# hyperplane-lab/RGBManip

Measured on AMD Instinct MI355X. Metric: adapose_poses_per_sec_batch256, higher is better.
Workload: dtype bf16

## Files before the change

### include/rgbm.h

```cpp
#ifndef RGBM_H_
#define RGBM_H_
#include <stddef.h>
#include <stdint.h>

#ifdef __cplusplus
extern "C" {
#endif

#define RGBM_VERSION 100
#define RGBM_F32 0
#define RGBM_BF16 1
#define RGBM_F16 2
#define RGBM_BF16X3 3

int rgbm_version(void);
const char* rgbm_last_error(void);

typedef struct rgbm_weight_desc {
  const char* name;
  const float* data;
  int ndim;
  const int64_t* shape;
} rgbm_weight_desc;

// ... 88 lines not shown
int rgbm_synth_render(const rgbm_synth_scene* scene, const double* rays_dev, float* color_dev, uint8_t* mask_dev, void* stream);

int rgbm_gae(int T, int N, const float* rewards, const uint8_t* dones, const float* values, const float* last_values,
             float gamma, float lam, float* returns, float* adv, double* sums, void* stream);
int rgbm_adv_normalise(int64_t n_local, float* adv, const double* sums, double count_total, void* stream);

typedef struct rgbm_policy_layout {
  int dims[5];
  int log_std;
  int w[2][4];
  int b[2][4];
  int total;
} rgbm_policy_layout;
int rgbm_policy_forward(const float* params, const rgbm_policy_layout* L, int n, int mode, const float* obs, const float* noise,
                        float* actions, float* logp, float* value, float* mu, void* stream);
int rgbm_ppo_partial_floats(const rgbm_policy_layout* L, int n, size_t* count);
int rgbm_ppo_minibatch_fwd_bwd(const float* params, const rgbm_policy_layout* L, int n, const float* obs, const float* actions,
                               const float* old_logp, const float* adv, const float* returns, const float* old_values,
                               const float* old_mu, const float* old_log_std, float clip, float vcoef, float ecoef,
                               float* partial_scratch, float* grads_flat, void* stream);
int rgbm_ppo_clip_adam(float* params, const float* grads_flat, float* exp_avg, float* exp_avg_sq, void* opt_state,
                       const rgbm_policy_layout* L, float inv_world, float max_norm, float desired_kl, float lr_min,
                       float lr_max, int adaptive, void* stream);

int rgbm_conv_nd(int dtype, const void* in_dev, int N, int D, int H, int W, int Cin, int Cin_pad, const float* w_host,
                 int Cout, int Cout_pad, int KD, int KH, int KW, int stride_d, int stride_hw, int pad_d, int pad_hw,
                 int dil_hw, int transposed, const float* bias_host, const float* bn_scale_host, const float* bn_shift_host,
                 const void* res_dev, int res_mode, int act, float slope, void* out_dev, void* stream);
int rgbm_bn_per_sample_scratch_bytes(int V, size_t* bytes);
int rgbm_bn_per_sample(int dtype, void* y_dev, const void* res_dev, const float* gamma_dev, const float* beta_dev, void* scratch_dev,
                       int V, int64_t nvox, int C, int relu, void* stream);
int rgbm_conv3d_tile(int layer, int dtype, const void* in_dev, int N, int D, int H, int W, const float* w_host,
                     const float* bn_scale_host, const float* bn_shift_host, const void* res_dev, void* out_dev, void* stream);
int rgbm_upsample_conv3x3(int dtype, const void* in_dev, int V, int h, int w, int Cin, const float* w_host, int Cout,
                          const float* bias_host, int act, float slope, void* z_scratch_dev, void* out_dev, void* stream);
int rgbm_upsample_conv3x3_final(int dtype, const void* in_dev, int V, int h, int w, const float* w3_host, const float* b3_host,
                                float slope, const float* wf_host, const float* bf_host, void* out_dev, int out_f32, void* stream);
int rgbm_stem(int dtype, const float* img1_dev, const float* img2_dev, const float* w_host, void* out_dev, int B, int S, void* stream);
int rgbm_maxpool3x3s2(int dtype, const void* in_dev, void* out_dev, int V, int H, int W, int C, void* stream);
int rgbm_resize_bilinear_ac(int dtype, const void* in_dev, void* out_dev, int V, int Hs, int Ws, int C, int Ho, int Wo,
                            void* stream);
int rgbm_adaptive_avgpool(int dtype, const void* in_dev, void* out_dev, int V, int H, int W, int C, int S, void* stream);
int rgbm_build_volume(int dtype, const void* feat_dev, const float* P_views_dev, const float* depths_dev, float* homog_scratch,
                      void* vol_dev, int V, int B, int D, int H, int W, void* stream);
int rgbm_conv0_sweep(const void* feat_dev, const float* P_views_dev, const float* depths_dev, float* homog_scratch,
                     const float* w_host, const float* bn_scale_host, const float* bn_shift_host, void* out_dev,
                     int V, int B, int D, int H, int W, void* stream);
int rgbm_conv0_sweep_dt(int dtype, const void* feat_dev, const float* P_views_dev, const float* depths_dev, float* homog_scratch,
                        const float* w_host, const float* bn_scale_host, const float* bn_shift_host, void* out_dev,
                        int V, int B, int D, int H, int W, void* stream);
int rgbm_conv0_sweep_f16feat(const void* feat_f16_dev, const float* P_views_dev, const float* depths_dev, float* homog_scratch,
                             const float* w_host, const float* bn_scale_host, const float* bn_shift_host, void* out_bf16_dev,
                             int V, int B, int D, int H, int W, void* stream);
int rgbm_adapose_forward_ex(rgbm_adapose_t* h, int B, const float* img1, const float* img2, const int32_t* choose1,
                            const int32_t* choose2, const float* P1, const float* P2, const float* depths, void* workspace,
                            size_t workspace_bytes, const rgbm_adapose_out* out, int stop_after, void* stream);
int rgbm_adapose_forward_graph(rgbm_adapose_t* h, int B, const float* img1, const float* img2, const int32_t* choose1,
                               const int32_t* choose2, const float* P1, const float* P2, const float* depths, void* workspace,
                               size_t workspace_bytes, const rgbm_adapose_out* out, void* stream, int32_t* n_nodes, int32_t* captured);
int rgbm_adapose_graph_clear(rgbm_adapose_t* h);
int rgbm_adapose_fetch(rgbm_adapose_t* h, int B, void* workspace, const char* name, float* out_dev, size_t capacity,
                       size_t* n_elems, void* stream);

#define RGBM_PROF_ROWS 42
int rgbm_debug_flags(int flags);
int rgbm_set_tuning(const char* key, long long value);
int rgbm_microbench_mfma_scratch_floats(int* n);
int rgbm_microbench_mfma(float* scratch, int iters, int random_operands, double* flops, void* stream);
int rgbm_microbench_copy(const void* src, void* dst, size_t bytes, void* stream);
int rgbm_prof_rows(void);
int rgbm_prof_start(void);
int rgbm_prof_stop(double* stats);
int rgbm_prof_select(int row);

#ifdef __cplusplus
}
#endif
#endif
```

### rgbmanip_amd/_lib.py

```python
from __future__ import annotations

import ctypes as C
import os

_HERE = os.path.dirname(os.path.abspath(__file__))
LIB_PATH = os.environ.get("RGBM_HIP_LIB") or os.path.join(_HERE, "librgbm_hip.so")

F32, BF16, F16, BF16X3 = 0, 1, 2, 3
ACT_NONE, ACT_RELU, ACT_PRELU, ACT_TANH = 0, 1, 2, 3
RES_NONE, RES_PRE_ACT, RES_POST_ACT = 0, 1, 2


PROF_ROWS = 42
PROF_KERNELS = [
    ("conv_igemm_glds_kernel<float, 16, 256>", "fp32"), ("conv_igemm_glds_kernel<float, 32, 256>", "fp32"),
    ("conv_igemm_glds_kernel<float, 64, 256>", "fp32"), ("conv_igemm_glds_kernel<float, 128, 128>", "fp32"),
    ("conv_igemm_glds_kernel<unsigned short, 16, 256>", "bf16"), ("conv_igemm_glds_kernel<unsigned short, 32, 256>", "bf16"),
    ("conv_igemm_glds_kernel<unsigned short, 64, 256>", "bf16"), ("conv_igemm_glds_kernel<unsigned short, 128, 128>", "bf16"),
    ("conv3d_tile_kernel<float, ...> (conv1..conv11)", "fp32"), ("conv3d_tile_kernel<unsigned short, ...> (conv1..conv11)", "bf16"),
    ("conv3d_tile_kernel<float, 32, 16, 4, 8, 8, 1, false, true> (conv0 + fused plane sweep)", "fp32"),
    ("conv3d_tile_kernel<unsigned short, 32, 16, 4, 8, 8, 1, false, true> (conv0 + fused plane sweep)", "bf16"),
    ("conv_igemm_ws_kernel<float, ...>", "fp32"), ("conv_igemm_ws_kernel<unsigned short, false, false> (128 channels x 256 pixels)", "bf16"),
    ("conv0_sweep_persistent_kernel<unsigned short> (conv0 + fused plane sweep of bf16 nets; sweep_f16 = 0 / fp16 nets: conv0_sweep_kernel)", "bf16"), ("conv_igemm_ws64_kernel", "bf16"),
    ("conv3d_tile_kernel<unsigned short, 32, 16, 6, 8, 8, 1, false, false> (conv0 on a materialised volume)", "bf16"),
# ... 47 lines not shown


class SynthScene(C.Structure):
    _fields_ = [("cam_pose", C.c_void_p), ("robot_pose", C.c_void_p), ("box", C.c_void_p),
                ("fx", C.c_double), ("fy", C.c_double), ("cx", C.c_double), ("cy", C.c_double),
                ("N", C.c_int), ("H", C.c_int), ("W", C.c_int), ("env0", C.c_int)]


_vp, _i, _f, _d, _sz, _i64 = C.c_void_p, C.c_int, C.c_float, C.c_double, C.c_size_t, C.c_int64

SIGNATURES = {
    "rgbm_version": (_i, []),
    "rgbm_last_error": (C.c_char_p, []),
    "rgbm_adapose_create": (_i, [C.POINTER(_vp), _i, C.POINTER(WeightDesc), _i, _i, _i]),
    "rgbm_adapose_destroy": (_i, [_vp]),
    "rgbm_adapose_set_chunk": (_i, [_vp, _i]),
    "rgbm_adapose_set_option": (_i, [_vp, C.c_char_p, _i]),
    "rgbm_adapose_workspace_bytes": (_i, [_vp, _i, C.POINTER(_sz)]),
    "rgbm_adapose_set_dropout": (_i, [_vp, _f, C.c_uint64]),
    "rgbm_adapose_dropout_masks": (_i, [_vp, _i, _vp]),
    "rgbm_adapose_set_dropout_masks": (_i, [_vp, _i, _vp]),
    "rgbm_adapose_forward": (_i, [_vp, _i, _vp, _vp, _vp, _vp, _vp, _vp, _vp, _vp, _sz, C.POINTER(AdaposeOut), _vp]),
    "rgbm_adapose_forward_ex": (_i, [_vp, _i, _vp, _vp, _vp, _vp, _vp, _vp, _vp, _vp, _sz, C.POINTER(AdaposeOut), _i, _vp]),
    "rgbm_adapose_forward_graph": (_i, [_vp, _i, _vp, _vp, _vp, _vp, _vp, _vp, _vp, _vp, _sz, C.POINTER(AdaposeOut), _vp, C.POINTER(C.c_int32),
                                        C.POINTER(C.c_int32)]),
    "rgbm_adapose_graph_clear": (_i, [_vp]),
    "rgbm_adapose_fetch": (_i, [_vp, _i, _vp, C.c_char_p, _vp, _sz, C.POINTER(_sz), _vp]),
    "rgbm_adapose_postprocess": (_i, [_i, _i, _i, _vp, _vp, _vp, _vp, _vp, _vp, _vp, _vp, _vp, _vp]),
    "rgbm_adapose_postprocess_scratch_bytes": (_i, [_i, C.POINTER(_sz)]),
    "rgbm_adapose_postprocess_ws": (_i, [_i, _i, _i, _vp, _vp, _vp, _vp, _vp, _vp, _vp, _vp, _vp, _vp, _sz, _vp]),
    "rgbm_adapose_postprocess_ransac": (_i, [_i, _i, _i, C.c_uint32, _vp, _vp, _vp, _vp, _vp, _vp, _vp, _vp, _vp]),
    "rgbm_adapose_postprocess_pnp": (_i, [_i, _i, C.c_uint32, _vp, _vp, _vp, _vp, _vp, _vp, _vp, _vp, _vp, _vp, _vp, _vp]),
    "rgbm_gae": (_i, [_i, _i, _vp, _vp, _vp, _vp, _f, _f, _vp, _vp, _vp, _vp]),
    "rgbm_adv_normalise": (_i, [_i64, _vp, _vp, _d, _vp]),
    "rgbm_policy_forward": (_i, [_vp, _vp, _i, _i, _vp, _vp, _vp, _vp, _vp, _vp, _vp]),
    "rgbm_ppo_partial_floats": (_i, [_vp, _i, C.POINTER(_sz)]),
    "rgbm_ppo_minibatch_fwd_bwd": (_i, [_vp, _vp, _i, _vp, _vp, _vp, _vp, _vp, _vp, _vp, _vp, _f, _f, _f, _vp, _vp, _vp]),
    "rgbm_ppo_clip_adam": (_i, [_vp, _vp, _vp, _vp, _vp, _vp, _f, _f, _f, _f, _f, _i, _vp]),
    "rgbm_conv_nd": (_i, [_i, _vp, _i, _i, _i, _i, _i, _i, _vp, _i, _i, _i, _i, _i, _i, _i, _i, _i, _i, _i, _vp, _vp, _vp,
                          _vp, _i, _i, _f, _vp, _vp]),
    "rgbm_bn_per_sample_scratch_bytes": (_i, [_i, C.POINTER(_sz)]),
    "rgbm_bn_per_sample": (_i, [_i, _vp, _vp, _vp, _vp, _vp, _i, _i64, _i, _i, _vp]),
    "rgbm_conv3d_tile": (_i, [_i, _i, _vp, _i, _i, _i, _i, _vp, _vp, _vp, _vp, _vp, _vp]),
    "rgbm_upsample_conv3x3": (_i, [_i, _vp, _i, _i, _i, _i, _vp, _i, _vp, _i, _f, _vp, _vp, _vp]),
    "rgbm_upsample_conv3x3_final": (_i, [_i, _vp, _i, _i, _i, _vp, _vp, _f, _vp, _vp, _vp, _i, _vp]),
    "rgbm_stem": (_i, [_i, _vp, _vp, _vp, _vp, _i, _i, _vp]),
    "rgbm_maxpool3x3s2": (_i, [_i, _vp, _vp, _i, _i, _i, _i, _vp]),
    "rgbm_resize_bilinear_ac": (_i, [_i, _vp, _vp, _i, _i, _i, _i, _i, _i, _vp]),
    "rgbm_adaptive_avgpool": (_i, [_i, _vp, _vp, _i, _i, _i, _i, _i, _vp]),
    "rgbm_build_volume": (_i, [_i, _vp, _vp, _vp, _vp, _vp, _i, _i, _i, _i, _i, _vp]),
    "rgbm_conv0_sweep": (_i, [_vp, _vp, _vp, _vp, _vp, _vp, _vp, _vp, _i, _i, _i, _i, _i, _vp]),
    "rgbm_conv0_sweep_dt": (_i, [_i, _vp, _vp, _vp, _vp, _vp, _vp, _vp, _vp, _i, _i, _i, _i, _i, _vp]),
    "rgbm_conv0_sweep_f16feat": (_i, [_vp, _vp, _vp, _vp, _vp, _vp, _vp, _vp, _i, _i, _i, _i, _i, _vp]),
    "rgbm_prepare_inputs": (_i, [_vp, _vp, _vp, _i, _i, _i, _i, _i, C.c_uint32, _vp, _vp, _vp, _vp, _vp, _vp, _vp, _vp]),
    "rgbm_prepare_inputs_indexed": (_i, [_vp, _vp, _vp, _vp, _i, _i, _i, _i, _i, C.c_uint32, _vp, _vp, _vp, _vp, _vp, _vp, _vp, _vp]),
    "rgbm_prepare_inputs_ex": (_i, [_vp, _vp, _vp, _vp, _i, _i, _i, _i, _i, _i, C.c_uint32, _vp, _vp, _vp, _vp, _vp, _vp, _vp, _vp]),
    "rgbm_projection": (_i, [_vp, _vp, _vp, _i, _vp]),
    "rgbm_mask_extent": (_i, [_vp, _i, _i, _i, _vp, _vp, _vp]),
    "rgbm_lookat_quat": (_i, [_vp, _i, _i, _vp, _vp]),
    "rgbm_control_action_to_pose": (_i, [_vp, _i, C.POINTER(C.c_double), C.POINTER(C.c_double), C.POINTER(C.c_double), _i, _vp, _vp]),
    "rgbm_control_reward": (_i, [C.POINTER(ControlRewardArgs), _vp]),
    "rgbm_control_grasp_frame": (_i, [_vp, _i, _vp, _vp, _vp]),
    "rgbm_synth_camera": (_i, [C.POINTER(SynthScene), _vp, _vp, _vp, _vp]),
    "rgbm_synth_render": (_i, [C.POINTER(SynthScene), _vp, _vp, _vp, _vp]),
    "rgbm_debug_flags": (_i, [_i]),
    "rgbm_set_tuning": (_i, [C.c_char_p, _i64]),
    "rgbm_prof_rows": (_i, []),
    "rgbm_microbench_mfma_scratch_floats": (_i, [C.POINTER(C.c_int)]),
    "rgbm_microbench_mfma": (_i, [_vp, _i, _i, C.POINTER(C.c_double), _vp]),
    "rgbm_microbench_copy": (_i, [_vp, _vp, C.c_size_t, _vp]),
    "rgbm_prof_start": (_i, []),
    "rgbm_prof_select": (_i, [_i]),
    "rgbm_prof_stop": (_i, [C.POINTER(C.c_double)]),
}

_lib = None


def load():
    global _lib
    if _lib is not None:
        return _lib
    if not os.path.exists(LIB_PATH):
        raise RgbmError(f"{LIB_PATH} not found: build it with rgbmanip_amd/csrc/build.sh "
                        f"(or `python -c 'import __graft_entry__ as g; g.build()'`). There is no CPU fallback.")
    lib = C.CDLL(LIB_PATH)
    for name, (res, args) in SIGNATURES.items():
        fn = getattr(lib, name)
        fn.restype = res
        fn.argtypes = args
    if lib.rgbm_prof_rows() != PROF_ROWS:
        raise RgbmError(f"{LIB_PATH}: rgbm_prof_rows() = {lib.rgbm_prof_rows()}, this binding expects {PROF_ROWS} (stale build?)")
    _lib = lib
    return lib


def check(rc: int, what: str = ""):
    if rc != 0:
        msg = load().rgbm_last_error()
        raise RgbmError(f"{what} failed (code {rc}): {msg.decode() if msg else ''}")


def stream_ptr(stream=None):
    import torch
    s = stream if stream is not None else torch.cuda.current_stream()
    return C.c_void_p(s.cuda_stream)
# ... 5 lines not shown
```

### rgbmanip_amd/csrc/adapose.cpp

```cpp
#include "adapose.h"

#include <math.h>
#include <string.h>

namespace rgbm {

static const int kLayerPlanes[4] = {64, 128, 256, 512};
static const int kLayerBlocks[4] = {3, 4, 6, 3};
static const int kLayerStride[4] = {1, 2, 1, 1};
static const int kLayerDil[4] = {1, 1, 2, 4};
static const int kPspBins[4] = {1, 2, 3, 6};
static const int kPspSmallViews = 32;


static const HostTensor* find(const StateDict& sd, const std::string& name) {
  auto it = sd.find(name);
  return it == sd.end() ? nullptr : &it->second;
}

#define GET(var, name)                                               \
  const HostTensor* var = find(sd, name);                            \
  RGBM_REQUIRE(var != nullptr, std::string("missing weight ") + (name))

static int init_conv2d(ConvLayer& L, int dtype, const StateDict& sd, const std::string& wname, const char* bname, int Cin,
// ... 205 lines not shown
      if (upload_f32(w->data, w->numel(), &head_w[h][l])) return -2;
      if (upload_f32(b->data, b->numel(), &head_b[h][l])) return -2;
    }
  }
  return 0;
}

void AdaPose::destroy() {
  conv1.destroy();
  if (stem_w) (void)hipFree(stem_w);
  stem_w = nullptr;
  for (int i = 0; i < n_blocks; ++i) { blocks[i].c1.destroy(); blocks[i].c2.destroy(); if (blocks[i].has_ds) blocks[i].ds.destroy(); }
  for (auto& l : psp) l.destroy();
  up1.destroy(); up2.destroy(); up3.destroy(); fin.destroy();
  up1c.destroy(); up2c.destroy(); tail.destroy();
  if (drop_masks) (void)hipFree(drop_masks);
  if (drop_state) (void)hipFree(drop_state);
  drop_masks = nullptr; drop_state = nullptr; drop_cap_views = 0; drop_p = 0.f; drop_explicit = 0; drop_last_B = 0;
  for (auto& l : c3d) l.destroy();
  for (auto& l : dc) l.destroy();
  for (auto& l : c3d_raw) l.destroy();
  for (auto& l : dc_raw) l.destroy();
  for (int i = 0; i < 10; ++i) { if (bn_gamma[i]) (void)hipFree(bn_gamma[i]); if (bn_beta[i]) (void)hipFree(bn_beta[i]); bn_gamma[i] = bn_beta[i] = nullptr; }
  inst.destroy();
  for (auto& l : nh) l.destroy();
  for (auto& l : npm) l.destroy();
  for (auto& l : pm1) l.destroy();
  for (auto& l : pm2) l.destroy();
  for (auto& t : t3d) { if (t.w) (void)hipFree(t.w); if (t.bias) (void)hipFree(t.bias); t.w = nullptr; t.bias = nullptr; }
  if (sweep_w) (void)hipFree(sweep_w);
  sweep_w = nullptr;
  if (sweep_w_f16) (void)hipFree(sweep_w_f16);
  sweep_w_f16 = nullptr;
  if (w11_x3) (void)hipFree(w11_x3);
  w11_x3 = nullptr;
  if (w11_taps) (void)hipFree(w11_taps);
  w11_taps = nullptr;
  if (wprob) (void)hipFree(wprob);
  if (pm2_0_wfull) (void)hipFree(pm2_0_wfull);
  if (pmlp_table) { (void)hipFree(pmlp_table); pmlp_table = nullptr; }
  if (pm2_0_bias) (void)hipFree(pm2_0_bias);
  for (int h = 0; h < 3; ++h) for (int l = 0; l < 3; ++l) { if (head_w[h][l]) (void)hipFree(head_w[h][l]); if (head_b[h][l]) (void)hipFree(head_b[h][l]); }
}

bool AdaPose::feat_f32_only() const {
  return dtype == BF16X3 && cost_impl == 3 && sweep_w != nullptr && norm_mode == 0 && !(g_debug_flags & 4096);
}

bool AdaPose::feat_f16() const {
  return dtype == BF16 && sweep_f16 != 0 && cost_impl == 3 && sweep_w_f16 != nullptr && norm_mode == 0 && !(g_debug_flags & 4096) && (upconv & 4) &&
         tail.ready() && tail.f16_ready();
}

bool AdaPose::sparse_active() const {
  const bool b16 = dtype_size(dtype) == 2;
  return sparse_dec != 0 && norm_mode == 0 && cost_impl == 3 && (b16 || (dtype == BF16X3 && w11_x3)) && sparse_tail && sweep_w != nullptr &&
         !(g_debug_flags & 4096);
}

int AdaPose::chunk_views(int V) const {
  const int cap = norm_mode == 1 && max_chunk > 32 ? 32 : max_chunk;
  return V < cap ? V : cap;
}

int AdaPose::plan(int B, Arena& A, Buffers& bf) const {
  const int V = 2 * B, P = n_pts, S = img;
  const size_t es = dtype_size(dtype);
  const size_t VP = (size_t)V * P;
  bf.Pviews = (float*)A.alloc((size_t)V * 16 * 4);
  bf.homog = (float*)A.alloc((size_t)V * 12 * 4);
  bf.choose = (int*)A.alloc(VP * 4);
  bf.masks = (unsigned char*)A.alloc((size_t)V * sparse_mask_bytes_per_view(img));
  bf.sweep_list = (int*)A.alloc((size_t)V * ((img + 11) / 12) * ((img + 15) / 16) * 4);
  bf.sweep_count = (int*)A.alloc((size_t)(V + 64) * 4);
  bf.feat = A.alloc((size_t)V * S * S * 32 * es);
  bf.featf = dtype == BF16X3 ? (float*)A.alloc((size_t)V * S * S * 32 * 4) : nullptr;
  bf.X0 = (float*)A.alloc(VP * 32 * 4);
  bf.X1 = (float*)A.alloc(VP * 64 * 4);
  bf.H128 = (float*)A.alloc(VP * 128 * 4);
  bf.H64 = (float*)A.alloc(VP * 64 * 4);
  bf.nocs4 = (float*)A.alloc(VP * 4 * 4);
  bf.N32 = (float*)A.alloc(VP * 32 * 4);
  bf.PF96 = (float*)A.alloc(VP * 96 * 4);
  bf.PF96h = pose_dtype() == F16 ? A.alloc(VP * 96 * 2) : nullptr;
  bf.prob = (float*)A.alloc(VP * n_depth * 4);
  bf.depth = (float*)A.alloc(VP * 4);
  bf.Q128a = (float*)A.alloc(VP * 128 * 4);
  bf.Q128b = (float*)A.alloc(VP * 128 * 4);
  bf.G256a = (float*)A.alloc(VP * 256 * 4);
  bf.G256b = (float*)A.alloc(VP * 256 * 4);
  bf.glob = (float*)A.alloc((size_t)V * 128 * 4);
  bf.vbias = (float*)A.alloc((size_t)V * 256 * 4);
  bf.pf2 = (float*)A.alloc((size_t)V * 256 * 4);
  bf.h1 = (float*)A.alloc((size_t)V * 256 * 4);
  bf.h2 = (float*)A.alloc((size_t)V * 128 * 4);
  bf.r6 = (float*)A.alloc((size_t)V * 8 * 4);
  bf.R = (float*)A.alloc((size_t)V * 9 * 4);
  bf.tv = (float*)A.alloc((size_t)V * 4 * 4);
  bf.sv = (float*)A.alloc((size_t)V * 4 * 4);
  const size_t m0 = A.mark();
  bf.imgpad = A.alloc((size_t)V * S * S * img_cpad * es);
  bf.c1 = A.alloc((size_t)V * (S / 2) * (S / 2) * 64 * es);
  const size_t lbuf = (size_t)V * ((size_t)(S / 4) * (S / 4) * 64 > (size_t)(S / 8) * (S / 8) * 512 ? (size_t)(S / 4) * (S / 4) * 64 : (size_t)(S / 8) * (S / 8) * 512) * es;
  for (int i = 0; i < 4; ++i) bf.lb[i] = A.alloc(lbuf);
  for (int i = 0; i < 4; ++i) {
    bf.pooled[i] = A.alloc((size_t)V * kPspBins[i] * kPspBins[i] * 512 * es);
    bf.stage[i] = A.alloc((size_t)V * kPspBins[i] * kPspBins[i] * 128 * es);
  }
  const size_t f8 = (size_t)(S / 8) * (S / 8), f4 = (size_t)(S / 4) * (S / 4), f2 = (size_t)(S / 2) * (S / 2), f1 = (size_t)S * S;
  bf.cat = A.alloc((size_t)V * f8 * 1024 * es);
  bf.ups = A.alloc((size_t)V * f4 * 1024 * es);
  bf.u1 = A.alloc((size_t)V * f4 * 256 * es);
  bf.u2 = A.alloc((size_t)V * f2 * 64 * es);
  bf.u3 = A.alloc((size_t)V * f1 * 64 * es);
  A.release(m0);
  const int Vc = chunk_views(V);
  const int D = n_depth;
  const size_t vox = (size_t)D * S * S;
  bf.vol = (cost_impl >= 2 && norm_mode == 0) ? nullptr : A.alloc((size_t)Vc * vox * 32 * es);
  bf.bn_scratch = norm_mode == 1 ? A.alloc(bn_scratch_bytes(Vc)) : nullptr;
  bf.c[0] = A.alloc((size_t)Vc * vox * 8 * es);
  bf.c[1] = A.alloc((size_t)Vc * (vox / 8) * 16 * es);
  bf.c[2] = A.alloc((size_t)Vc * (vox / 8) * 16 * es);
  bf.c[3] = A.alloc((size_t)Vc * (vox / 64) * 32 * es);
  bf.c[4] = A.alloc((size_t)Vc * (vox / 64) * 32 * es);
  bf.c[5] = A.alloc((size_t)Vc * (vox / 512) * 64 * es);
  bf.c[6] = A.alloc((size_t)Vc * (vox / 512) * 64 * es);
  bf.u7 = A.alloc((size_t)Vc * (vox / 64) * 32 * es);
// ... 39 lines not shown
      if (int rc = blk.ds.run(x, r, V, 1, H, W, blk.planes, nullptr, 0, nullptr, 0, s)) return rc;
      res = r;
    }
    if (int rc = blk.c2.run(t, y, V, 1, Ho, Wo, blk.planes, res, RES_PRE_ACT, nullptr, 0, s)) return rc;
    H = Ho; W = Wo;
    xi = (xi + 3) & 3;
  }
  const void* f = bf.lb[xi];
  last_f_index = xi;
  RGBM_REQUIRE(H == S / 8 && W == S / 8, "feature stride");
  if (g_debug_flags & 1024) {
    if (int rc = launch_copy_channels(dtype, f, bf.cat, (long long)V * H * W, 512, 1024, 0, s)) return rc;
    {
      void* outs[4] = {bf.pooled[0], bf.pooled[1], bf.pooled[2], bf.pooled[3]};
      if (int rc = launch_adaptive_avgpool_multi(dtype, f, outs, kPspBins, 4, V, H, W, 512, s)) return rc;
    }
    for (int i = 0; i < 4; ++i) {
      const int Sb = kPspBins[i];
      if (int rc = psp[i].run(bf.pooled[i], bf.stage[i], V, 1, Sb, Sb, 128, nullptr, 0, nullptr, 0, s)) return rc;
      if (int rc = launch_resize_bilinear_ac(dtype, bf.stage[i], bf.cat, V, Sb, Sb, 128, H, W, 1024, 512 + 128 * i, s)) return rc;
    }
  } else {
    bool small = V <= kPspSmallViews;
    for (int i = 0; i < 4; ++i)
      small = small && psp[i].packs.size() == 1 && psp[i].packs[0].Kpad == 512 && psp[i].Cout_pad == 128 && psp[i].bias == nullptr;
    if (small) {
      const void* w[4] = {psp[0].packs[0].w, psp[1].packs[0].w, psp[2].packs[0].w, psp[3].packs[0].w};
      void* outs[4] = {bf.stage[0], bf.stage[1], bf.stage[2], bf.stage[3]};
      if (int rc = launch_psp_pool_conv(dtype, f, 512, w, outs, kPspBins, V, H, W, psp[0].g.act, psp[0].g.slope, s)) return rc;
    } else {
      void* outs[4] = {bf.pooled[0], bf.pooled[1], bf.pooled[2], bf.pooled[3]};
      if (int rc = launch_adaptive_avgpool_multi(dtype, f, outs, kPspBins, 4, V, H, W, 512, s)) return rc;
      for (int i = 0; i < 4; ++i)
        if (int rc = psp[i].run(bf.pooled[i], bf.stage[i], V, 1, kPspBins[i], kPspBins[i], 128, nullptr, 0, nullptr, 0, s)) return rc;
    }
    const void* stages[4] = {bf.stage[0], bf.stage[1], bf.stage[2], bf.stage[3]};
    if (int rc = launch_psp_resize_cat(dtype, f, stages, kPspBins, bf.cat, V, H, W, s)) return rc;
  }
  RGBM_REQUIRE(drop == nullptr || (upconv & 3) == 3, "dropout needs option upconv bits 0 and 1 (up_1 / up_2 through the tap combination)");
  if (upconv & 1) {
    if (int rc = up1c.run(bf.cat, bf.ups, bf.u1, V, H, W, 256, s, drop)) return rc;
  } else {
    if (int rc = launch_resize_bilinear_ac(dtype, bf.cat, bf.ups, V, H, W, 1024, 2 * H, 2 * W, 1024, 0, s)) return rc;
    if (int rc = up1.run(bf.ups, bf.u1, V, 1, 2 * H, 2 * W, 256, nullptr, 0, nullptr, 0, s)) return rc;
  }
  if (upconv & 2) {
    if (int rc = up2c.run(bf.u1, bf.ups, bf.u2, V, 2 * H, 2 * W, 64, s, drop ? drop + 256 : nullptr)) return rc;
  } else {
    if (int rc = launch_resize_bilinear_ac(dtype, bf.u1, bf.ups, V, 2 * H, 2 * W, 256, 4 * H, 4 * W, 256, 0, s)) return rc;
    if (int rc = up2.run(bf.ups, bf.u2, V, 1, 4 * H, 4 * W, 64, nullptr, 0, nullptr, 0, s)) return rc;
  }
  fin.out_plain_f32 = feat_f32_only();
  if ((upconv & 4) && tail.ready())
    return tail.run(bf.u2, fin.out_plain_f32 ? (void*)bf.featf : bf.feat, fin.out_plain_f32 ? 1 : feat_f16() ? 2 : 0, V, 4 * H, 4 * W, s);
  if (int rc = launch_resize_bilinear_ac(dtype, bf.u2, bf.ups, V, 4 * H, 4 * W, 64, 8 * H, 8 * W, 64, 0, s)) return rc;
  fin.out_plain_f32 = feat_f32_only();
  if (int rc = up3.run_then_1x1(fin, bf.ups, bf.u3, 64, fin.out_plain_f32 ? (void*)bf.featf : bf.feat, 32, V, 1, 8 * H, 8 * W, fuse_final != 0, nullptr, s)) return rc;
  return 0;
}

int AdaPose::cost_volume(const Buffers& bf, int V, int B, const float* depths, hipStream_t s) const {
  const int S = img, D = n_depth, P = n_pts;
  const int Vh = view2_heads ? V : B;
  const int Vc0 = chunk_views(V);
  const bool b16 = dtype_size(dtype) == 2;
  bool sweep_sparse = false;
  auto tile = [&](int layer, const void* in, void* out, const void* res, int Vc, int Di, int Hi, int Wi, int Do, int Ho,
                  int Wo, bool transposed, int v0, const unsigned char* tmask = nullptr) -> int {
    const int li = layer == 10 ? 0 : layer;
    Conv3dTileDesc d;
    memset(&d, 0, sizeof(d));
    d.in = in; d.wgt = t3d[li].w; d.out = out; d.bias = t3d[li].bias; d.res = res;
    d.N = Vc; d.Di = Di; d.Hi = Hi; d.Wi = Wi; d.Do = Do; d.Ho = Ho; d.Wo = Wo;
    d.Dq = transposed ? Di : Do; d.Hq = transposed ? Hi : Ho; d.Wq = transposed ? Wi : Wo;
    d.Cout = t3d[li].Cout; d.relu = 1;
    d.feat = bf.feat; d.homog = bf.homog; d.depths = depths; d.v0 = v0; d.V = V; d.B = B;
    d.out_classmajor = layer == 9 ? 1 : 0;
    d.tile_mask = tmask;
    d.tile_mask_stride = sparse_mask_bytes_per_view(S);
    if (layer == 10 && sweep_sparse) { d.tile_list = bf.sweep_list; d.tile_count = bf.sweep_count; }
    d.prof_variant = dtype == BF16X3 ? (layer == 10 ? 28 : 27) : layer == 10 ? 10 + (dtype != F32 ? 1 : 0) : (dtype != F32 ? 16 + layer : 8);
    d.algo_flops = 2.0 * Vc * (double)(transposed ? Di * Hi * Wi : Do * Ho * Wo) * t3d[li].Cout * 27.0 * t3d[li].Cin;
    d.algo_bytes = ((layer == 10 ? (double)Vc * Hi * Wi * t3d[li].Cin : (double)Vc * Di * Hi * Wi * t3d[li].Cin) +
                    (double)Vc * Do * Ho * Wo * t3d[li].Cout * (res ? 2 : 1)) * (double)dtype_size(dtype);
    if (layer == 10 && cost_impl == 3 && b16 && sweep_w && !(g_debug_flags & 4096)) {
      d.wgt = sweep_w;
      if (feat_f16()) { d.wgt = sweep_w_f16; d.feat_f16 = 1; }
      return launch_conv0_sweep(d, dtype, s);
    }
    if (layer == 10 && cost_impl == 3 && dtype == BF16X3 && sweep_w && !(g_debug_flags & 4096)) {
      d.wgt = sweep_w;
      d.feat = bf.featf;
      return launch_conv0_sweep_x3(d, s);
    }
    return launch_conv3d_tile(layer, dtype, d, s);
  };
  const bool sparse_ok = sparse_active();
  for (int v0 = 0; norm_mode == 0 && cost_impl >= 1 && v0 < Vh; v0 += Vc0) {
    const int Vc = Vh - v0 < Vc0 ? Vh - v0 : Vc0;
    const unsigned char* mk[10] = {nullptr, nullptr, nullptr, nullptr, nullptr, nullptr, nullptr, nullptr, nullptr, nullptr};
    sweep_sparse = false;
    if (sparse_ok) {
      int td, th, tw;
      for (int L : {1, 2, 3, 4, 5, 7, 8}) RGBM_REQUIRE(!conv3d_tile_dims(L, dtype, &td, &th, &tw) && th == 8 && tw == 8, "sparse cost regularisation: 8 x 8 tiles expected");
      if (int rc = launch_sparse_masks(bf.choose, v0, Vc, P, S, bf.masks, bf.sweep_list, bf.sweep_count, s)) return rc;
      for (int L : {7, 8}) mk[L] = bf.masks + sparse_mask_offset(S, L);
      if (sparse_dec >= 2) {
        for (int L : {1, 2, 3, 4, 5}) mk[L] = bf.masks + sparse_mask_offset(S, L);
        sweep_sparse = true;
      }
    }
    if (cost_impl == 1) {
      if (int rc = launch_build_volume(dtype, bf.feat, bf.homog, depths, bf.vol, v0, Vc, V, B, D, S, S, s)) return rc;
      if (int rc = tile(0, bf.vol, bf.c[0], nullptr, Vc, D, S, S, D, S, S, false, v0)) return rc;
    } else {
      if (int rc = tile(10, nullptr, bf.c[0], nullptr, Vc, D, S, S, D, S, S, false, v0)) return rc;
    }
    if (int rc = tile(1, bf.c[0], bf.c[1], nullptr, Vc, D, S, S, D / 2, S / 2, S / 2, false, v0, mk[1])) return rc;
    if (int rc = tile(2, bf.c[1], bf.c[2], nullptr, Vc, D / 2, S / 2, S / 2, D / 2, S / 2, S / 2, false, v0, mk[2])) return rc;
    if (int rc = tile(3, bf.c[2], bf.c[3], nullptr, Vc, D / 2, S / 2, S / 2, D / 4, S / 4, S / 4, false, v0, mk[3])) return rc;
    if (int rc = tile(4, bf.c[3], bf.c[4], nullptr, Vc, D / 4, S / 4, S / 4, D / 4, S / 4, S / 4, false, v0, mk[4])) return rc;
    if (int rc = tile(5, bf.c[4], bf.c[5], nullptr, Vc, D / 4, S / 4, S / 4, D / 8, S / 8, S / 8, false, v0, mk[5])) return rc;
    if (cost_impl == 3 && (b16 || dtype == BF16X3) && igemm_conv6) {
      if (int rc = c3d[6].run(bf.c[5], bf.c[6], Vc, D / 8, S / 8, S / 8, 64, nullptr, RES_NONE, nullptr, 0, s)) return rc;
    } else {
      if (int rc = tile(6, bf.c[5], bf.c[6], nullptr, Vc, D / 8, S / 8, S / 8, D / 8, S / 8, S / 8, false, v0)) return rc;
    }
    if (int rc = tile(7, bf.c[6], bf.u7, bf.c[4], Vc, D / 8, S / 8, S / 8, D / 4, S / 4, S / 4, true, v0, mk[7])) return rc;
    if (int rc = tile(8, bf.u7, bf.u9, bf.c[2], Vc, D / 4, S / 4, S / 4, D / 2, S / 2, S / 2, true, v0, mk[8])) return rc;
    if (cost_impl == 3 && (b16 || (dtype == BF16X3 && w11_x3)) && sparse_tail) {
      if (int rc = launch_prob_sparse(bf.u9, bf.c[0], dtype == BF16X3 ? w11_x3 : t3d[9].w, t3d[9].bias, wprob, bf.choose, depths, bf.prob,
                                      bf.depth, v0, Vc, B, P, D, S, S, dtype, s, w11_taps)) return rc;
      continue;
    }
    if (int rc = tile(9, bf.u9, bf.u11, bf.c[0], Vc, D / 2, S / 2, S / 2, D, S, S, true, v0)) return rc;
    if (int rc = launch_prob_softmax_depth(dtype, bf.u11, wprob, bf.choose, depths, bf.prob, bf.depth, v0, Vc, B, P, D, S, S, 1, s)) return rc;
  }
  for (int v0 = 0; norm_mode == 1 && v0 < Vh; v0 += Vc0) {
    const int Vc = Vh - v0 < Vc0 ? Vh - v0 : Vc0;
    if (int rc = launch_build_volume(dtype, bf.feat, bf.homog, depths, bf.vol, v0, Vc, V, B, D, S, S, s)) return rc;
// ... 28 lines not shown
    if (int rc = c3d[5].run(bf.c[4], bf.c[5], Vc, D / 4, S / 4, S / 4, 64, nullptr, 0, nullptr, 0, s)) return rc;
    if (int rc = c3d[6].run(bf.c[5], bf.c[6], Vc, D / 8, S / 8, S / 8, 64, nullptr, 0, nullptr, 0, s)) return rc;
    if (int rc = dc[0].run(bf.c[6], bf.u7, Vc, D / 8, S / 8, S / 8, 32, bf.c[4], RES_POST_ACT, nullptr, 0, s)) return rc;
    if (int rc = dc[1].run(bf.u7, bf.u9, Vc, D / 4, S / 4, S / 4, 16, bf.c[2], RES_POST_ACT, nullptr, 0, s)) return rc;
    if (int rc = dc[2].run(bf.u9, bf.u11, Vc, D / 2, S / 2, S / 2, 8, bf.c[0], RES_POST_ACT, nullptr, 0, s)) return rc;
    if (int rc = launch_prob_softmax_depth(dtype, bf.u11, wprob, bf.choose, depths, bf.prob, bf.depth, v0, Vc, B, P, D, S, S, 0, s)) return rc;
  }
  return 0;
}

int AdaPose::forward(int B, const float* img1, const float* img2, const int* choose1, const int* choose2, const float* P1,
                     const float* P2, const float* depths, void* workspace, size_t workspace_size, const Outputs& out,
                     hipStream_t s, int stop_after) const {
  RGBM_REQUIRE(B > 0, "batch");
  RGBM_REQUIRE(((uintptr_t)workspace & 255) == 0, "workspace must be 256-byte aligned");
  RGBM_REQUIRE(n_depth % 8 == 0 && img % 8 == 0, "depth/img must be multiples of 8");
  const size_t need = workspace_bytes(B);
  RGBM_REQUIRE(workspace_size >= need, "workspace too small: need " + std::to_string(need));
  Arena A(workspace, workspace_size);
  Buffers bf;
  plan(B, A, bf);
  const int V = 2 * B, P = n_pts, S = img, D = n_depth;
  const size_t VP = (size_t)V * P;

  if (int rc = launch_stage_in(P1, P2, choose1, choose2, bf.Pviews, bf.choose, B, P, s)) return rc;
  const float* drop = nullptr;
  if (drop_active()) {
    RGBM_REQUIRE(V <= drop_cap_views && drop_masks && (drop_explicit || drop_state), "dropout: mask buffer smaller than the batch");
    RGBM_REQUIRE((upconv & 3) == 3, "dropout needs option upconv bits 0 and 1 (up_1 / up_2 through the tap combination)");
    if (drop_explicit) {
      RGBM_REQUIRE(drop_explicit == B, "dropout: the masks set for the next forward are for batch " + std::to_string(drop_explicit));
      drop_explicit = 0;
    } else {
      if (int rc = launch_dropout_masks(drop_masks, drop_state, B, drop_p, drop_seed, drop_no_advance ? 0 : 1, s)) return rc;
    }
    drop = drop_masks;
    drop_last_B = B;
  }
  if (int rc = pspnet(bf, V, img1, img2, s, drop)) return rc;
  if (int rc = launch_homography(bf.Pviews, bf.homog, V, B, s)) return rc;
  const void* featg = bf.feat;
  int fdt = dtype;
  if (dtype == BF16X3) {
    if (!feat_f32_only())
      if (int rc = launch_bx3_to_f32(bf.feat, bf.featf, (long long)V * S * S * 32, s)) return rc;
    featg = bf.featf; fdt = F32;
  }
  if (feat_f16()) fdt = F16;
  if (stop_after == 1) return 0;

  const int Vh = view2_heads ? V : B;
  if (pmlp_table != nullptr && !(g_debug_flags & 2048) && ((long long)Vh * P) % 64 == 0) {
    PointMlpDesc pd{};
    pd.table = pmlp_table; pd.feat = featg; pd.choose = bf.choose; pd.nocs4 = bf.nocs4; pd.pf = bf.PF96 + 32; pd.ldpf = 96; pd.P = P; pd.HW = S * S;
    pd.N = (long long)Vh * P;
    if (int rc = launch_point_mlp(fdt, pd, s)) return rc;
  } else {
    if (int rc = launch_gather_points(fdt, featg, bf.choose, bf.X0, Vh, P, S * S, 32, s)) return rc;
    if (int rc = inst.run(bf.X0, bf.X1, Vh, 1, 1, P, 64, nullptr, 0, nullptr, 0, s)) return rc;
    if (int rc = nh[0].run(bf.X1, bf.H128, Vh, 1, 1, P, 128, nullptr, 0, nullptr, 0, s)) return rc;
    if (int rc = nh[1].run(bf.H128, bf.H64, Vh, 1, 1, P, 64, nullptr, 0, nullptr, 0, s)) return rc;
    if (int rc = nh[2].run(bf.H64, bf.nocs4, Vh, 1, 1, P, 4, nullptr, 0, nullptr, 0, s)) return rc;
    if (int rc = npm[0].run(bf.nocs4, bf.N32, Vh, 1, 1, P, 32, nullptr, 0, nullptr, 0, s)) return rc;
    if (int rc = npm[1].run(bf.N32, bf.PF96 + 32, Vh, 1, 1, P, 96, nullptr, 0, nullptr, 0, s)) return rc;
  }

  if (int rc = cost_volume(bf, V, B, depths, s)) return rc;
  if (stop_after == 2) return 0;

  if (int rc = launch_fuse_points(fdt, featg, bf.homog, depths, bf.choose, bf.prob, bf.PF96, V, B, P, D, S, S, 96, 0, s, Vh)) return rc;
  const int pdt = pose_dtype();
  const void* pf_in = bf.PF96;
  if (pdt == F16) {
    if (int rc = launch_f32_to_f16(bf.PF96, bf.PF96h, (long long)Vh * P * 96, s)) return rc;
    pf_in = bf.PF96h;
  } else if (pdt == BF16X3) {
    if (int rc = launch_f32_to_bx3(bf.PF96, bf.PF96, (long long)Vh * P * 96, s)) return rc;
  }
  if (int rc = pm1[0].run(pf_in, bf.Q128a, Vh, 1, 1, P, 128, nullptr, 0, nullptr, 0, s)) return rc;
  if (int rc = pm1[1].run(bf.Q128a, bf.Q128b, Vh, 1, 1, P, 128, nullptr, 0, nullptr, 0, s)) return rc;
  if (int rc = launch_mean_points_partial(pdt, bf.Q128b, (float*)bf.Q128a, Vh, P, 128, s)) return rc;
  if (int rc = launch_view_linear_mean((const float*)bf.Q128a, P, bf.glob, pm2_0_wfull, pm2_0_bias, bf.vbias, Vh, 128, 256, 256, 128, 0, s)) return rc;
  if (int rc = pm2[0].run(bf.Q128b, bf.G256a, Vh, 1, 1, P, 256, nullptr, 0, bf.vbias, 256, s)) return rc;
  if (int rc = pm2[1].run(bf.G256a, bf.G256b, Vh, 1, 1, P, 256, nullptr, 0, nullptr, 0, s)) return rc;
  if (int rc = launch_mean_points_partial(pdt, bf.G256b, (float*)bf.G256a, Vh, P, 256, s)) return rc;
  float* hout[3] = {bf.r6, bf.tv, bf.sv};
  const int hdim[3] = {6, 3, 3};
  if (int rc = launch_pose_heads_mean((const float*)bf.G256a, P, bf.pf2, bf.R, head_w, head_b, hout, hdim, Vh, s)) return rc;

  {
    float* const on[2] = {out.nocs1, out.nocs2};
    float* const od[2] = {out.depth1, out.depth2};
    float* const orr[2] = {out.r1, out.r2};
    float* const ot[2] = {out.t1, out.t2};
    float* const os[2] = {out.s1, out.s2};
    if (int rc = launch_stage_out(bf.nocs4, bf.depth, bf.R, bf.tv, bf.sv, on, od, orr, ot, os, B, P, view2_heads, s)) return rc;
  }
  (void)VP;
  return 0;
}

}
```

### rgbmanip_amd/csrc/adapose.h

```cpp
#pragma once
#include "kernels.h"
#include "layers.h"

namespace rgbm {

struct Arena {
  char* base; size_t off; size_t cap; size_t peak;
  explicit Arena(void* b, size_t c) : base((char*)b), off(0), cap(c), peak(0) {}
  void* alloc(size_t bytes) {
    off = align_up(off, 256);
    void* p = base ? base + off : nullptr;
    off += bytes;
    if (off > peak) peak = off;
    return p;
  }
  size_t mark() const { return off; }
  void release(size_t m) { off = m; }
};

struct AdaPose {
  int dtype = F32;
  int pose_dtype() const { return dtype == BF16 ? F16 : (dtype == BF16X3 && pose_x3) ? BF16X3 : F32; }
  int pose_x3 = 1;
  int img = 224, n_pts = 1024, n_depth = 24;
// ... 28 lines not shown
  void* sweep_w = nullptr;
  int cost_impl = 3;
  void* w11_x3 = nullptr;
  float* wprob = nullptr;
  ConvLayer inst, nh[3], npm[2], pm1[2], pm2[2];
  float* pm2_0_wfull = nullptr;
  float* pmlp_table = nullptr;
  float* pm2_0_bias = nullptr;
  float* head_w[3][3] = {{nullptr}};
  float* head_b[3][3] = {{nullptr}};

  float drop_p = 0.f;
  unsigned long long drop_seed = 0;
  float* drop_masks = nullptr;
  unsigned long long* drop_state = nullptr;
  int drop_cap_views = 0;
  mutable int drop_explicit = 0;
  mutable int drop_last_B = 0;
  int drop_no_advance = 0;
  bool drop_active() const { return drop_p > 0.f || drop_explicit > 0; }

  struct Buffers {
    float *Pviews, *homog; int* choose; void* feat;
    unsigned char* masks;
    int *sweep_list, *sweep_count;
    float* featf;
    float *X0, *X1, *H128, *H64, *nocs4, *N32, *PF96, *prob, *depth, *Q128a, *Q128b, *G256a, *G256b;
    void* PF96h;
    float *glob, *vbias, *pf2, *h1, *h2, *r6, *R, *tv, *sv;
    void *imgpad, *c1, *lb[4], *pooled[4], *stage[4], *cat, *ups, *u1, *u2, *u3;
    void *vol, *c[7], *u7, *u9, *u11;
    void* bn_scratch;
  };
  struct Outputs {
    float *nocs1, *nocs2;
    float *depth1, *depth2;
    float *r1, *r2;
    float *t1, *t2, *s1, *s2;
  };

  int create(const StateDict& sd, int dtype, int norm_mode = 0);
  void destroy();
  size_t workspace_bytes(int B) const;
  int forward(int B, const float* img1, const float* img2, const int* choose1, const int* choose2, const float* P1,
              const float* P2, const float* depths, void* workspace, size_t workspace_size, const Outputs& out,
              hipStream_t s, int stop_after = 0) const;
  mutable int last_f_index = 0;

  int plan(int B, Arena& A, Buffers& bf) const;
  int pspnet(const Buffers& bf, int V, const float* img1, const float* img2, hipStream_t s, const float* drop = nullptr) const;
  int cost_volume(const Buffers& bf, int V, int B, const float* depths, hipStream_t s) const;
  int chunk_views(int V) const;
  bool feat_f32_only() const;
  bool feat_f16() const;
  bool sparse_active() const;
};

const char* last_error_cstr();

}
```

### rgbmanip_amd/csrc/capi.cpp

```cpp
#include "../../include/rgbm.h"

#include <string.h>

#include <algorithm>
#include <string>
#include <vector>

#include "adapose.h"
#include "control.h"
#include "prof.h"

using namespace rgbm;

struct ForwardGraph {
  int B = 0;
  const void* in[7] = {nullptr};
  void* ws = nullptr;
  size_t ws_bytes = 0;
  rgbm_adapose_out out;
  int opt_version = 0;
  int tuning_version = 0;
  hipGraph_t graph = nullptr;
  hipGraphExec_t exec = nullptr;
  size_t nodes = 0;
// ... 189 lines not shown
    ++i;
  }
  if (!hit) {
    h->net.drop_no_advance = 1;
    const int rw = h->net.forward(B, img1, img2, choose1, choose2, P1, P2, depths, workspace, workspace_bytes, to_out(out), s, 0);
    h->net.drop_no_advance = 0;
    if (rw) return rw;
    ForwardGraph g;
    g.B = B; memcpy(g.in, in, sizeof(in)); g.ws = workspace; g.ws_bytes = workspace_bytes; g.out = *out;
    g.opt_version = h->opt_version; g.tuning_version = g_tuning_version;
    RGBM_CHECK_HIP(hipStreamBeginCapture(s, hipStreamCaptureModeThreadLocal));
    const int rc = h->net.forward(B, img1, img2, choose1, choose2, P1, P2, depths, workspace, workspace_bytes, to_out(out), s, 0);
    const hipError_t ee = hipStreamEndCapture(s, &g.graph);
    if (rc) { if (g.graph) (void)hipGraphDestroy(g.graph); return rc; }
    if (ee != hipSuccess || !g.graph) { set_error(std::string("hipStreamEndCapture: ") + hipGetErrorString(ee)); return -2; }
    if (hipGraphGetNodes(g.graph, nullptr, &g.nodes) != hipSuccess) g.nodes = 0;
    const hipError_t ei = hipGraphInstantiate(&g.exec, g.graph, nullptr, nullptr, 0);
    if (ei != hipSuccess) { (void)hipGraphDestroy(g.graph); set_error(std::string("hipGraphInstantiate: ") + hipGetErrorString(ei)); return -2; }
    if (h->graphs.size() >= kMaxGraphs) {
      size_t lru = 0;
      for (size_t i = 1; i < h->graphs.size(); ++i) if (h->graphs[i].last_use < h->graphs[lru].last_use) lru = i;
      drop_graph(h->graphs[lru]);
      h->graphs.erase(h->graphs.begin() + lru);
    }
    h->graphs.push_back(g);
    hit = &h->graphs.back();
    if (captured) *captured = 1;
  }
  hit->last_use = ++h->tick;
  if (n_nodes) *n_nodes = (int32_t)hit->nodes;
  RGBM_CHECK_HIP(hipGraphLaunch(hit->exec, s));
  return 0;
}

int rgbm_adapose_fetch(rgbm_adapose_t* h, int B, void* workspace, const char* name, float* out_dev, size_t capacity,
                       size_t* n_elems, void* stream) {
  RGBM_REQUIRE(h && workspace && name && out_dev && n_elems, "fetch arguments");
  const AdaPose& n = h->net;
  Arena A(workspace, 0);
  AdaPose::Buffers bf;
  n.plan(B, A, bf);
  const size_t V = 2 * (size_t)B, S = n.img, P = n.n_pts, D = n.n_depth;
  const size_t Vc = n.chunk_views((int)V);
  const std::string nm = name;
  const void* src = nullptr; size_t cnt = 0; int dt = n.dtype;
  if (nm == "imgpad") { src = bf.imgpad; cnt = V * S * S * n.img_cpad; }
  else if (nm == "conv1") { src = bf.c1; cnt = V * (S / 2) * (S / 2) * 64; }
  else if (nm == "layer4") { src = bf.lb[n.last_f_index]; cnt = V * (S / 8) * (S / 8) * 512; }
  else if (nm == "cat") { src = bf.cat; cnt = V * (S / 8) * (S / 8) * 1024; }
  else if (nm == "u1") { src = bf.u1; cnt = V * (S / 4) * (S / 4) * 256; }
  else if (nm == "u2") { src = bf.u2; cnt = V * (S / 2) * (S / 2) * 64; }
  else if (nm == "u3") { src = bf.u3; cnt = V * S * S * 64; }
  else if (nm == "feat") { src = bf.feat; cnt = V * S * S * 32; if (n.feat_f32_only()) { src = bf.featf; dt = F32; } else if (n.feat_f16()) dt = F16; }
  else if (nm == "vol") { src = bf.vol; cnt = Vc * D * S * S * 32; }
  else if (nm == "c0") { src = bf.c[0]; cnt = Vc * D * S * S * 8; }
  else if (nm == "c2") { src = bf.c[2]; cnt = Vc * (D / 2) * (S / 2) * (S / 2) * 16; }
  else if (nm == "c4") { src = bf.c[4]; cnt = Vc * (D / 4) * (S / 4) * (S / 4) * 32; }
  else if (nm == "c6") { src = bf.c[6]; cnt = Vc * (D / 8) * (S / 8) * (S / 8) * 64; }
  else if (nm == "u7") { src = bf.u7; cnt = Vc * (D / 4) * (S / 4) * (S / 4) * 32; }
  else if (nm == "u9") { src = bf.u9; cnt = Vc * (D / 2) * (S / 2) * (S / 2) * 16; }
  else if (nm == "u11") { src = bf.u11; cnt = Vc * D * S * S * 8; }
  else if (nm == "homog") { src = bf.homog; cnt = V * 12; dt = F32; }
  else if (nm == "prob") { src = bf.prob; cnt = V * P * D; dt = F32; }
  else if (nm == "pf96") { src = bf.PF96; cnt = V * P * 96; dt = n.pose_dtype() == BF16X3 ? BF16X3 : F32; }
  else if (nm == "pf2") { src = bf.pf2; cnt = V * 256; dt = F32; }
  else if (nm == "r6") { src = bf.r6; cnt = V * 6; dt = F32; }
  RGBM_REQUIRE(src != nullptr, "unknown intermediate name: " + nm);
  const bool tap3d = nm == "c0" || nm == "c2" || nm == "c4" || nm == "c6" || nm == "u7" || nm == "u9";
  RGBM_REQUIRE(!(tap3d && n.sparse_active()), "tap '" + nm + "' needs a dense cost regularisation: set option sparse_dec = 0 before the forward "
               "(the default computes it only inside the chosen pixels' dependency cones)");
  *n_elems = cnt;
  RGBM_REQUIRE(cnt <= capacity, "fetch capacity too small");
  return launch_to_f32(dt, src, out_dev, (long long)cnt, (hipStream_t)stream);
}

int rgbm_adapose_postprocess(int B, int P, int img_size, const float* nocs1, const float* depth1, const float* r1,
                             const int32_t* choose1, const double* Kcrop, const double* E1, double* bbox_world, double* ts,
                             int32_t* valid, void* stream) {
  RGBM_REQUIRE(B > 0 && nocs1 && depth1 && r1 && choose1 && Kcrop && E1 && bbox_world && ts && valid, "postprocess arguments");
  return launch_postprocess(nocs1, depth1, r1, choose1, Kcrop, E1, bbox_world, ts, valid, B, P, img_size, (hipStream_t)stream);
}

int rgbm_adapose_postprocess_scratch_bytes(int B, size_t* bytes) {
  RGBM_REQUIRE(B > 0 && bytes, "postprocess_scratch_bytes arguments");
  *bytes = postprocess_slices(B) > 1 ? postprocess_scratch_bytes(B) : 0;
  return 0;
}

int rgbm_adapose_postprocess_ws(int B, int P, int img_size, const float* nocs1, const float* depth1, const float* r1,
                                const int32_t* choose1, const double* Kcrop, const double* E1, double* bbox_world, double* ts,
                                int32_t* valid, void* scratch, size_t scratch_bytes, void* stream) {
  RGBM_REQUIRE(B > 0 && nocs1 && depth1 && r1 && choose1 && Kcrop && E1 && bbox_world && ts && valid, "postprocess arguments");
  return launch_postprocess(nocs1, depth1, r1, choose1, Kcrop, E1, bbox_world, ts, valid, B, P, img_size, (hipStream_t)stream,
                            scratch, scratch_bytes);
}

int rgbm_adapose_postprocess_ransac(int B, int P, int img_size, uint32_t seed, const float* nocs1, const float* depth1,
                                    const int32_t* choose1, const double* Kcrop, const double* E1, double* bbox_world, double* srt,
                                    int32_t* valid, void* stream) {
  return launch_umeyama_ransac(nocs1, depth1, choose1, Kcrop, E1, bbox_world, srt, valid, B, P, img_size, seed, (hipStream_t)stream);
}

int rgbm_gae(int T, int N, const float* rewards, const uint8_t* dones, const float* values, const float* last_values,
             float gamma, float lam, float* returns, float* adv, double* sums, void* stream) {
  RGBM_REQUIRE(rewards && dones && values && last_values && returns && adv && sums, "gae arguments");
  return launch_gae(T, N, rewards, dones, values, last_values, gamma, lam, returns, adv, sums, (hipStream_t)stream);
}

int rgbm_adv_normalise(int64_t n_local, float* adv, const double* sums, double count_total, void* stream) {
  RGBM_REQUIRE(adv && sums && n_local > 0 && count_total > 1.0, "adv_normalise arguments");
  return launch_adv_normalise(n_local, adv, sums, count_total, (hipStream_t)stream);
}

int rgbm_conv_nd(int dtype, const void* in_dev, int N, int D, int H, int W, int Cin, int Cin_pad, const float* w_host,
                 int Cout, int Cout_pad, int KD, int KH, int KW, int stride_d, int stride_hw, int pad_d, int pad_hw,
                 int dil_hw, int transposed, const float* bias_host, const float* bn_scale_host, const float* bn_shift_host,
                 const void* res_dev, int res_mode, int act, float slope, void* out_dev, void* stream) {
  RGBM_REQUIRE(in_dev && w_host && out_dev, "conv arguments");
  ConvGeom g;
  g.Cin = Cin; g.Cout = Cout; g.KD = KD; g.KH = KH; g.KW = KW;
  g.sd = stride_d; g.sh = g.sw = stride_hw; g.pd = pad_d; g.ph = g.pw = pad_hw;
  g.dild = 1; g.dilh = g.dilw = dil_hw; g.transposed = transposed != 0; g.act = act; g.slope = slope;
  ConvLayer L;
  int rc = L.init(dtype, g, w_host, bias_host, bn_scale_host, bn_shift_host, Cin_pad, Cout_pad);
  if (!rc) rc = L.run(in_dev, out_dev, N, D, H, W, Cout_pad, res_dev, res_mode, nullptr, 0, (hipStream_t)stream);
// ... 73 lines not shown
}
int rgbm_microbench_mfma(float* scratch, int iters, int random_operands, double* flops, void* stream) {
  return rgbm::launch_microbench_mfma(scratch, iters, random_operands, flops, (hipStream_t)stream);
}
int rgbm_microbench_copy(const void* src, void* dst, size_t bytes, void* stream) {
  return rgbm::launch_microbench_copy(src, dst, bytes, (hipStream_t)stream);
}
int rgbm_prof_start(void) { return rgbm::prof_start(); }
int rgbm_prof_select(int row) {
  RGBM_REQUIRE(row >= -1 && row < rgbm::kProfVariants, "prof_select: row out of range");
  return rgbm::prof_select(row);
}
int rgbm_prof_stop(double* stats) {
  RGBM_REQUIRE(stats != nullptr, "prof_stop arguments");
  return rgbm::prof_stop(stats, rgbm::kProfVariants);
}
}

extern "C" int rgbm_conv3d_tile(int layer, int dtype, const void* in_dev, int N, int D, int H, int W, const float* w_host,
                                const float* bn_scale_host, const float* bn_shift_host, const void* res_dev, void* out_dev,
                                void* stream) {
  static const int cin[10] = {32, 8, 16, 16, 32, 32, 64, 64, 32, 16};
  static const int cout[10] = {8, 16, 16, 32, 32, 64, 64, 32, 16, 8};
  static const int stride[10] = {1, 2, 1, 2, 1, 2, 1, 1, 1, 1};
  RGBM_REQUIRE(layer >= 0 && layer < 10 && in_dev && w_host && bn_scale_host && bn_shift_host && out_dev, "conv3d_tile arguments");
  const bool tr = layer >= 7;
  const int coutp = cout[layer] < 16 ? 16 : cout[layer];
  std::vector<float> packed;
  conv3d_tile_pack(w_host, bn_scale_host, cin[layer], cout[layer], coutp, tr, dtype, packed);
  void* wdev = nullptr; float* bdev = nullptr;
  if (upload_packed(packed, dtype, &wdev)) return -2;
  std::vector<float> bpad(coutp, 0.f);
  for (int o = 0; o < cout[layer]; ++o) bpad[o] = bn_shift_host[o];
  if (upload_f32(bpad.data(), bpad.size(), &bdev)) return -2;
  Conv3dTileDesc d;
  memset(&d, 0, sizeof(d));
  d.in = in_dev; d.wgt = wdev; d.out = out_dev; d.bias = bdev; d.res = res_dev;
  d.N = N; d.Di = D; d.Hi = H; d.Wi = W;
  if (tr) { d.Do = 2 * D; d.Ho = 2 * H; d.Wo = 2 * W; d.Dq = D; d.Hq = H; d.Wq = W; }
  else {
    const int s = stride[layer];
    d.Do = (D + 2 - 3) / s + 1; d.Ho = (H + 2 - 3) / s + 1; d.Wo = (W + 2 - 3) / s + 1;
    d.Dq = d.Do; d.Hq = d.Ho; d.Wq = d.Wo;
  }
  d.Cout = cout[layer]; d.relu = 1; d.prof_variant = -1;
  int rc = launch_conv3d_tile(layer, dtype, d, (hipStream_t)stream);
  if (!rc) { hipError_t e = hipStreamSynchronize((hipStream_t)stream); if (e != hipSuccess) { set_error(hipGetErrorString(e)); rc = -2; } }
  (void)hipFree(wdev); (void)hipFree(bdev);
  return rc;
}

static int conv0_sweep_entry(int dtype, int feat_f16, const void* feat_dev, const float* P_views_dev, const float* depths_dev,
                             float* homog_scratch, const float* w_host, const float* bn_scale_host, const float* bn_shift_host,
                             void* out_dev, int V, int B, int D, int H, int W, void* stream) {
  RGBM_REQUIRE(feat_dev && P_views_dev && depths_dev && homog_scratch && w_host && bn_scale_host && bn_shift_host && out_dev,
               "conv0_sweep arguments");
  RGBM_REQUIRE(dtype == BF16 || dtype == F16 || dtype == BF16X3, "conv0_sweep: 16-bit storage types or bf16x3 (fp32 features in, split-pair c0 out)");
  if (int rc = launch_homography(P_views_dev, homog_scratch, V, B, (hipStream_t)stream)) return rc;
  std::vector<float> packed;
  conv0_sweep_pack(w_host, bn_scale_host, packed);
  void* wdev = nullptr; float* bdev = nullptr;
  if (dtype == BF16X3) { if (conv0_sweep_x3_upload(packed, &wdev)) return -2; }
  else if (upload_packed(packed, feat_f16 ? (int)F16 : dtype, &wdev)) return -2;
  std::vector<float> bpad(16, 0.f);
  for (int o = 0; o < 8; ++o) bpad[o] = bn_shift_host[o];
  if (upload_f32(bpad.data(), bpad.size(), &bdev)) return -2;
  Conv3dTileDesc d;
  memset(&d, 0, sizeof(d));
  d.wgt = wdev; d.out = out_dev; d.bias = bdev;
  d.N = V; d.Di = D; d.Hi = H; d.Wi = W; d.Do = D; d.Ho = H; d.Wo = W; d.Dq = D; d.Hq = H; d.Wq = W;
  d.Cout = 8; d.relu = 1; d.prof_variant = -1;
  d.feat = feat_dev; d.homog = homog_scratch; d.depths = depths_dev; d.v0 = 0; d.V = V; d.B = B;
  d.feat_f16 = feat_f16;
  int rc = dtype == BF16X3 ? launch_conv0_sweep_x3(d, (hipStream_t)stream) : launch_conv0_sweep(d, dtype, (hipStream_t)stream);
  if (!rc) { hipError_t e = hipStreamSynchronize((hipStream_t)stream); if (e != hipSuccess) { set_error(hipGetErrorString(e)); rc = -2; } }
  (void)hipFree(wdev); (void)hipFree(bdev);
  return rc;
}

extern "C" int rgbm_conv0_sweep_dt(int dtype, const void* feat_dev, const float* P_views_dev, const float* depths_dev,
                                   float* homog_scratch, const float* w_host, const float* bn_scale_host, const float* bn_shift_host,
                                   void* out_dev, int V, int B, int D, int H, int W, void* stream) {
  return conv0_sweep_entry(dtype, 0, feat_dev, P_views_dev, depths_dev, homog_scratch, w_host, bn_scale_host, bn_shift_host, out_dev, V, B, D,
                           H, W, stream);
}

extern "C" int rgbm_conv0_sweep_f16feat(const void* feat_f16_dev, const float* P_views_dev, const float* depths_dev,
                                        float* homog_scratch, const float* w_host, const float* bn_scale_host,
                                        const float* bn_shift_host, void* out_bf16_dev, int V, int B, int D, int H, int W, void* stream) {
  return conv0_sweep_entry(BF16, 1, feat_f16_dev, P_views_dev, depths_dev, homog_scratch, w_host, bn_scale_host, bn_shift_host, out_bf16_dev,
                           V, B, D, H, W, stream);
}

extern "C" int rgbm_conv0_sweep(const void* feat_dev, const float* P_views_dev, const float* depths_dev, float* homog_scratch,
                                const float* w_host, const float* bn_scale_host, const float* bn_shift_host, void* out_dev,
                                int V, int B, int D, int H, int W, void* stream) {
  return rgbm_conv0_sweep_dt(BF16, feat_dev, P_views_dev, depths_dev, homog_scratch, w_host, bn_scale_host, bn_shift_host, out_dev,
                             V, B, D, H, W, stream);
}

extern "C" int rgbm_prepare_inputs(const float* rgb_dev, const uint8_t* mask_dev, const double* K_dev, int N, int H, int W, int S,
                                   int P, uint32_t seed, float* img_out, int32_t* choose_out, float* pts2d_out, double* Kcrop_out,
                                   int32_t* window_out, int32_t* valid_out, uint8_t* scratch, void* stream) {
  return launch_prepare_inputs(rgb_dev, mask_dev, K_dev, nullptr, N, H, W, S, P, seed, img_out, choose_out, pts2d_out, Kcrop_out,
                               window_out, valid_out, scratch, (hipStream_t)stream);
}

extern "C" int rgbm_prepare_inputs_indexed(const float* rgb_dev, const uint8_t* mask_dev, const double* K_dev,
                                           const int32_t* frame_map_dev, int N, int H, int W, int S, int P, uint32_t seed,
                                           float* img_out, int32_t* choose_out, float* pts2d_out, double* Kcrop_out,
                                           int32_t* window_out, int32_t* valid_out, uint8_t* scratch, void* stream) {
  RGBM_REQUIRE(frame_map_dev, "prepare_inputs_indexed frame_map");
  return launch_prepare_inputs(rgb_dev, mask_dev, K_dev, frame_map_dev, N, H, W, S, P, seed, img_out, choose_out, pts2d_out,
                               Kcrop_out, window_out, valid_out, scratch, (hipStream_t)stream);
}

extern "C" int rgbm_prepare_inputs_ex(const float* rgb_dev, const uint8_t* mask_dev, const double* K_dev, const int32_t* frame_map_dev,
                                      int frame0, int N, int H, int W, int S, int P, uint32_t seed, float* img_out, int32_t* choose_out,
                                      float* pts2d_out, double* Kcrop_out, int32_t* window_out, int32_t* valid_out, uint8_t* scratch,
                                      void* stream) {
  RGBM_REQUIRE(frame0 >= 0, "prepare_inputs_ex frame0");
  return launch_prepare_inputs(rgb_dev, mask_dev, K_dev, frame_map_dev, N, H, W, S, P, seed, img_out, choose_out, pts2d_out,
                               Kcrop_out, window_out, valid_out, scratch, (hipStream_t)stream, frame0);
}

extern "C" int rgbm_adapose_postprocess_pnp(int B, int P, uint32_t seed, const float* nocs1, const float* pts2d1, const float* nocs2,
                                            const float* pts2d2, const double* K, const double* E1, const double* E2, double* bbox_out,
                                            double* srt_out, int32_t* info_out, int32_t* valid_out, void* stream) {
  return launch_pnp_ransac(nocs1, pts2d1, nocs2, pts2d2, K, E1, E2, bbox_out, srt_out, info_out, valid_out, B, P, seed, (hipStream_t)stream);
}

extern "C" int rgbm_projection(const double* Kcrop_dev, const double* E_dev, float* P_dev, int N, void* stream) {
  return launch_projection(Kcrop_dev, E_dev, P_dev, N, (hipStream_t)stream);
}

extern "C" int rgbm_mask_extent(const uint8_t* mask_dev, int N, int H, int W, int32_t* ext_out, int32_t* count_out, void* stream) {
  return launch_mask_extent(mask_dev, N, H, W, ext_out, count_out, (hipStream_t)stream);
}

static_assert(sizeof(rgbm_control_reward_args) == sizeof(rgbm::ControlRewardArgs), "control reward args ABI mismatch");
static_assert(sizeof(rgbm_synth_scene) == sizeof(rgbm::SynthScene), "synth scene ABI mismatch");
extern "C" int rgbm_lookat_quat(const double* dir_dev, int N, int batch_zero, double* quat_dev, void* stream) {
  return rgbm::launch_lookat_quat(dir_dev, quat_dev, N, batch_zero, (hipStream_t)stream);
}
// ... 68 lines not shown
```

### rgbmanip_amd/csrc/conv0_sweep.hip

```cpp
#include <type_traits>
#include "common.h"
#include "kernels.h"
#include "prof.h"


namespace rgbm {

namespace {

constexpr int SW_TH = 12, SW_TW = 16;
constexpr int SW_HH = SW_TH + 2, SW_HW = SW_TW + 2;
constexpr int SW_NV = SW_HH * SW_HW;
#ifndef SW_COOP
#define SW_COOP 1
#endif
constexpr int SW_LAG = 1;
#ifndef SW_NSLOT_N
#define SW_NSLOT_N 3
#endif
#ifndef SW_VS_BYTES
#define SW_VS_BYTES 80
#endif
constexpr int SW_VS = SW_VS_BYTES;
constexpr int SW_SLOT = SW_NV * SW_VS;
constexpr int SW_NPW = (SW_NV + 63) / 64;
#ifndef SW_SKIP
#define SW_SKIP 0
#endif
#ifndef SW_OCC
#define SW_OCC 3
#endif
#ifndef SW_CR
#define SW_CR 3
#endif
constexpr int SW_CR_ = SW_CR;
constexpr int SW_NCW = SW_TH / SW_CR_;
constexpr int SW_THREADS = (SW_NPW + SW_NCW) * 64;
constexpr int SW_NSLOT = SW_NSLOT_N;
constexpr int SW_LDS = SW_NSLOT * SW_SLOT;
static_assert(SW_TH % SW_CR_ == 0, "a consumer wave owns SW_CR rows");
static_assert(SW_NSLOT_N > SW_LAG, "the ring holds the plane being written and the SW_LAG behind it");
constexpr int SW_NPAIR = (SW_CR_ + 1) / 2;

struct SweepDesc {
  const unsigned short* feat;
  const unsigned short* wgt;
  const float* bias;
  const float* homog;
  const float* depths;
  unsigned short* out;
  int N, D, H, W, v0, V, B, nth, ntw, relu;
  const int* tile_list; const int* tile_count;
};

struct Corner {
  unsigned off[4];
  float w[4];
  unsigned wp[4];
  bool skip;
};

typedef __attribute__((ext_vector_type(2))) float f32x2;
typedef __attribute__((ext_vector_type(4))) unsigned u32x4;

template <typename T> struct Sw16;
typedef __attribute__((ext_vector_type(4))) unsigned sw_u4v;
template <> struct Sw16<unsigned short> {
  __device__ static __forceinline__ f32x2 unpack(unsigned u) { return f32x2{__uint_as_float(u << 16), __uint_as_float(u & 0xffff0000u)}; }
  __device__ static __forceinline__ unsigned pack(f32x2 v) { return pack2_bf16(v.x, v.y); }
  __device__ static __forceinline__ f32x4 mma(const uint4& a, const uint4& b, const f32x4& c) {
    return __builtin_amdgcn_mfma_f32_16x16x32_bf16(__builtin_bit_cast(bf16x8, a), __builtin_bit_cast(bf16x8, b), c, 0, 0, 0);
  }
};
template <> struct Sw16<f16_t> {
  typedef __attribute__((ext_vector_type(2))) _Float16 h2;
  __device__ static __forceinline__ f32x2 unpack(unsigned u) { return __builtin_convertvector(__builtin_bit_cast(h2, u), f32x2); }
  __device__ static __forceinline__ unsigned pack(f32x2 v) {
    const h2 h = {(f16_t)sat_f16(v.x), (f16_t)sat_f16(v.y)};
    return __builtin_bit_cast(unsigned, h);
  }
  __device__ static __forceinline__ f32x4 mma(const uint4& a, const uint4& b, const f32x4& c) {
    return __builtin_amdgcn_mfma_f32_16x16x32_f16(__builtin_bit_cast(f16x8, a), __builtin_bit_cast(f16x8, b), c, 0, 0, 0);
  }
};

template <typename T, int BL>
__device__ __forceinline__ uint4 blend_chunk(const uint4& r, const u32x4& a, const u32x4& b, const u32x4& c, const u32x4& e,
                                             const Corner& cn) {
  const float* w = cn.w;
  const unsigned rr[4] = {r.x, r.y, r.z, r.w}, aa[4] = {a[0], a[1], a[2], a[3]}, bb[4] = {b[0], b[1], b[2], b[3]};
  const unsigned cc[4] = {c[0], c[1], c[2], c[3]}, ee[4] = {e[0], e[1], e[2], e[3]};
  unsigned o[4];
#pragma unroll
  for (int q = 0; q < 4; ++q) {
    if constexpr (BL == 2) {
      const f32x2 fr = Sw16<T>::unpack(rr[q]);
      const unsigned ab_lo = __builtin_amdgcn_perm(bb[q], aa[q], 0x05040100u), ab_hi = __builtin_amdgcn_perm(bb[q], aa[q], 0x07060302u);
      const unsigned ce_lo = __builtin_amdgcn_perm(ee[q], cc[q], 0x05040100u), ce_hi = __builtin_amdgcn_perm(ee[q], cc[q], 0x07060302u);
      typedef __bf16 bf2 __attribute__((ext_vector_type(2)));
      const bf2 w01 = __builtin_bit_cast(bf2, cn.wp[0]), w23 = __builtin_bit_cast(bf2, cn.wp[1]);
      float t0 = __builtin_amdgcn_fdot2_f32_bf16(__builtin_bit_cast(bf2, ab_lo), w01, fr.x, false);
      float t1 = __builtin_amdgcn_fdot2_f32_bf16(__builtin_bit_cast(bf2, ab_hi), w01, fr.y, false);
      t0 = __builtin_amdgcn_fdot2_f32_bf16(__builtin_bit_cast(bf2, ce_lo), w23, t0, false);
      t1 = __builtin_amdgcn_fdot2_f32_bf16(__builtin_bit_cast(bf2, ce_hi), w23, t1, false);
// ... 41 lines not shown
    asm("v_pk_fma_f16 %0, %1, %2, %0" : "+v"(t) : "v"(ee[q]), "v"(cn.wp[3]));
    o[q] = t;
  }
  } else {
#pragma unroll
  for (int q = 0; q < 4; ++q) {
    float lo, hi;
    asm("v_fma_mix_f32 %0, %1, %2, 0 op_sel:[0,0,0] op_sel_hi:[1,0,0]" : "=v"(lo) : "v"(aa[q]), "v"(w[0]));
    asm("v_fma_mix_f32 %0, %1, %2, 0 op_sel:[1,0,0] op_sel_hi:[1,0,0]" : "=v"(hi) : "v"(aa[q]), "v"(w[0]));
    SW_MIX(0, lo, bb[q], w[1], lo); SW_MIX(1, hi, bb[q], w[1], hi);
    SW_MIX(0, lo, cc[q], w[2], lo); SW_MIX(1, hi, cc[q], w[2], hi);
    SW_MIX(0, lo, ee[q], w[3], lo); SW_MIX(1, hi, ee[q], w[3], hi);
    asm("v_fma_mix_f32 %0, %1, 1.0, %2 op_sel:[0,0,0] op_sel_hi:[1,0,0]" : "=v"(lo) : "v"(rr[q]), "v"(lo));
    asm("v_fma_mix_f32 %0, %1, 1.0, %2 op_sel:[1,0,0] op_sel_hi:[1,0,0]" : "=v"(hi) : "v"(rr[q]), "v"(hi));
    const h2 h = {(f16_t)lo, (f16_t)hi};
    o[q] = __builtin_bit_cast(unsigned, h);
  }
  }
  return make_uint4(o[0], o[1], o[2], o[3]);
}
#undef SW_MIX

__device__ __forceinline__ void sw_ray(const float (&hm)[12], float x, float y, float& rx, float& ry, float& rz) {
  rx = __builtin_fmaf(hm[0], x, __builtin_fmaf(hm[1], y, hm[2]));
  ry = __builtin_fmaf(hm[3], x, __builtin_fmaf(hm[4], y, hm[5]));
  rz = __builtin_fmaf(hm[6], x, __builtin_fmaf(hm[7], y, hm[8]));
}
__device__ __forceinline__ void sw_corner_weights(float rx, float ry, float rz, float t0, float t1, float t2, float depth, float sx, float sy,
                                                  int W, int H, bool inb, float (&w)[4], unsigned (&off)[4]) {
  const float px = __builtin_fmaf(rx, depth, t0), py = __builtin_fmaf(ry, depth, t1), pz = __builtin_fmaf(rz, depth, t2);
  const float rinv = __builtin_amdgcn_rcpf(pz);
  const float ix = __builtin_fmaf(px * rinv, sx, -0.5f), iy = __builtin_fmaf(py * rinv, sy, -0.5f);
  const bool fin = isfinite(ix) && isfinite(iy);
  const float fx = floorf(ix), fy = floorf(iy);
  const int x0 = (int)fx, y0 = (int)fy;
  const float tx = ix - fx, ty = iy - fy;
  const bool xin0 = (unsigned)x0 < (unsigned)W, xin1 = (unsigned)(x0 + 1) < (unsigned)W;
  const bool yin0 = (unsigned)y0 < (unsigned)H, yin1 = (unsigned)(y0 + 1) < (unsigned)H;
  const int xc0 = min(max(x0, 0), W - 1), xc1 = min(max(x0, -1) + 1, W - 1);
  const int yc0 = min(max(y0, 0), H - 1), yc1 = min(max(y0, -1) + 1, H - 1);
  const float ux = 1.f - tx, uy = 1.f - ty;
  w[0] = (inb && xin0 && yin0) ? ux * uy : 0.f;
  w[1] = (inb && xin1 && yin0) ? tx * uy : 0.f;
  w[2] = (inb && xin0 && yin1) ? ux * ty : 0.f;
  w[3] = (inb && xin1 && yin1) ? tx * ty : 0.f;
  if (inb && !fin) w[0] = __builtin_nanf("");
  const unsigned r0 = (unsigned)(yc0 * W), r1 = (unsigned)(yc1 * W);
  off[0] = (r0 + (unsigned)xc0) * 64u;
  off[1] = (r0 + (unsigned)xc1) * 64u;
  off[2] = (r1 + (unsigned)xc0) * 64u;
  off[3] = (r1 + (unsigned)xc1) * 64u;
}

}

template <typename T, typename TO, int BL>
__global__ __launch_bounds__(SW_THREADS, SW_OCC) void conv0_sweep_kernel(const SweepDesc d) {
  extern __shared__ __attribute__((aligned(16))) unsigned char planes[];
  const int tid = threadIdx.x, lane = tid & 63, wave = tid >> 6;

  const int nblk = d.tile_list ? d.tile_count[0] : (int)gridDim.x;
  if ((int)blockIdx.x >= nblk) return;
  const int bq = nblk >> 3, br = nblk & 7, xcd = blockIdx.x & 7, bidx = blockIdx.x >> 3;
  int t = (xcd < br ? xcd * (bq + 1) : br * (bq + 1) + (xcd - br) * bq) + bidx;
  if (d.tile_list) t = d.tile_list[t];
  const int tw = t % d.ntw; t /= d.ntw;
  const int th = t % d.nth; t /= d.nth;
  const int n = t;
  const int h0 = th * SW_TH, w0 = tw * SW_TW;
  const int D = d.D, H = d.H, W = d.W;
  const int vv = d.v0 + n;

  if (wave < SW_NPW) {
    if (std::is_same<T, f16_t>::value) __builtin_amdgcn_s_setreg(1 | (23 << 6), 1);
    if constexpr (BL == 3 && SW_COOP != 0) {
    const int ck = lane & 3;
    const int pv = tid;
    const bool act = pv < SW_NV;
    const int hh = pv / SW_HW, hw = pv - hh * SW_HW;
    const int gh = h0 - 1 + hh, gw = w0 - 1 + hw;
    const bool inb = act && (unsigned)gh < (unsigned)H && (unsigned)gw < (unsigned)W;
    const int partner = (vv + d.B) % d.V, bb = vv % d.B;
    const float* __restrict__ hm = d.homog + (long long)vv * 12;
    const float* __restrict__ dep = d.depths + (long long)bb * D;
    const unsigned char* __restrict__ srcb = reinterpret_cast<const unsigned char*>(d.feat + (long long)partner * H * W * 32);
    uint4 ref[4];
    unsigned dsto[4];
    bool actr[4];
#pragma unroll
    for (int r = 0; r < 4; ++r) {
      const int cv = wave * 64 + (lane & ~3) + r;
      const int ch_ = cv / SW_HW, cw_ = cv - ch_ * SW_HW;
      const int ggh = h0 - 1 + ch_, ggw = w0 - 1 + cw_;
      actr[r] = cv < SW_NV;
      dsto[r] = (unsigned)(cv * SW_VS + ck * 16);
      ref[r] = make_uint4(0u, 0u, 0u, 0u);
      if (actr[r] && (unsigned)ggh < (unsigned)H && (unsigned)ggw < (unsigned)W)
        ref[r] = *reinterpret_cast<const uint4*>(d.feat + (((long long)vv * H + ggh) * W + ggw) * 32 + ck * 8);
    }
    float hmv[12];
#pragma unroll
    for (int e = 0; e < 12; ++e) hmv[e] = hm[e];
    float rx, ry, rz;
    sw_ray(hmv, (float)gw, (float)gh, rx, ry, rz);
    const float t0 = hmv[9], t1 = hmv[10], t2 = hmv[11];
    const float sx = (float)W / (float)(W - 1), sy = (float)H / (float)(H - 1);
    const int dbits = __float_as_int(lane < D ? dep[lane] : 1.f);
    auto corners = [&](int z, unsigned (&off)[4], unsigned (&wp)[4]) {
      float w[4];
      sw_corner_weights(rx, ry, rz, t0, t1, t2, __int_as_float(__builtin_amdgcn_readlane(dbits, z)), sx, sy, W, H, inb, w, off);
#pragma unroll
      for (int q = 0; q < 4; ++q) {
        const Sw16<f16_t>::h2 h = {(f16_t)w[q], (f16_t)w[q]};
        wp[q] = __builtin_bit_cast(unsigned, h);
      }
    };
    u32x4 g[4][4];
#pragma unroll
    for (int k = 0; k < 4; ++k)
#pragma unroll
      for (int q = 0; q < 4; ++q) g[k][q] = u32x4{0u, 0u, 0u, 0u};
    unsigned wco[4][4];
#define SW_CGATHER(R, Q, OFF) asm volatile("global_load_dwordx4 %0, %1, %2" : "+v"(g[R][Q]) : "v"(OFF), "s"(srcb) : "memory")
#define SW_CWAIT12(K) asm volatile("s_waitcnt vmcnt(12)" : "+v"(g[K][0]), "+v"(g[K][1]), "+v"(g[K][2]), "+v"(g[K][3]) :: "memory")
#define SW_CREQ(R, OFFV, WPV)                                                                                         \
    do {                                                                                                              \
      unsigned o_[4];                                                                                                 \
      _Pragma("unroll") for (int q = 0; q < 4; ++q) {                                                                 \
        o_[q] = (unsigned)__builtin_amdgcn_update_dpp(0, (int)(OFFV)[q], (R) * 0x55, 0xf, 0xf, false) | (unsigned)(ck * 16);      \
        wco[R][q] = (unsigned)__builtin_amdgcn_update_dpp(0, (int)(WPV)[q], (R) * 0x55, 0xf, 0xf, false);             \
      }                                                                                                               \
      SW_CGATHER(R, 0, o_[0]); SW_CGATHER(R, 1, o_[1]); SW_CGATHER(R, 2, o_[2]); SW_CGATHER(R, 3, o_[3]);             \
    } while (0)
    unsigned noff[4], nwp[4];
    corners(0, noff, nwp);
    SW_CREQ(0, noff, nwp); SW_CREQ(1, noff, nwp); SW_CREQ(2, noff, nwp); SW_CREQ(3, noff, nwp);
    auto blend4 = [&](const uint4& r, const u32x4& a, const u32x4& b, const u32x4& c, const u32x4& e, const unsigned (&w)[4]) {
      const unsigned rr[4] = {r.x, r.y, r.z, r.w}, aa[4] = {a[0], a[1], a[2], a[3]}, bb4[4] = {b[0], b[1], b[2], b[3]};
      const unsigned cc[4] = {c[0], c[1], c[2], c[3]}, ee[4] = {e[0], e[1], e[2], e[3]};
      unsigned o[4];
#pragma unroll
      for (int q = 0; q < 4; ++q) {
        unsigned t;
        asm("v_pk_fma_f16 %0, %1, %2, %3" : "=v"(t) : "v"(aa[q]), "v"(w[0]), "v"(rr[q]));
        asm("v_pk_fma_f16 %0, %1, %2, %0" : "+v"(t) : "v"(bb4[q]), "v"(w[1]));
        asm("v_pk_fma_f16 %0, %1, %2, %0" : "+v"(t) : "v"(cc[q]), "v"(w[2]));
        asm("v_pk_fma_f16 %0, %1, %2, %0" : "+v"(t) : "v"(ee[q]), "v"(w[3]));
        o[q] = t;
      }
      return make_uint4(o[0], o[1], o[2], o[3]);
    };
    for (int z = 0; z < D; ++z) {
      corners(min(z + 1, D - 1), noff, nwp);
#pragma unroll
      for (int k = 0; k < 4; ++k) asm volatile("" : "+v"(ref[k].x), "+v"(ref[k].y), "+v"(ref[k].z), "+v"(ref[k].w));
      unsigned char* dst = planes + (z % SW_NSLOT) * SW_SLOT;
#define SW_CROUND(R)                                                                                                  \
      do {                                                                                                            \
        SW_CWAIT12(R);                                                                                                \
        {                                                                                                             \
          const uint4 o4 = blend4(ref[R], g[R][0], g[R][1], g[R][2], g[R][3], wco[R]);                                \
          if (actr[R]) *reinterpret_cast<uint4*>(dst + dsto[R]) = o4;                                                 \
        }                                                                                                             \
        SW_CREQ(R, noff, nwp);                                                                                        \
      } while (0)
      SW_CROUND(0); SW_CROUND(1); SW_CROUND(2); SW_CROUND(3);
#undef SW_CROUND
      asm volatile("s_waitcnt lgkmcnt(0)" ::: "memory");
      __builtin_amdgcn_s_barrier();
      asm volatile("" ::: "memory");
    }
    for (int z = D; z < D + SW_LAG; ++z) {
      __builtin_amdgcn_s_barrier();
      asm volatile("" ::: "memory");
    }
#undef SW_CGATHER
#undef SW_CWAIT12
#undef SW_CREQ
    } else {
    const int pv = tid;
    const bool act = pv < SW_NV;
    const int hh = pv / SW_HW, hw = pv - hh * SW_HW;
    const int gh = h0 - 1 + hh, gw = w0 - 1 + hw;
    const bool inb = act && (unsigned)gh < (unsigned)H && (unsigned)gw < (unsigned)W;
    const int partner = (vv + d.B) % d.V, bb = vv % d.B;
    const float* __restrict__ hm = d.homog + (long long)vv * 12;
    const float* __restrict__ dep = d.depths + (long long)bb * D;
    const unsigned char* __restrict__ srcb = reinterpret_cast<const unsigned char*>(d.feat + (long long)partner * H * W * 32);
    unsigned char* dst0 = planes + pv * SW_VS;

    uint4 ref[4];
#pragma unroll
    for (int k = 0; k < 4; ++k) ref[k] = make_uint4(0u, 0u, 0u, 0u);
    if (inb) {
      const unsigned short* pr = d.feat + (((long long)vv * H + gh) * W + gw) * 32;
#pragma unroll
      for (int k = 0; k < 4; ++k) ref[k] = *reinterpret_cast<const uint4*>(pr + k * 8);
    }

    float hmv[12];
#pragma unroll
    for (int e = 0; e < 12; ++e) hmv[e] = hm[e];
    float rx, ry, rz;
    sw_ray(hmv, (float)gw, (float)gh, rx, ry, rz);
    const float t0 = hmv[9], t1 = hmv[10], t2 = hmv[11];
    const float sx = (float)W / (float)(W - 1), sy = (float)H / (float)(H - 1);

    const int dbits = __float_as_int(lane < D ? dep[lane] : 1.f);

    auto corners = [&](int z, Corner& c) {
      sw_corner_weights(rx, ry, rz, t0, t1, t2, __int_as_float(__builtin_amdgcn_readlane(dbits, z)), sx, sy, W, H, inb, c.w, c.off);
      if constexpr (BL == 2) {
        c.wp[0] = pack2_bf16(c.w[0], c.w[1]);
        c.wp[1] = pack2_bf16(c.w[2], c.w[3]);
      }
      if constexpr (std::is_same<T, f16_t>::value && BL == 3) {
#pragma unroll
        for (int q = 0; q < 4; ++q) {
          const Sw16<f16_t>::h2 h = {(f16_t)c.w[q], (f16_t)c.w[q]};
          c.wp[q] = __builtin_bit_cast(unsigned, h);
        }
      }
      if constexpr (SW_SKIP && std::is_same<T, unsigned short>::value) {
        c.skip = __builtin_amdgcn_ballot_w64(c.w[0] != 0.f || c.w[1] != 0.f || c.w[2] != 0.f || c.w[3] != 0.f) == 0ull;
        const unsigned keep = c.skip ? 0u : ~0u;
#pragma unroll
        for (int q = 0; q < 4; ++q) c.off[q] &= keep;
      } else {
        c.skip = false;
// ... 95 lines not shown
        }
        if (o >= 0 && ook[pr]) {
          float v[4];
          TO* const dst = reinterpret_cast<TO*>(d.out) + ((((long long)n * D + o) * H + oh[pr]) * W + ow) * 8 + ch;
#pragma unroll
          for (int r = 0; r < 4; ++r) {
            v[r] = hi[r] + Lp[pr][r];
            v[r] = v[r] < 0.f ? 0.f : v[r];
          }
          store4(dst, v);
        }
        Lp[pr] = lo;
      }
    };

    for (int z = 0; z < D + SW_LAG; ++z) {
      if (z >= SW_LAG) {
        const int p = z - SW_LAG;
        const unsigned char* slot = planes + (p % SW_NSLOT) * SW_SLOT + boff;
        f32x4 Xn[SW_CR_];
#pragma unroll
        for (int f = 0; f < SW_CR_; ++f) Xn[f] = binit;
        uint4 b[SW_CR_ + 2][3];
#pragma unroll
        for (int r = 0; r < SW_CR_ + 2; ++r)
#pragma unroll
          for (int c = 0; c < 3; ++c) {
            b[r][c] = *reinterpret_cast<const uint4*>(slot + (r * SW_HW + c) * SW_VS);
          }
#pragma unroll
        for (int tp = 0; tp < 9; ++tp) {
#pragma unroll
          for (int f = 0; f < SW_CR_; ++f) {
            Xn[f] = Sw16<T>::mma(A01[tp], b[f + tp / 3][tp % 3], Xn[f]);
            Xp[f] = Sw16<T>::mma(A2[tp], b[f + tp / 3][tp % 3], Xp[f]);
          }
        }
        emit(p - 1);
#pragma unroll
        for (int f = 0; f < SW_CR_; ++f) Xp[f] = Xn[f];
      }
      asm volatile("s_waitcnt lgkmcnt(0)" ::: "memory");
      __builtin_amdgcn_s_barrier();
      asm volatile("" ::: "memory");
    }
    emit(D - 1);
  }
}

constexpr int SWP_LAG = 1;
constexpr int SWP_NSLOT = 4;
constexpr int SWP_LDS = SWP_NSLOT * SW_SLOT;

template <typename TO, bool MIX>
__global__ __launch_bounds__(SW_THREADS, 2) void conv0_sweep_persistent_kernel(const SweepDesc d) {
  typedef f16_t T;
  extern __shared__ __attribute__((aligned(16))) unsigned char planes[];
  const int tid = threadIdx.x, lane = tid & 63, wave = tid >> 6;
  const int D = d.D, H = d.H, W = d.W;
  const int nblk = d.tile_list ? d.tile_count[0] : d.N * d.nth * d.ntw;
  const int bq = nblk >> 3, br = nblk & 7, xcd = blockIdx.x & 7;
  const int xbase = xcd < br ? xcd * (bq + 1) : br * (bq + 1) + (xcd - br) * bq, xcnt = bq + (xcd < br);
  const int nt = ((int)(blockIdx.x >> 3) < xcnt) ? (xcnt - (int)(blockIdx.x >> 3) + (int)(gridDim.x >> 3) - 1) / (int)(gridDim.x >> 3) : 0;
  if (nt <= 0) return;
  auto tile_index = [&](int i) -> int {
    const int t = xbase + (int)(blockIdx.x >> 3) + i * (int)(gridDim.x >> 3);
    return __builtin_amdgcn_readfirstlane(d.tile_list ? d.tile_list[t] : t);
  };

  if (wave < SW_NPW) {
    __builtin_amdgcn_s_setreg(1 | (23 << 6), 1);
    const int ck = lane & 3;
    const int pv = tid;
    const bool act = pv < SW_NV;
    const int hh = pv / SW_HW, hw = pv - hh * SW_HW;
    unsigned dsto[4];
    bool actr[4];
    int rhh[4], rhw[4];
#pragma unroll
    for (int r = 0; r < 4; ++r) {
      const int cv = wave * 64 + (lane & ~3) + r;
      rhh[r] = cv / SW_HW; rhw[r] = cv - rhh[r] * SW_HW;
      actr[r] = cv < SW_NV;
      dsto[r] = (unsigned)(cv * SW_VS + ck * 16);
    }
    const float sx = (float)W / (float)(W - 1), sy = (float)H / (float)(H - 1);
    struct TileP { int inb; float rx, ry, rz, t0, t1, t2; int dbits; const unsigned char* srcb; };
    struct TileRaw { float hm[12]; int dbits; int gh, gw; const unsigned char* srcb; };
    auto tile_request = [&](int t, TileRaw& R, uint4 (&rf)[4]) {
      const int tw = t % d.ntw; t /= d.ntw;
      const int th = t % d.nth; t /= d.nth;
      const int n = t, h0 = th * SW_TH, w0 = tw * SW_TW, vv = d.v0 + n;
      const int partner = (vv + d.B) % d.V, bb = vv % d.B;
      const float* __restrict__ hm = d.homog + (long long)vv * 12;
#pragma unroll
      for (int e = 0; e < 12; ++e) R.hm[e] = hm[e];
      R.dbits = __float_as_int(lane < D ? d.depths[(long long)bb * D + lane] : 1.f);
      R.gh = h0 - 1 + hh; R.gw = w0 - 1 + hw;
      R.srcb = reinterpret_cast<const unsigned char*>(d.feat + (long long)partner * H * W * 32);
#pragma unroll
      for (int r = 0; r < 4; ++r) {
        const int ggh = h0 - 1 + rhh[r], ggw = w0 - 1 + rhw[r];
        rf[r] = make_uint4(0u, 0u, 0u, 0u);
        if (actr[r] && (unsigned)ggh < (unsigned)H && (unsigned)ggw < (unsigned)W)
          rf[r] = *reinterpret_cast<const uint4*>(d.feat + (((long long)vv * H + ggh) * W + ggw) * 32 + ck * 8);
      }
    };
    auto tile_finish = [&](const TileRaw& R, TileP& P) {
      P.inb = act && (unsigned)R.gh < (unsigned)H && (unsigned)R.gw < (unsigned)W;
      sw_ray(R.hm, (float)R.gw, (float)R.gh, P.rx, P.ry, P.rz);
      P.t0 = R.hm[9]; P.t1 = R.hm[10]; P.t2 = R.hm[11];
      P.dbits = R.dbits; P.srcb = R.srcb;
    };
    auto corners = [&](int z, const TileP& P, unsigned (&off)[4], unsigned (&wp)[4]) {
      float w[4];
      sw_corner_weights(P.rx, P.ry, P.rz, P.t0, P.t1, P.t2, __int_as_float(__builtin_amdgcn_readlane(P.dbits, z)), sx, sy, W, H, P.inb != 0, w, off);
#pragma unroll
      for (int q = 0; q < 4; ++q) {
        if constexpr (MIX) wp[q] = __float_as_uint(w[q]);
        else {
          const Sw16<f16_t>::h2 h = {(f16_t)w[q], (f16_t)w[q]};
          wp[q] = __builtin_bit_cast(unsigned, h);
        }
      }
    };
    u32x4 g[4][4];
#pragma unroll
    for (int k = 0; k < 4; ++k)
#pragma unroll
      for (int q = 0; q < 4; ++q) g[k][q] = u32x4{0u, 0u, 0u, 0u};
    unsigned wco[4][4];
#define SWP_GATHER(R, Q, OFF, BASE) asm volatile("global_load_dwordx4 %0, %1, %2" : "+v"(g[R][Q]) : "v"(OFF), "s"(BASE) : "memory")
#define SWP_WAIT12(K) asm volatile("s_waitcnt vmcnt(12)" : "+v"(g[K][0]), "+v"(g[K][1]), "+v"(g[K][2]), "+v"(g[K][3]) :: "memory")
#define SWP_REQ(R, OFFV, WPV, BASE)                                                                                   \
    do {                                                                                                              \
      unsigned o_[4];                                                                                                 \
      _Pragma("unroll") for (int q = 0; q < 4; ++q) {                                                                 \
        o_[q] = (unsigned)__builtin_amdgcn_update_dpp(0, (int)(OFFV)[q], (R) * 0x55, 0xf, 0xf, false) | (unsigned)(ck * 16);      \
        wco[R][q] = (unsigned)__builtin_amdgcn_update_dpp(0, (int)(WPV)[q], (R) * 0x55, 0xf, 0xf, false);             \
      }                                                                                                               \
      SWP_GATHER(R, 0, o_[0], BASE); SWP_GATHER(R, 1, o_[1], BASE); SWP_GATHER(R, 2, o_[2], BASE); SWP_GATHER(R, 3, o_[3], BASE);  \
    } while (0)
    auto blend4 = [&](const uint4& r, const u32x4& a, const u32x4& b, const u32x4& c, const u32x4& e, const unsigned (&w)[4]) {
      const unsigned rr[4] = {r.x, r.y, r.z, r.w}, aa[4] = {a[0], a[1], a[2], a[3]}, bb4[4] = {b[0], b[1], b[2], b[3]};
      const unsigned cc[4] = {c[0], c[1], c[2], c[3]}, ee[4] = {e[0], e[1], e[2], e[3]};
      unsigned o[4];
      if constexpr (MIX) {
#define SWP_MIX(HI, D, H, W, C) asm("v_fma_mix_f32 %0, %1, %2, %3 op_sel:[" #HI ",0,0] op_sel_hi:[1,0,0]" : "=v"(D) : "v"(H), "v"(W), "v"(C))
#pragma unroll
        for (int q = 0; q < 4; ++q) {
          float lo, hi;
          asm("v_fma_mix_f32 %0, %1, %2, 0 op_sel:[0,0,0] op_sel_hi:[1,0,0]" : "=v"(lo) : "v"(aa[q]), "v"(w[0]));
          asm("v_fma_mix_f32 %0, %1, %2, 0 op_sel:[1,0,0] op_sel_hi:[1,0,0]" : "=v"(hi) : "v"(aa[q]), "v"(w[0]));
          SWP_MIX(0, lo, bb4[q], w[1], lo); SWP_MIX(1, hi, bb4[q], w[1], hi);
          SWP_MIX(0, lo, cc[q], w[2], lo); SWP_MIX(1, hi, cc[q], w[2], hi);
          SWP_MIX(0, lo, ee[q], w[3], lo); SWP_MIX(1, hi, ee[q], w[3], hi);
          asm("v_fma_mix_f32 %0, %1, 1.0, %2 op_sel:[0,0,0] op_sel_hi:[1,0,0]" : "=v"(lo) : "v"(rr[q]), "v"(lo));
          asm("v_fma_mix_f32 %0, %1, 1.0, %2 op_sel:[1,0,0] op_sel_hi:[1,0,0]" : "=v"(hi) : "v"(rr[q]), "v"(hi));
          const Sw16<f16_t>::h2 h = {(f16_t)lo, (f16_t)hi};
          o[q] = __builtin_bit_cast(unsigned, h);
        }
#undef SWP_MIX
      } else {
#pragma unroll
      for (int q = 0; q < 4; ++q) {
        unsigned t;
        asm("v_pk_fma_f16 %0, %1, %2, %3" : "=v"(t) : "v"(aa[q]), "v"(w[0]), "v"(rr[q]));
        asm("v_pk_fma_f16 %0, %1, %2, %0" : "+v"(t) : "v"(bb4[q]), "v"(w[1]));
        asm("v_pk_fma_f16 %0, %1, %2, %0" : "+v"(t) : "v"(cc[q]), "v"(w[2]));
        asm("v_pk_fma_f16 %0, %1, %2, %0" : "+v"(t) : "v"(ee[q]), "v"(w[3]));
        o[q] = t;
      }
      }
      return make_uint4(o[0], o[1], o[2], o[3]);
    };
#define SWP_PLANE(PREQ, ZREQ)                                                                                         \
    do {                                                                                                              \
      corners((ZREQ), (PREQ), noff, nwp);                                                                             \
      unsigned char* dst = planes + slot * SW_SLOT;                                                                   \
      SWP_ROUND(0, (PREQ).srcb); SWP_ROUND(1, (PREQ).srcb); SWP_ROUND(2, (PREQ).srcb); SWP_ROUND(3, (PREQ).srcb);     \
      slot = (slot + 1) & (SWP_NSLOT - 1);                                                                            \
      asm volatile("s_waitcnt lgkmcnt(0)" ::: "memory");       \
      __builtin_amdgcn_s_barrier();                                                                                   \
      asm volatile("" ::: "memory");                                                                                  \
    } while (0)
#define SWP_ROUND(R, BASE)                                                                                            \
    do {                                                                                                              \
      SWP_WAIT12(R);                                                                                                  \
      const uint4 o4 = blend4(ref[R], g[R][0], g[R][1], g[R][2], g[R][3], wco[R]);                                    \
      if (actr[R]) *reinterpret_cast<uint4*>(dst + dsto[R]) = o4;                                                     \
      SWP_REQ(R, noff, nwp, BASE);                                                                                    \
    } while (0)
    TileRaw raw;
    TileP cur, nxt;
    uint4 ref[4], nref[4];
    unsigned noff[4], nwp[4];
    int slot = 0;
    int t1 = nt > 1 ? tile_index(1) : 0;
    tile_request(tile_index(0), raw, ref);
    tile_finish(raw, cur);
    corners(0, cur, noff, nwp);
    SWP_REQ(0, noff, nwp, cur.srcb); SWP_REQ(1, noff, nwp, cur.srcb); SWP_REQ(2, noff, nwp, cur.srcb); SWP_REQ(3, noff, nwp, cur.srcb);
    for (int ti = 0; ti < nt; ++ti) {
      const bool has_next = ti + 1 < nt;
      if (has_next) tile_request(t1, raw, nref);
      const int t2 = ti + 2 < nt ? tile_index(ti + 2) : 0;
      for (int z = 0; z + 1 < D; ++z) {
#pragma unroll
        for (int k = 0; k < 4; ++k) asm volatile("" : "+v"(ref[k].x), "+v"(ref[k].y), "+v"(ref[k].z), "+v"(ref[k].w));
        SWP_PLANE(cur, z + 1);
      }
      if (has_next) tile_finish(raw, nxt); else nxt = cur;
      SWP_PLANE(nxt, has_next ? 0 : D - 1);
      if (has_next) {
        cur = nxt;
#pragma unroll
        for (int r = 0; r < 4; ++r) ref[r] = nref[r];
      }
      t1 = t2;
    }
    for (int k = 0; k < SWP_LAG; ++k) {
      __builtin_amdgcn_s_barrier();
      asm volatile("" ::: "memory");
    }
#undef SWP_GATHER
#undef SWP_WAIT12
#undef SWP_REQ
#undef SWP_PLANE
#undef SWP_ROUND
  } else {
    const int cw = wave - SW_NPW;
    const int lr = lane & 15, lg = lane >> 4;
    uint4 A01[9], A2[9];
    {
      const uint4* wq = reinterpret_cast<const uint4*>(d.wgt);
#pragma unroll
      for (int s = 0; s < 9; ++s) {
        A01[s] = wq[(s * 16 + lr) * 4 + lg];
        A2[s] = wq[((9 + s) * 16 + lr) * 4 + lg];
      }
    }
    const int ch = (lg & 1) * 4;
    f32x4 binit;
#pragma unroll
    for (int r = 0; r < 4; ++r) binit[r] = lg >= 2 ? d.bias[(lg & 1) * 4 + r] : 0.f;
    const int boff = ((cw * SW_CR_) * SW_HW + lr) * SW_VS + lg * 16;
    __builtin_amdgcn_s_barrier();
    asm volatile("" ::: "memory");
    int slot = 0;
    int t1 = nt > 1 ? tile_index(1) : 0;
    int tcur = tile_index(0);
    for (int ti = 0; ti < nt; ++ti) {
      const int t2 = ti + 2 < nt ? tile_index(ti + 2) : 0;
      int t = tcur;
      const int tw = t % d.ntw; t /= d.ntw;
      const int th = t % d.nth; t /= d.nth;
      const int n = t, h0 = th * SW_TH, w0 = tw * SW_TW;
      const int ow = w0 + lr;
      int oh[SW_NPAIR];
      bool ook[SW_NPAIR];
#pragma unroll
      for (int pr = 0; pr < SW_NPAIR; ++pr) {
        const bool self = 2 * pr + 1 >= SW_CR_;
        oh[pr] = h0 + cw * SW_CR_ + pr * 2 + (self ? 0 : (lg >> 1));
        ook[pr] = oh[pr] < H && ow < W && !(self && lg >= 2);
      }
      f32x4 Xp[SW_CR_], Lp[SW_NPAIR];
#pragma unroll
      for (int f = 0; f < SW_CR_; ++f) Xp[f] = f32x4{0.f, 0.f, 0.f, 0.f};
#pragma unroll
      for (int pr = 0; pr < SW_NPAIR; ++pr) Lp[pr] = f32x4{0.f, 0.f, 0.f, 0.f};
      auto emit = [&](int o) {
#pragma unroll
        for (int pr = 0; pr < SW_NPAIR; ++pr) {
          f32x4 hi, lo;
#pragma unroll
          for (int r = 0; r < 4; ++r) {
            const int f1 = 2 * pr + 1 < SW_CR_ ? 2 * pr + 1 : 2 * pr;
// ... 19 lines not shown
        f32x4 Xn[SW_CR_];
#pragma unroll
        for (int f = 0; f < SW_CR_; ++f) Xn[f] = binit;
#pragma unroll
        for (int tp = 0; tp < 9; ++tp) {
#pragma unroll
          for (int f = 0; f < SW_CR_; ++f) {
            const uint4 b = *reinterpret_cast<const uint4*>(sl + ((f + tp / 3) * SW_HW + tp % 3) * SW_VS);
            Xn[f] = Sw16<T>::mma(A01[tp], b, Xn[f]);
            Xp[f] = Sw16<T>::mma(A2[tp], b, Xp[f]);
          }
        }
        emit(p - 1);
#pragma unroll
        for (int f = 0; f < SW_CR_; ++f) Xp[f] = Xn[f];
        asm volatile("s_waitcnt lgkmcnt(0)" ::: "memory");
        __builtin_amdgcn_s_barrier();
        asm volatile("" ::: "memory");
      }
      emit(D - 1);
      tcur = t1; t1 = t2;
    }
  }
}

void conv0_sweep_pack(const float* w, const float* scale, std::vector<float>& packed) {
  packed.assign((size_t)18 * 16 * 4 * 8, 0.f);
  for (int s = 0; s < 18; ++s)
    for (int row = 0; row < 16; ++row) {
      const int tpl = s % 9, o = row & 7;
      int kd;
      if (s < 9) kd = row < 8 ? 0 : 1;
      else { if (row < 8) continue; kd = 2; }
      const int widx = kd * 9 + tpl;
      for (int g = 0; g < 4; ++g)
        for (int e = 0; e < 8; ++e) {
          const int c = g * 8 + e;
          packed[(((size_t)s * 16 + row) * 4 + g) * 8 + e] = w[((long long)o * 32 + c) * 27 + widx] * (scale ? scale[o] : 1.f);
        }
    }
}

int launch_conv0_sweep(const Conv3dTileDesc& t, int dtype, hipStream_t s) {
  RGBM_REQUIRE(dtype == BF16 || dtype == F16, "conv0 sweep: 16-bit storage types only");
  RGBM_REQUIRE(!t.feat_f16 || dtype == BF16, "conv0 sweep: feat_f16 is the bf16 nets' option");
  SweepDesc d;
  d.feat = reinterpret_cast<const unsigned short*>(t.feat);
  d.wgt = reinterpret_cast<const unsigned short*>(t.wgt);
  d.bias = t.bias; d.homog = t.homog; d.depths = t.depths;
  d.out = reinterpret_cast<unsigned short*>(t.out);
  d.N = t.N; d.D = t.Di; d.H = t.Hi; d.W = t.Wi; d.v0 = t.v0; d.V = t.V; d.B = t.B; d.relu = t.relu;
  d.nth = (d.H + SW_TH - 1) / SW_TH; d.ntw = (d.W + SW_TW - 1) / SW_TW;
  d.tile_list = t.tile_list; d.tile_count = t.tile_count;
  RGBM_REQUIRE(d.feat && d.wgt && d.bias && d.homog && d.depths && d.out && d.D >= 1 && d.D <= 64 && t.Cout == 8, "conv0 sweep arguments");
  RGBM_REQUIRE(t.relu == 1, "conv0 sweep: the kernel applies conv0's ReLU unconditionally");
  RGBM_REQUIRE((d.tile_list == nullptr) == (d.tile_count == nullptr), "conv0 sweep: tile list and count go together");
  const long long nblk = (long long)d.N * d.nth * d.ntw;
  RGBM_REQUIRE(nblk > 0 && nblk < (1ll << 31), "conv0 sweep grid out of range");
  typedef unsigned short u16;
#define SW_LAUNCH(...)                                                                                             \
  do {                                                                                                             \
    auto kern = conv0_sweep_kernel<__VA_ARGS__>;                                                                   \
    if (int rc = ensure_dynamic_lds(reinterpret_cast<const void*>(kern), SW_LDS)) return rc;                       \
    prof_begin_launch(s, t.prof_variant >= 0 ? 14 : -1, t.algo_flops, t.algo_bytes);                               \
    hipLaunchKernelGGL(kern, dim3((unsigned)nblk), dim3(SW_THREADS), SW_LDS, s, d);                                \
  } while (0)
  const bool f21 = (g_debug_flags & (1 << 21)) != 0, f22 = (g_debug_flags & (1 << 22)) != 0;
  if (((dtype == BF16 && t.feat_f16) || dtype == F16) && !(g_debug_flags & (1 << 28))) {
    auto kern = dtype == BF16 ? conv0_sweep_persistent_kernel<u16, false> : f21 ? conv0_sweep_persistent_kernel<f16_t, false>
                                                                                : conv0_sweep_persistent_kernel<f16_t, true>;
    if (int rc = ensure_dynamic_lds(reinterpret_cast<const void*>(kern), SWP_LDS)) return rc;
    int n_cu = 0;
    if (int rc = persistent_grid_cus(&n_cu)) return rc;
    const int grid = nblk < n_cu ? (int)((nblk + 7) / 8 * 8) : n_cu;
    prof_begin_launch(s, t.prof_variant >= 0 ? 14 : -1, t.algo_flops, t.algo_bytes);
    hipLaunchKernelGGL(kern, dim3((unsigned)grid), dim3(SW_THREADS), SWP_LDS, s, d);
  }
  else if (dtype == BF16 && t.feat_f16) SW_LAUNCH(f16_t, u16, 3);
  else if (dtype == BF16 && f22) SW_LAUNCH(u16, u16, 2);
  else if (dtype == BF16 && f21) SW_LAUNCH(u16, u16, 1);
  else if (dtype == BF16) SW_LAUNCH(u16, u16, 0);
  else if (f21) SW_LAUNCH(f16_t, f16_t, 3);
  else SW_LAUNCH(f16_t, f16_t, 0);
#undef SW_LAUNCH
  prof_end_launch(s);
  RGBM_CHECK_HIP(hipGetLastError());
  return 0;
}

}
```

### rgbmanip_amd/csrc/head_kernels.hip

```cpp
#include "common.h"
#include "kernels.h"

namespace rgbm {

template <typename T>
__global__ void gather_points_kernel(const T* __restrict__ feat, const int* __restrict__ choose, float* __restrict__ out,
                                     int V, int P, int HW, int C) {
  const int q = C / 4;
  const long long total = (long long)V * P * q;
  for (long long i = blockIdx.x * (long long)blockDim.x + threadIdx.x; i < total; i += (long long)gridDim.x * blockDim.x) {
    const int c4 = (int)(i % q);
    const long long vp = i / q;
    const long long v = vp / P;
    const int pix = choose[vp];
    float x[4];
    load4(feat + (v * HW + pix) * C + c4 * 4, x);
    store4(out + vp * C + c4 * 4, x);
  }
}

int launch_gather_points(int dtype, const void* feat, const int* choose, float* out, int V, int P, int HW, int C,
                         hipStream_t s) {
  const long long total = (long long)V * P * (C / 4);
  const unsigned g = (unsigned)((total + 255) / 256);
  if (dtype == BF16)
    hipLaunchKernelGGL(gather_points_kernel<unsigned short>, dim3(g), dim3(256), 0, s, (const unsigned short*)feat, choose,
                       out, V, P, HW, C);
  else if (dtype == F16)
    hipLaunchKernelGGL(gather_points_kernel<f16_t>, dim3(g), dim3(256), 0, s, (const f16_t*)feat, choose,
                       out, V, P, HW, C);
  else if (dtype == BF16X3)
    hipLaunchKernelGGL(gather_points_kernel<bx3_t>, dim3(g), dim3(256), 0, s, (const bx3_t*)feat, choose,
                       out, V, P, HW, C);
  else
    hipLaunchKernelGGL(gather_points_kernel<float>, dim3(g), dim3(256), 0, s, (const float*)feat, choose, out, V, P, HW, C);
  RGBM_CHECK_HIP(hipGetLastError());
  return 0;
}


namespace pmlp {
constexpr int NL = 6;
constexpr int cin(int l) { return l == 0 ? 32 : l == 1 ? 64 : l == 2 ? 128 : l == 3 ? 64 : l == 4 ? 16 : 32; }
constexpr int cout(int l) { return l == 0 ? 64 : l == 1 ? 128 : l == 2 ? 64 : l == 3 ? 16 : l == 4 ? 32 : 64; }
constexpr int act(int l) { return l == 3 ? ACT_TANH : ACT_RELU; }
constexpr int w_off(int l) { int o = 0; for (int i = 0; i < l; ++i) o += cin(i) * cout(i); return o; }
constexpr int b_off(int l) { int o = 0; for (int i = 0; i < l; ++i) o += cout(i); return o; }
constexpr int W_FLOATS = w_off(NL), B_FLOATS = b_off(NL);
constexpr int ACT_A = 128 * 16, ACT_B = 64 * 16;
constexpr size_t LDS_BYTES = (size_t)(W_FLOATS + B_FLOATS + 4 * (ACT_A + ACT_B)) * sizeof(float);
}

template <int L>
__device__ __forceinline__ void pmlp_layer(const float* __restrict__ wl, const float* __restrict__ bl, const float* __restrict__ xin,
                                           float* __restrict__ xout, int lane, float* __restrict__ gout4, float* __restrict__ gout64, int ldg) {
  using namespace pmlp;
  constexpr int CI = cin(L), CO = cout(L), KS4 = CI / 16, NT = CO / 16, G = NT < 4 ? NT : 4, AC = act(L);
  const float* wf = wl + w_off(L);
  const float* bf = bl + b_off(L);
#pragma unroll
  for (int t0 = 0; t0 < NT; t0 += G) {
    f32x4 acc[G];
#pragma unroll
    for (int g = 0; g < G; ++g) acc[g] = f32x4{0.f, 0.f, 0.f, 0.f};
#pragma unroll
    for (int k4 = 0; k4 < KS4; ++k4) {
      float bx[4];
#pragma unroll
      for (int j = 0; j < 4; ++j) bx[j] = xin[(k4 * 4 + j) * 64 + lane];
      f32x4 a[G];
#pragma unroll
      for (int g = 0; g < G; ++g) a[g] = *reinterpret_cast<const f32x4*>(wf + (((t0 + g) * KS4 + k4) * 64 + lane) * 4);
#pragma unroll
      for (int j = 0; j < 4; ++j)
#pragma unroll
        for (int g = 0; g < G; ++g) acc[g] = __builtin_amdgcn_mfma_f32_16x16x4f32(a[g][j], bx[j], acc[g], 0, 0, 0);
    }
#pragma unroll
    for (int g = 0; g < G; ++g) {
      const int ch = (t0 + g) * 16 + 4 * (lane >> 4);
      const f32x4 bv = *reinterpret_cast<const f32x4*>(bf + ch);
      float v[4];
#pragma unroll
      for (int i = 0; i < 4; ++i) {
        const float r = acc[g][i] + bv[i];
        v[i] = AC == ACT_RELU ? (r < 0.f ? 0.f : r) : AC == ACT_TANH ? tanhf(r) : r;
      }
      if (L == 3) {
        if (lane < 16) *reinterpret_cast<float4*>(gout4 + (long long)lane * 4) = make_float4(v[0], v[1], v[2], v[3]);
      }
      if (L == NL - 1) {
        *reinterpret_cast<float4*>(gout64 + (long long)(lane & 15) * ldg + ch) = make_float4(v[0], v[1], v[2], v[3]);
      } else {
#pragma unroll
        for (int i = 0; i < 4; ++i) xout[(ch + i) * 16 + (lane & 15)] = v[i];
      }
    }
  }
}

template <typename TF>
__global__ __launch_bounds__(256) void point_mlp_kernel(const PointMlpDesc d) {
  using namespace pmlp;
  extern __shared__ __attribute__((aligned(16))) float pm_lds[];
  float* wl = pm_lds;
  float* bl = wl + W_FLOATS;
  const int tid = threadIdx.x, lane = tid & 63, wave = tid >> 6;
  float* xa = bl + B_FLOATS + wave * (ACT_A + ACT_B);
  float* xb = xa + ACT_A;
  for (int i = tid; i < (W_FLOATS + B_FLOATS) / 4; i += 256) reinterpret_cast<float4*>(wl)[i] = reinterpret_cast<const float4*>(d.table)[i];
  __syncthreads();
  const TF* __restrict__ feat = reinterpret_cast<const TF*>(d.feat);
  const long long ntile = d.N / 64;
  for (long long tile = blockIdx.x; tile < ntile; tile += gridDim.x) {
    const long long p0 = tile * 64 + wave * 16;
#pragma unroll
    for (int r = 0; r < 2; ++r) {
      const int q = lane + 64 * r, pt = q >> 3, c4 = q & 7;
      const long long vp = p0 + pt;
      const long long v = vp / d.P;
      const int pix = d.choose[vp];
      float x[4];
      load4(feat + (v * d.HW + pix) * 32 + c4 * 4, x);
#pragma unroll
      for (int e = 0; e < 4; ++e) xa[(c4 * 4 + e) * 16 + pt] = x[e];
    }
    pmlp_layer<0>(wl, bl, xa, xb, lane, nullptr, nullptr, 0);
    pmlp_layer<1>(wl, bl, xb, xa, lane, nullptr, nullptr, 0);
    pmlp_layer<2>(wl, bl, xa, xb, lane, nullptr, nullptr, 0);
    pmlp_layer<3>(wl, bl, xb, xa, lane, d.nocs4 + p0 * 4, nullptr, 0);
    pmlp_layer<4>(wl, bl, xa, xb, lane, nullptr, nullptr, 0);
    pmlp_layer<5>(wl, bl, xb, xa, lane, nullptr, d.pf + p0 * d.ldpf, d.ldpf);
  }
}

int point_mlp_table_floats() { return pmlp::W_FLOATS + pmlp::B_FLOATS; }

void point_mlp_pack(const float* const w[6], const float* const b[6], float* table) {
  using namespace pmlp;
  const int cin_real[NL] = {32, 64, 128, 64, 3, 32}, cout_real[NL] = {64, 128, 64, 3, 32, 64};
  for (int l = 0; l < NL; ++l) {
    const int CI = cin(l), CO = cout(l), KS4 = CI / 16;
    for (int i = 0; i < CI * CO; ++i) {
      const int j = i & 3, ln = (i >> 2) & 63, q = i >> 8;
      const int k4 = q % KS4, t = q / KS4;
      const int row = 16 * t + (ln & 15), k = 16 * k4 + 4 * j + (ln >> 4);
      table[w_off(l) + i] = (row < cout_real[l] && k < cin_real[l]) ? w[l][(size_t)row * cin_real[l] + k] : 0.f;
    }
    for (int i = 0; i < CO; ++i) table[W_FLOATS + b_off(l) + i] = (b[l] != nullptr && i < cout_real[l]) ? b[l][i] : 0.f;
  }
}

int launch_point_mlp(int feat_dtype, const PointMlpDesc& d, hipStream_t s) {
  RGBM_REQUIRE(d.N > 0 && d.N % 64 == 0 && d.P > 0 && d.ldpf % 4 == 0 && d.table, "point MLP: V * P must be a multiple of 64");
  static_assert((pmlp::W_FLOATS + pmlp::B_FLOATS) % 4 == 0, "the table is copied in 16-byte pieces");
  static_assert(pmlp::LDS_BYTES <= 160 * 1024, "point MLP: weights + four waves' activations must fit the LDS");
  int n_cu = 0;
  if (int rc = persistent_grid_cus(&n_cu)) return rc;
  const long long ntile = d.N / 64;
  const unsigned grid = (unsigned)(ntile < n_cu ? ntile : n_cu);
  const void* fn = feat_dtype == BF16 ? reinterpret_cast<const void*>(point_mlp_kernel<unsigned short>)
                   : feat_dtype == F16 ? reinterpret_cast<const void*>(point_mlp_kernel<f16_t>)
                   : feat_dtype == BF16X3 ? reinterpret_cast<const void*>(point_mlp_kernel<bx3_t>)
                                          : reinterpret_cast<const void*>(point_mlp_kernel<float>);
  if (int rc = ensure_dynamic_lds(fn, (int)pmlp::LDS_BYTES)) return rc;
  if (feat_dtype == BF16)
    hipLaunchKernelGGL(point_mlp_kernel<unsigned short>, dim3(grid), dim3(256), pmlp::LDS_BYTES, s, d);
  else if (feat_dtype == F16)
    hipLaunchKernelGGL(point_mlp_kernel<f16_t>, dim3(grid), dim3(256), pmlp::LDS_BYTES, s, d);
  else if (feat_dtype == BF16X3)
    hipLaunchKernelGGL(point_mlp_kernel<bx3_t>, dim3(grid), dim3(256), pmlp::LDS_BYTES, s, d);
  else
    hipLaunchKernelGGL(point_mlp_kernel<float>, dim3(grid), dim3(256), pmlp::LDS_BYTES, s, d);
  RGBM_CHECK_HIP(hipGetLastError());
  return 0;
}
// ... 55 lines not shown
    float dep = 0.f;
    const int b = v % B;
    const long long o = ((long long)v * P + (pidx - (long long)vl * P));
    for (int dz = 0; dz < D; ++dz) {
      const float pr = logit[pl][dz] * inv;
      prob[o * D + dz] = pr;
      dep += pr * depths[b * D + dz];
    }
    depth_out[o] = dep;
  }
}

int launch_prob_softmax_depth(int dtype, const void* u11, const float* wprob, const int* choose, const float* depths,
                              float* prob, float* depth_out, int v0, int Vc, int B, int P, int D, int H, int W,
                              int classmajor, hipStream_t s) {
  RGBM_REQUIRE(D <= 24, "prob kernel supports up to 24 depth planes");
  const unsigned g = (unsigned)(((long long)Vc * P + 63) / 64);
  if (dtype == BF16)
    hipLaunchKernelGGL(prob_softmax_depth_kernel<unsigned short>, dim3(g), dim3(256), 0, s, (const unsigned short*)u11, wprob,
                       choose, depths, prob, depth_out, v0, Vc, B, P, D, H, W, classmajor);
  else if (dtype == F16)
    hipLaunchKernelGGL(prob_softmax_depth_kernel<f16_t>, dim3(g), dim3(256), 0, s, (const f16_t*)u11, wprob,
                       choose, depths, prob, depth_out, v0, Vc, B, P, D, H, W, classmajor);
  else if (dtype == BF16X3)
    hipLaunchKernelGGL(prob_softmax_depth_kernel<bx3_t>, dim3(g), dim3(256), 0, s, (const bx3_t*)u11, wprob,
                       choose, depths, prob, depth_out, v0, Vc, B, P, D, H, W, classmajor);
  else
    hipLaunchKernelGGL(prob_softmax_depth_kernel<float>, dim3(g), dim3(256), 0, s, (const float*)u11, wprob, choose, depths,
                       prob, depth_out, v0, Vc, B, P, D, H, W, classmajor);
  RGBM_CHECK_HIP(hipGetLastError());
  return 0;
}

__device__ __forceinline__ void warp_coords_h(const float* __restrict__ hm, float x, float y, float depth, int H, int W,
                                              float& ix, float& iy) {
  const float rx = hm[0] * x + hm[1] * y + hm[2];
  const float ry = hm[3] * x + hm[4] * y + hm[5];
  const float rz = hm[6] * x + hm[7] * y + hm[8];
  const float px = rx * depth + hm[9], py = ry * depth + hm[10], pz = rz * depth + hm[11];
  const float u = px / pz, vv = py / pz;
  const float gx = u / ((float)(W - 1) / 2.f) - 1.f;
  const float gy = vv / ((float)(H - 1) / 2.f) - 1.f;
  ix = ((gx + 1.f) * (float)W - 1.f) / 2.f;
  iy = ((gy + 1.f) * (float)H - 1.f) / 2.f;
}

template <typename T> __device__ __forceinline__ float round_through(float f) { return f; }
template <> __device__ __forceinline__ float round_through<unsigned short>(float f) { return bf16_to_f32(f32_to_bf16(f)); }
template <> __device__ __forceinline__ float round_through<f16_t>(float f) { return (float)(f16_t)sat_f16(f); }

template <typename T, bool ROUND_BF16>
__global__ void fuse_points_kernel(const T* __restrict__ feat, const float* __restrict__ homog, const float* __restrict__ depths,
                                   const int* __restrict__ choose, const float* __restrict__ prob, float* __restrict__ out,
                                   int V, int B, int P, int D, int H, int W, int ldo, int ch_off, int Vn) {
  constexpr int C = 32;
  const long long total = (long long)Vn * P * (C / 4);
  for (long long i = blockIdx.x * (long long)blockDim.x + threadIdx.x; i < total; i += (long long)gridDim.x * blockDim.x) {
    const int c4 = (int)(i & 7);
    const long long vp = i >> 3;
    const int v = (int)(vp / P);
    const int partner = (v + B) % V;
    const int b = v % B;
    const int pix = choose[vp];
    const int y = pix / W, x = pix - y * W;
    float ref[4];
    load4(feat + (((long long)v * H + y) * W + x) * C + c4 * 4, ref);
    const T* src = feat + (long long)partner * H * W * C + c4 * 4;
    float acc[4] = {0.f, 0.f, 0.f, 0.f};
    const int lane = threadIdx.x & 63, grp = lane & ~7;
    float cix[3], ciy[3];
    const float* hmv = homog + (long long)__builtin_amdgcn_readfirstlane(v) * 12;
#pragma unroll
    for (int q = 0; q < 3; ++q) {
      const int dz = q * 8 + c4;
      cix[q] = ciy[q] = 0.f;
      if (dz < D) warp_coords_h(hmv, (float)x, (float)y, depths[b * D + dz], H, W, cix[q], ciy[q]);
    }
    for (int dz = 0; dz < D; ++dz) {
      const int q = dz >> 3, srcl = grp + (dz & 7);
      float ix = __shfl(q == 0 ? cix[0] : (q == 1 ? cix[1] : cix[2]), srcl);
      float iy = __shfl(q == 0 ? ciy[0] : (q == 1 ? ciy[1] : ciy[2]), srcl);
      const bool fin = isfinite(ix) && isfinite(iy);
      ix = fminf(fmaxf(fin ? ix : 0.f, -4.f), 1.0e6f);
      iy = fminf(fmaxf(fin ? iy : 0.f, -4.f), 1.0e6f);
      const float fx = floorf(ix), fy = floorf(iy);
      const int x0 = (int)fx, y0 = (int)fy;
      const float tx = ix - fx, ty = iy - fy;
      const bool xin0 = (unsigned)x0 < (unsigned)W, xin1 = (unsigned)(x0 + 1) < (unsigned)W;
      const bool yin0 = (unsigned)y0 < (unsigned)H, yin1 = (unsigned)(y0 + 1) < (unsigned)H;
      const int xc0 = min(max(x0, 0), W - 1), xc1 = min(max(x0 + 1, 0), W - 1);
      const int yc0 = min(max(y0, 0), H - 1), yc1 = min(max(y0 + 1, 0), H - 1);
      float s00[4], s01[4], s10[4], s11[4];
      load4(src + ((long long)yc0 * W + xc0) * C, s00);
      load4(src + ((long long)yc0 * W + xc1) * C, s01);
      load4(src + ((long long)yc1 * W + xc0) * C, s10);
      load4(src + ((long long)yc1 * W + xc1) * C, s11);
      const float w00 = (xin0 && yin0) ? (1.f - tx) * (1.f - ty) : 0.f, w01 = (xin1 && yin0) ? tx * (1.f - ty) : 0.f;
      const float w10 = (xin0 && yin1) ? (1.f - tx) * ty : 0.f, w11 = (xin1 && yin1) ? tx * ty : 0.f;
      const float pr = prob[vp * D + dz];
#pragma unroll
      for (int e = 0; e < 4; ++e) {
        float wv = 0.f;
        if (xin0 && yin0) wv += s00[e] * w00;
        if (xin1 && yin0) wv += s01[e] * w01;
        if (xin0 && yin1) wv += s10[e] * w10;
        if (xin1 && yin1) wv += s11[e] * w11;
        if (!fin) wv = __builtin_nanf("");
        float f = ref[e] + wv;
        if (ROUND_BF16) f = round_through<T>(f);
        acc[e] += f * pr;
      }
    }
    store4(out + vp * ldo + ch_off + c4 * 4, acc);
  }
}

int launch_fuse_points(int dtype, const void* feat, const float* homog, const float* depths, const int* choose,
                       const float* prob, float* out, int V, int B, int P, int D, int H, int W, int ldo, int ch_off,
                       hipStream_t s, int Vn) {
  if (Vn < 0) Vn = V;
  const long long total = (long long)Vn * P * 8;
  RGBM_REQUIRE(D >= 1 && D <= 24 && total > 0 && (total + 255) / 256 < (1ll << 31), "fuse_points supports up to 24 depth planes");
  RGBM_REQUIRE((P & 7) == 0, "fuse_points: the point count must be a multiple of 8 (a wave's 8 points share one view's homography)");
  const unsigned g = (unsigned)((total + 255) / 256);
  if (dtype == BF16)
    hipLaunchKernelGGL((fuse_points_kernel<unsigned short, true>), dim3(g), dim3(256), 0, s, (const unsigned short*)feat,
                       homog, depths, choose, prob, out, V, B, P, D, H, W, ldo, ch_off, Vn);
  else if (dtype == F16)
    hipLaunchKernelGGL((fuse_points_kernel<f16_t, true>), dim3(g), dim3(256), 0, s, (const f16_t*)feat,
                       homog, depths, choose, prob, out, V, B, P, D, H, W, ldo, ch_off, Vn);
  else if (dtype == BF16X3)
    hipLaunchKernelGGL((fuse_points_kernel<bx3_t, false>), dim3(g), dim3(256), 0, s, (const bx3_t*)feat,
                       homog, depths, choose, prob, out, V, B, P, D, H, W, ldo, ch_off, Vn);
  else
    hipLaunchKernelGGL((fuse_points_kernel<float, false>), dim3(g), dim3(256), 0, s, (const float*)feat, homog, depths,
                       choose, prob, out, V, B, P, D, H, W, ldo, ch_off, Vn);
  RGBM_CHECK_HIP(hipGetLastError());
  return 0;
}

constexpr int kMeanSplit = 8;
template <typename TI>
__global__ __launch_bounds__(256) void mean_points_kernel(const TI* __restrict__ in, float* __restrict__ partial, int P, int C) {
  constexpr int E = 16 / sizeof(TI);
  __shared__ float part[256 * E];
  const int v = blockIdx.x / kMeanSplit, sl = blockIdx.x % kMeanSplit;
  const int p0 = (int)((long long)P * sl / kMeanSplit), p1 = (int)((long long)P * (sl + 1) / kMeanSplit);
  const int tpr = C / E, rows = 256 / tpr;
  const int cc = threadIdx.x % tpr, rp = threadIdx.x / tpr;
  float acc[E];
#pragma unroll
  for (int e = 0; e < E; ++e) acc[e] = 0.f;
  if (rp < rows)
#pragma unroll 8
    for (int p = p0 + rp; p < p1; p += rows) {
      float t[E];
      unpack_chunk(*reinterpret_cast<const uint4*>(in + ((long long)v * P + p) * C + cc * E), t, TI());
#pragma unroll
      for (int e = 0; e < E; ++e) acc[e] += t[e];
    }
  if (rp < rows) {
#pragma unroll
    for (int e = 0; e < E; ++e) part[rp * C + cc * E + e] = acc[e];
  }
  __syncthreads();
  for (int c = threadIdx.x; c < C; c += 256) {
    float sum = 0.f;
    for (int r = 0; r < rows; ++r) sum += part[r * C + c];
    partial[(long long)blockIdx.x * C + c] = sum;
  }
}

__device__ __forceinline__ float mean_from_partials(const float* __restrict__ partial, long long v, int c, int C, int P) {
  float sum = 0.f;
#pragma unroll
  for (int sl = 0; sl < kMeanSplit; ++sl) sum += partial[(v * kMeanSplit + sl) * C + c];
  return sum / (float)P;
}

__global__ __launch_bounds__(256) void mean_points_finish_kernel(const float* __restrict__ partial, float* __restrict__ out, int P, int C) {
  const int v = blockIdx.x;
  for (int c = threadIdx.x; c < C; c += 256) out[(long long)v * C + c] = mean_from_partials(partial, v, c, C, P);
}

int launch_mean_points_partial(int dtype, const void* in, float* scratch, int V, int P, int C, hipStream_t s) {
  RGBM_REQUIRE(dtype == F32 || dtype == F16 || dtype == BF16X3, "mean_points: fp32, fp16 or split-pair input");
  RGBM_REQUIRE(scratch != nullptr && (const void*)scratch != in, "mean_points: scratch");
  const int E = dtype == F16 ? 8 : 4;
  RGBM_REQUIRE(C % E == 0 && C / E <= 256 && 256 % (C / E) == 0, "mean_points: channel count");
// ... 256 lines not shown
```

### rgbmanip_amd/csrc/kernels.h

```cpp
#pragma once
#include <vector>

#include "common.h"

namespace rgbm {

int launch_nchw_to_nhwc_pad(int dtype, const float* in, void* out, int V, int C, int H, int W, int Cp, hipStream_t s);
int launch_maxpool3x3s2(int dtype, const void* in, void* out, int V, int H, int W, int C, hipStream_t s);
int launch_resize_bilinear_ac(int dtype, const void* in, void* out, int V, int Hs, int Ws, int C, int Ho, int Wo, int ldo,
                              int ch_off, hipStream_t s);
int launch_copy_channels(int dtype, const void* in, void* out, long long npix, int C, int ldo, int ch_off, hipStream_t s);
int launch_adaptive_avgpool(int dtype, const void* in, void* out, int V, int H, int W, int C, int S, hipStream_t s);
int launch_adaptive_avgpool_multi(int dtype, const void* in, void* const* outs, const int* bins, int nb, int V, int H, int W, int C,
                                  hipStream_t s);
int launch_psp_pool_conv(int dtype, const void* in, int ldi, const void* const* w, void* const* outs, const int* bins, int V, int H, int W,
                         int act, float slope, hipStream_t s);
int launch_psp_resize_cat(int dtype, const void* f, const void* const* stages, const int* bins, void* out, int V, int Ho, int Wo, hipStream_t s);
int launch_homography(const float* P_views, float* out, int V, int B, hipStream_t s);
int launch_build_volume(int dtype, const void* feat, const float* homog, const float* depths, void* vol, int v0, int Vc, int V,
                        int B, int D, int H, int W, hipStream_t s);

int launch_upconv_combine(int dtype, const void* z, const float* bias, void* out, int V, int h, int w, int Co, int ldo, int act,
                          float slope, hipStream_t s, const float* drop = nullptr);
int launch_upconv_final(int dtype, const void* x, const void* wz, const float* bias, float slope, const void* wf, const float* biasf,
                        void* out, int out_f32, int V, int h, int w, hipStream_t s, const void* wf_f16 = nullptr);

constexpr int kDropoutPerView = 256 + 64;
unsigned dropout_threshold(float p);
float dropout_scale(float p);
int launch_dropout_masks(float* masks, unsigned long long* state, int B, float p, unsigned long long seed, int advance, hipStream_t s);

size_t bn_scratch_bytes(int V);
int launch_bn_per_sample(int dtype, void* y, const void* res, const float* gamma, const float* beta, void* scratch, int V,
                         long long nvox, int C, int relu, hipStream_t s);

int launch_to_f32(int dtype, const void* in, float* out, long long n, hipStream_t s);

int launch_gather_points(int dtype, const void* feat, const int* choose, float* out, int V, int P, int HW, int C, hipStream_t s);
int launch_prob_softmax_depth(int dtype, const void* u11, const float* wprob, const int* choose, const float* depths,
                              float* prob, float* depth_out, int v0, int Vc, int B, int P, int D, int H, int W, int classmajor,
                              hipStream_t s);
int launch_fuse_points(int dtype, const void* feat, const float* homog, const float* depths, const int* choose,
                       const float* prob, float* out, int V, int B, int P, int D, int H, int W, int ldo, int ch_off,
                       hipStream_t s, int Vn = -1);
int launch_mean_points(int dtype, const void* in, float* out, float* scratch, int V, int P, int C, hipStream_t s);
int launch_f32_to_f16(const float* in, void* out, long long n, hipStream_t s);
void stem_pack(const float* w, std::vector<float>& packed);
int launch_stem(int dtype, const float* img1, const float* img2, const void* wpk, void* out, int B, int V, int S, hipStream_t s);
int launch_f32_to_bx3(const float* in, void* out, long long n, hipStream_t s);
int launch_view_linear(const float* x, const float* W, const float* bias, float* out, int V, int I, int O, int ldw, int i0,
                       int relu, hipStream_t s);
struct PointMlpDesc {
  const float* table;
  const void* feat;
  const int* choose;
  float* nocs4;
  float* pf;
  int ldpf, P, HW;
  long long N;
};
int point_mlp_table_floats();
void point_mlp_pack(const float* const w[6], const float* const b[6], float* table);
int launch_point_mlp(int feat_dtype, const PointMlpDesc& d, hipStream_t s);
int launch_ortho6d(const float* r6, float* R, int V, hipStream_t s);
int launch_mean_points_partial(int dtype, const void* in, float* scratch, int V, int P, int C, hipStream_t s);
int launch_view_linear_mean(const float* partial, int P, float* mean_out, const float* W, const float* bias, float* out, int V, int I, int O,
                            int ldw, int i0, int relu, hipStream_t s);
int launch_pose_heads_mean(const float* partial, int P, float* mean_out, float* R, float* const w[3][3], float* const b[3][3],
                           float* const out[3], const int odim[3], int V, hipStream_t s);
int launch_pose_heads(const float* pf2, float* const w[3][3], float* const b[3][3], float* const out[3], const int odim[3], int V,
                      hipStream_t s);
int launch_stage_in(const float* P1, const float* P2, const int* c1, const int* c2, float* Pviews, int* choose, int B, int P, hipStream_t s);
int launch_stage_out(const float* nocs4, const float* depth, const float* R, const float* tv, const float* sv, float* const nocs[2],
                     float* const dep[2], float* const r[2], float* const t[2], float* const sz[2], int B, int P, int view2, hipStream_t s);
int launch_copy_cols(const float* in, float* out, long long rows, int ldi, int ldo, int n, hipStream_t s);

struct Conv3dTileDesc {
  const void* in; const void* wgt; void* out; const float* bias; const void* res;
  int N, Di, Hi, Wi;
  int Do, Ho, Wo;
  int Dq, Hq, Wq;
  int ntd, nth, ntw;
  int Cout, relu;
  const void* feat; const float* homog; const float* depths; int v0, V, B;
  int prof_variant; double algo_flops, algo_bytes;
  int out_classmajor;
  int feat_f16;
  const int* tile_list; const int* tile_count;
  int tile_mask_stride;
  const unsigned char* tile_mask;
};
extern int g_debug_flags;
extern long long g_ws_min_rows;
extern int g_tuning_version;
extern int g_gemm_kernel;
void conv3d_tile_pack(const float* w, const float* scale, int Cin, int Cout, int coutp, bool transposed, int dtype,
                      std::vector<float>& packed);
int launch_conv3d_tile(int layer, int dtype, const Conv3dTileDesc& d, hipStream_t s);
int sparse_mask_bytes_per_view(int S);
int sparse_mask_offset(int S, int layer);
int launch_sparse_masks(const int* choose, int v0, int Vc, int P, int S, unsigned char* masks, int* sweep_list, int* sweep_count,
                        hipStream_t s);
int conv3d_tile_dims(int layer, int dtype, int* TD, int* TH, int* TW);

void conv0_sweep_pack(const float* w, const float* scale, std::vector<float>& packed);
int launch_conv0_sweep(const Conv3dTileDesc& d, int dtype, hipStream_t s);

int conv0_sweep_x3_upload(const std::vector<float>& packed, void** dev);
int launch_conv0_sweep_x3(const Conv3dTileDesc& d, hipStream_t s);
int launch_bx3_to_f32(const void* in, float* out, long long n, hipStream_t s);

int launch_prob_sparse(const void* u9, const void* c0, const void* w11_packed, const float* bias11, const float* wprob,
                       const int* choose, const float* depths, float* prob, float* depth_out, int v0, int Vc, int B, int P,
                       int D, int H, int W, int dtype, hipStream_t s, const void* w11_taps = nullptr);
void prob_sparse_pack(const float* w, const float* scale, std::vector<float>& packed);

int launch_prepare_inputs(const float* rgb, const unsigned char* mask, const double* K, const int* frame_map, int N, int H, int W, int S, int P,
                          unsigned seed, float* img, int* choose, float* pts2d, double* Kcrop, int* window, int* valid,
                          unsigned char* small_scratch, hipStream_t s, int frame0 = 0);

int launch_umeyama_ransac(const float* nocs, const float* depth, const int* choose, const double* Kc, const double* E1,
                          double* bbox, double* srt, int* valid, int B, int P, int img, unsigned seed, hipStream_t s);

int launch_projection(const double* Kc, const double* E, float* P, int n, hipStream_t s);
int launch_pnp_ransac(const float* nocs1, const float* pts1, const float* nocs2, const float* pts2, const double* K, const double* E1,
                      const double* E2, double* bbox, double* srt, int* info, int* valid, int B, int P, unsigned seed, hipStream_t s);

int launch_mask_extent(const unsigned char* mask, int N, int H, int W, int* ext, int* count, hipStream_t s);

int launch_postprocess(const float* nocs, const float* depth, const float* rot, const int* choose, const double* Kc,
                       const double* E1, double* bbox, double* ts_out, int* valid, int B, int P, int img, hipStream_t s,
                       void* scratch = nullptr, size_t scratch_bytes = 0);
int launch_microbench_mfma(float* scratch, int iters, int random_operands, double* flops, hipStream_t s);
int microbench_mfma_scratch_floats(int* n);
int launch_microbench_copy(const void* src, void* dst, size_t bytes, hipStream_t s);
size_t postprocess_scratch_bytes(int B);
int postprocess_slices(int B);

int launch_gae(int T, int N, const float* rewards, const unsigned char* dones, const float* values, const float* last_values,
               float gamma, float lam, float* returns, float* adv, double* sums, hipStream_t s);
// ... 16 lines not shown
```

### rgbmanip_amd/csrc/layers.cpp

```cpp
#include "layers.h"
#include "kernels.h"

#include <string.h>

#include <map>
#include <mutex>
#include <utility>
#include <vector>

namespace rgbm {

static thread_local std::string g_err;
void set_error(const std::string& s) { g_err = s; }
const char* last_error_cstr() { return g_err.c_str(); }

static inline unsigned short host_f32_to_bf16(float f) {
  unsigned u;
  memcpy(&u, &f, 4);
  if ((u & 0x7fffffffu) > 0x7f800000u) return (unsigned short)((u >> 16) | 0x40);
  u += 0x7fffu + ((u >> 16) & 1u);
  return (unsigned short)(u >> 16);
}

int ensure_dynamic_lds(const void* fn, int bytes) {
// ... 262 lines not shown
  g.Cin = Cin; g.Cout = 9 * Cout; g.act = ACT_NONE;
  split = (dtype != F32 && 9 * Cout > 256 && (9 * Cout) % 256 != 0 && (9 * Cout) % 256 <= 64 && Cin % 64 == 0) ? (9 * Cout) / 256 * 256 : 0;
  if (split) {
    ConvGeom g1 = g, g2 = g;
    g1.Cout = split; g2.Cout = 9 * Cout - split;
    if (int rc = gemm.init(dtype, g1, wz.data(), nullptr, nullptr, nullptr, Cin, g1.Cout)) return rc;
    if (int rc = gemm2.init(dtype, g2, wz.data() + (size_t)split * Cin, nullptr, nullptr, nullptr, Cin, g2.Cout)) return rc;
  } else {
    if (int rc = gemm.init(dtype, g, wz.data(), nullptr, nullptr, nullptr, Cin, 9 * Cout)) return rc;
  }
  if (bias_h) { if (upload_f32(bias_h, Cout, &bias)) return -2; }
  return 0;
}

void UpConvLayer::destroy() {
  gemm.destroy();
  gemm2.destroy();
  split = 0;
  if (bias) (void)hipFree(bias);
  bias = nullptr;
}

int UpConvLayer::run(const void* in, void* z, void* out, int V, int h, int w, int ldo, hipStream_t s, const float* drop) const {
  if (int rc = gemm.run(in, z, V, 1, h, w, 9 * Cout, nullptr, RES_NONE, nullptr, 0, s)) return rc;
  if (split)
    if (int rc = gemm2.run(in, reinterpret_cast<char*>(z) + (size_t)split * dtype_size(gemm.dtype), V, 1, h, w, 9 * Cout, nullptr, RES_NONE, nullptr, 0, s)) return rc;
  return launch_upconv_combine(gemm.dtype, z, bias, out, V, h, w, Cout, ldo, act, slope, s, drop);
}

int UpConvFinal::init(int dtype_, const float* w3, const float* b3, float slope_, const float* wfin, const float* bfin) {
  RGBM_REQUIRE(dtype_ == BF16 || dtype_ == F16 || dtype_ == BF16X3, "upconv + final: 16-bit or split-pair storage");
  dtype = dtype_; slope = slope_;
  std::vector<float> z((size_t)9 * 64 * 64), f(wfin, wfin + 32 * 64);
  for (int t = 0; t < 9; ++t)
    for (int o = 0; o < 64; ++o)
      for (int c = 0; c < 64; ++c) z[((size_t)t * 64 + o) * 64 + c] = w3[((size_t)o * 64 + c) * 9 + t];
  if (int rc = upload_packed(z, dtype, &wz)) return rc;
  if (int rc = upload_packed(f, dtype, &wf)) return rc;
  if (dtype == BF16 && weights_fit_f16(f)) if (int rc = upload_packed(f, F16, &wf_h)) return rc;
  if (upload_f32(b3, 64, &bias) || upload_f32(bfin, 32, &biasf)) return -2;
  return 0;
}

void UpConvFinal::destroy() {
  if (wz) (void)hipFree(wz);
  if (wf) (void)hipFree(wf);
  if (wf_h) (void)hipFree(wf_h);
  wf_h = nullptr;
  if (bias) (void)hipFree(bias);
  if (biasf) (void)hipFree(biasf);
  wz = wf = nullptr; bias = biasf = nullptr;
}

int UpConvFinal::run(const void* in, void* out, int out_kind, int V, int h, int w, hipStream_t s) const {
  return launch_upconv_final(dtype, in, wz, bias, slope, wf, biasf, out, out_kind, V, h, w, s, wf_h);
}

}
```

### rgbmanip_amd/csrc/layers.h

```cpp
#pragma once
#include <map>
#include <string>
#include <vector>

#include "common.h"

namespace rgbm {

struct HostTensor {
  const float* data = nullptr;
  std::vector<long long> shape;
  long long numel() const { long long n = 1; for (auto s : shape) n *= s; return n; }
};
typedef std::map<std::string, HostTensor> StateDict;

struct ConvGeom {
  int Cin = 0, Cout = 0;
  int KD = 1, KH = 1, KW = 1;
  int sd = 1, sh = 1, sw = 1;
  int pd = 0, ph = 0, pw = 0;
  int dild = 1, dilh = 1, dilw = 1;
  bool transposed = false;
  int act = ACT_NONE;
  float slope = 0.f;
// ... 2 lines not shown
struct PackedConv {
  void* w = nullptr;
  int KD = 1, KH = 1, KW = 1, ntaps = 1, Kpad = 0, KT = 0;
};

struct ConvLayer {
  ConvGeom g;
  int dtype = F32;
  int Cin_pad = 0;
  int Cout_pad = 0;
  float* bias = nullptr;
  std::vector<PackedConv> packs;
  std::vector<void*> owned;
  mutable bool out_plain_f32 = false;

  int init(int dtype, const ConvGeom& g, const float* w, const float* bias, const float* bn_scale, const float* bn_shift,
           int Cin_pad, int Cout_pad);
  void destroy();

  int run(const void* in, void* out, int N, int Di, int Hi, int Wi, int ldo, const void* res, int res_mode,
          const float* bias_override, int bias_stride, hipStream_t s) const;
  void out_dims(int Di, int Hi, int Wi, int& Do, int& Ho, int& Wo) const;
  int run_then_1x1(const ConvLayer& next, const void* in, void* mid, int ldmid, void* out2, int ldo2, int N, int Di, int Hi, int Wi,
                   bool allow_fuse, bool* fused, hipStream_t s) const;
  int build_desc(ConvDesc& d, const void* in, void* out, int N, int Di, int Hi, int Wi, int ldo, const void* res, int res_mode,
                 const float* bias_override, int bias_stride, int cls) const;
};

struct UpConvLayer {
  ConvLayer gemm;
  ConvLayer gemm2;
  int split = 0;
  float* bias = nullptr;
  int Cout = 0, act = ACT_NONE;
  float slope = 0.f;
  int init(int dtype, int Cin, int Cout, const float* w, const float* bias_h, int act, float slope);
  void destroy();
  size_t scratch_elems(int V, int h, int w) const { return (size_t)V * h * w * 9 * Cout; }
  int run(const void* in, void* z, void* out, int V, int h, int w, int ldo, hipStream_t s, const float* drop = nullptr) const;
};

struct UpConvFinal {
  void* wz = nullptr;
  void* wf = nullptr;
  void* wf_h = nullptr;
  float* bias = nullptr;
  float* biasf = nullptr;
  float slope = 0.f;
  int dtype = 0;
  bool ready() const { return wz != nullptr; }
  bool f16_ready() const { return wf_h != nullptr; }
  int init(int dtype, const float* w3, const float* b3, float slope, const float* wfin, const float* bfin);
  void destroy();
  int run(const void* in, void* out, int out_kind, int V, int h, int w, hipStream_t s) const;
};

bool weights_fit_f16(const std::vector<float>& w);
int upload_packed(const std::vector<float>& w, int dtype, void** dev);
int upload_f32(const float* host, size_t n, float** dev);

}
```

### rgbmanip_amd/csrc/upconv_final.hip

```cpp
#include <type_traits>

#include "common.h"
#include "kernels.h"
#include "prof.h"

namespace rgbm {

namespace {

constexpr int kC = 64;
constexpr int kC2 = 32;
constexpr int kLow = 10;
constexpr int kZRow = 272;
constexpr int kNT = 7;

template <typename T> struct Mma16;
template <> struct Mma16<unsigned short> {
  __device__ static __forceinline__ f32x4 run(const uint4& a, const uint4& b, const f32x4& c) {
    return __builtin_amdgcn_mfma_f32_16x16x32_bf16(__builtin_bit_cast(bf16x8, a), __builtin_bit_cast(bf16x8, b), c, 0, 0, 0);
  }
};
template <> struct Mma16<f16_t> {
  __device__ static __forceinline__ f32x4 run(const uint4& a, const uint4& b, const f32x4& c) {
    return __builtin_amdgcn_mfma_f32_16x16x32_f16(__builtin_bit_cast(f16x8, a), __builtin_bit_cast(f16x8, b), c, 0, 0, 0);
// ... 25 lines not shown
      for (int b = 0; b < 4; ++b) acc[a][b] += coef * hx[b];
    }
  }
}

typedef _Float16 uf_h2 __attribute__((ext_vector_type(2)));
__device__ __forceinline__ unsigned uf_pk_fma(unsigned a, unsigned b, unsigned c) {
  return __builtin_bit_cast(unsigned, __builtin_elementwise_fma(__builtin_bit_cast(uf_h2, a), __builtin_bit_cast(uf_h2, b), __builtin_bit_cast(uf_h2, c)));
}
__device__ __forceinline__ unsigned uf_pk_mul(unsigned a, unsigned b) {
  return __builtin_bit_cast(unsigned, __builtin_bit_cast(uf_h2, a) * __builtin_bit_cast(uf_h2, b));
}
constexpr int kZRowH = 144;
template <int KH, int KW>
__device__ __forceinline__ void combine_tap_h(const unsigned char* zl, const unsigned (&wy)[6][2], const unsigned (&wx)[6][2], uint2 (&acc)[4][4]) {
  constexpr int JMIN = KH >> 1, JMAX = ((KH + 3) >> 1) + 1;
  constexpr int CMIN = KW >> 1, CMAX = ((KW + 3) >> 1) + 1;
#pragma unroll
  for (int j = JMIN; j <= JMAX; ++j) {
    uint2 p[4];
#pragma unroll
    for (int c = CMIN; c <= CMAX; ++c) p[c] = *reinterpret_cast<const uint2*>(zl + (j * kLow + c) * kZRowH);
    uint2 hx[4];
#pragma unroll
    for (int b = 0; b < 4; ++b) {
      const int c0 = (b + KW) >> 1;
      hx[b].x = uf_pk_fma(wx[b + KW][1], p[c0 + 1].x, uf_pk_mul(wx[b + KW][0], p[c0].x));
      hx[b].y = uf_pk_fma(wx[b + KW][1], p[c0 + 1].y, uf_pk_mul(wx[b + KW][0], p[c0].y));
    }
#pragma unroll
    for (int a = 0; a < 4; ++a) {
      const int ra = (a + KH) >> 1;
      if (j != ra && j != ra + 1) continue;
      const unsigned coef = wy[a + KH][j == ra ? 0 : 1];
#pragma unroll
      for (int b = 0; b < 4; ++b) {
        acc[a][b].x = uf_pk_fma(coef, hx[b].x, acc[a][b].x);
        acc[a][b].y = uf_pk_fma(coef, hx[b].y, acc[a][b].y);
      }
    }
  }
}

#ifndef UF_HF_WAVES
#define UF_HF_WAVES 2
#endif
#ifndef UF_HF_XLDS
#define UF_HF_XLDS 1
#endif
template <typename T, int OUTK>
__global__ __launch_bounds__(256) __attribute__((amdgpu_waves_per_eu(OUTK == 2 ? UF_HF_WAVES : 2, 8))) void upconv_final_kernel(const T* __restrict__ x, const T* __restrict__ wz,
                                                           const float* __restrict__ bias, float nslope, const T* __restrict__ wf,
                                                           const float* __restrict__ biasf, void* __restrict__ out, int V, int h,
                                                           int w, float sy, float sx) {
  constexpr bool X3 = std::is_same<T, bx3_t>::value;
  constexpr bool HF = OUTK == 2;
  constexpr int ZROW = HF ? kZRowH : kZRow;
  if constexpr (HF) __builtin_amdgcn_s_setreg(1 | (23 << 6), 1);
  constexpr int EB = (int)sizeof(T);
  constexpr int XROW = kC * EB + 16;
  constexpr int CH = kC * EB / 16;
  constexpr int NLD = (kLow * kLow * CH + 255) / 256;
  extern __shared__ __attribute__((aligned(16))) unsigned char lds[];
  unsigned char* Xs = lds;
  unsigned char* Zs = lds + 16 * kNT * XROW;
  unsigned char* Ys = lds;
  const int tid = threadIdx.x, lane = tid & 63, wv = tid >> 6, lr = lane & 15, lg = lane >> 4;
  const int Ho = 2 * h, Wo = 2 * w, nty = Ho / 16, ntx = Wo / 16;
  const unsigned ntile = (unsigned)(V * nty * ntx), per_xcd = (ntile + 7) / 8;
  const unsigned tile = (blockIdx.x & 7) * per_xcd + (blockIdx.x >> 3);
  if (tile >= ntile) return;
  const unsigned v = tile / (unsigned)(nty * ntx);
  const unsigned rem = tile - v * (unsigned)(nty * ntx);
  const int ty = (int)(rem / (unsigned)ntx), tx = (int)(rem - (unsigned)ty * (unsigned)ntx);

  {
    uint4 val[NLD];
#pragma unroll
    for (int k = 0; k < NLD; ++k) {
      const int i = tid + k * 256;
      const int px = min(i / CH, kLow * kLow - 1), c = i & (CH - 1);
      const int pr = px / kLow, pc = px - pr * kLow;
      const int gr = min(max(8 * ty - 1 + pr, 0), h - 1), gc = min(max(8 * tx - 1 + pc, 0), w - 1);
      val[k] = *reinterpret_cast<const uint4*>(reinterpret_cast<const unsigned char*>(x) +
                                               (((long long)v * h + gr) * w + gc) * (kC * EB) + c * 16);
    }
#pragma unroll
    for (int k = 0; k < NLD; ++k) {
      const int i = tid + k * 256;
      if (i < kLow * kLow * CH) *reinterpret_cast<uint4*>(Xs + (i / CH) * XROW + (i & (CH - 1)) * 16) = val[k];
    }
  }

  const int g = tid & 15, blk = tid >> 4, bi = blk >> 2, bj = blk & 3;
  float wy[6][2], wx[6][2];
  {
    const int BI = 4 * ty + bi, BJ = 4 * tx + bj;
#pragma unroll
    for (int k = 0; k < 6; ++k) {
      const int u = 4 * BI - 1 + k;
      const float rel = __fsub_rn(__fmul_rn(sy, (float)u), (float)(2 * BI - 1 + (k >> 1)));
      const bool ok = u >= 0 && u < Ho;
      wy[k][1] = ok ? rel : 0.f;
      wy[k][0] = ok ? 1.f - rel : 0.f;
    }
#pragma unroll
    for (int k = 0; k < 6; ++k) {
// ... 127 lines not shown
  }
  __syncthreads();

  f32x4 facc[2][4];
#pragma unroll
  for (int m = 0; m < 2; ++m)
#pragma unroll
    for (int q = 0; q < 4; ++q) facc[m][q] = f32x4{0.f, 0.f, 0.f, 0.f};
#pragma unroll
  for (int ks = 0; ks < 2; ++ks) {
    if constexpr (X3) {
      uint4 ah[2], al[2], bh[4], bl[4];
#pragma unroll
      for (int m = 0; m < 2; ++m) {
        const T* row = wf + (m * 16 + lr) * kC + ks * 32 + lg * 8;
        bx3_pair(*reinterpret_cast<const uint4*>(row), *reinterpret_cast<const uint4*>(row + 4), ah[m], al[m]);
      }
#pragma unroll
      for (int q = 0; q < 4; ++q) {
        const unsigned char* p = Ys + ((4 * wv + q) * 16 + lr) * XROW + ks * 128 + lg * 32;
        bx3_pair(*reinterpret_cast<const uint4*>(p), *reinterpret_cast<const uint4*>(p + 16), bh[q], bl[q]);
      }
#pragma unroll
      for (int m = 0; m < 2; ++m)
#pragma unroll
        for (int q = 0; q < 4; ++q) facc[m][q] = Mma16<unsigned short>::run(al[m], bh[q], facc[m][q]);
#pragma unroll
      for (int m = 0; m < 2; ++m)
#pragma unroll
        for (int q = 0; q < 4; ++q) facc[m][q] = Mma16<unsigned short>::run(ah[m], bl[q], facc[m][q]);
#pragma unroll
      for (int m = 0; m < 2; ++m)
#pragma unroll
        for (int q = 0; q < 4; ++q) facc[m][q] = Mma16<unsigned short>::run(ah[m], bh[q], facc[m][q]);
    } else {
      uint4 a2[2];
#pragma unroll
      for (int m = 0; m < 2; ++m) a2[m] = *reinterpret_cast<const uint4*>(wf + (m * 16 + lr) * kC + ks * 32 + lg * 8);
#pragma unroll
      for (int q = 0; q < 4; ++q) {
        const uint4 b2 = *reinterpret_cast<const uint4*>(Ys + ((4 * wv + q) * 16 + lr) * XROW + ks * 64 + lg * 16);
#pragma unroll
        for (int m = 0; m < 2; ++m)
          facc[m][q] = Mma16<typename std::conditional<X3, unsigned short, typename std::conditional<HF, f16_t, T>::type>::type>::run(a2[m], b2, facc[m][q]);
      }
    }
  }
#pragma unroll
  for (int m = 0; m < 2; ++m) {
    const f32x4 bv = *reinterpret_cast<const f32x4*>(biasf + m * 16 + lg * 4);
#pragma unroll
    for (int q = 0; q < 4; ++q) {
      const int oy = 16 * ty + 4 * wv + q, ox = 16 * tx + lr;
      const long long o = (((long long)v * Ho + oy) * Wo + ox) * kC2 + m * 16 + lg * 4;
      float r[4];
#pragma unroll
      for (int e = 0; e < 4; ++e) r[e] = facc[m][q][e] + bv[e];
      if constexpr (OUTK == 1) store4(reinterpret_cast<float*>(out) + o, r);
      else if constexpr (OUTK == 2) store4(reinterpret_cast<f16_t*>(out) + o, r);
      else store4(reinterpret_cast<T*>(out) + o, r);
    }
  }
}

template <typename T, int OUTK>
int launch_t(const void* x, const void* wz, const float* bias, float nslope, const void* wf, const float* biasf, void* out, int V,
             int h, int w, hipStream_t s) {
  constexpr int XROW = kC * (int)sizeof(T) + 16;
  constexpr int lds_taps = 16 * kNT * XROW + 16 * kNT * (OUTK == 2 ? kZRowH : kZRow), lds_y = 256 * XROW;
  constexpr int lds = lds_taps > lds_y ? lds_taps : lds_y;
  auto kern = upconv_final_kernel<T, OUTK>;
  if (int rc = ensure_dynamic_lds(reinterpret_cast<const void*>(kern), lds)) return rc;
  const long long ntile = (long long)V * (2 * h / 16) * (2 * w / 16);
  RGBM_REQUIRE(ntile > 0 && ntile < (1ll << 30), "upconv + final grid out of range");
  const unsigned grid = (unsigned)(((ntile + 7) / 8) * 8);
  const float sy = (float)(h - 1) / (float)(2 * h - 1), sx = (float)(w - 1) / (float)(2 * w - 1);
  hipLaunchKernelGGL(kern, dim3(grid), dim3(256), lds, s, (const T*)x, (const T*)wz, bias, nslope, (const T*)wf, biasf, out, V, h, w,
                     sy, sx);
  RGBM_CHECK_HIP(hipGetLastError());
  return 0;
}

}

int launch_upconv_final(int dtype, const void* x, const void* wz, const float* bias, float slope, const void* wf, const float* biasf,
                        void* out, int out_f32, int V, int h, int w, hipStream_t s, const void* wf_f16) {
  RGBM_REQUIRE(dtype == BF16 || dtype == F16 || dtype == BF16X3, "upconv + final: 16-bit or split-pair storage");
  RGBM_REQUIRE(h >= 8 && w >= 8 && h % 8 == 0 && w % 8 == 0, "upconv + final: low-resolution size must be a multiple of 8");
  RGBM_REQUIRE(out_f32 >= 0 && out_f32 <= 2 && (out_f32 != 1 || dtype == BF16X3) && (out_f32 != 2 || dtype == BF16),
               "upconv + final: plain fp32 output is the split-pair path's, f16 output the bf16 path's");
  const double npx = (double)V * 4.0 * h * w;
  prof_begin_launch(s, 39, 2.0 * (npx / 4.0) * 9.0 * kC * kC + 72.0 * npx * kC + 2.0 * npx * kC * kC2,
                    (npx / 4.0) * kC * dtype_size(dtype) + npx * kC2 * (out_f32 == 1 ? 4.0 : (double)dtype_size(dtype)));
  int rc;
  RGBM_REQUIRE(out_f32 != 2 || wf_f16 != nullptr, "upconv + final: the f16 tail needs `final`'s weights in f16");
  if (dtype == BF16 && out_f32 == 2) rc = launch_t<unsigned short, 2>(x, wz, bias, slope, wf_f16, biasf, out, V, h, w, s);
  else if (dtype == BF16) rc = launch_t<unsigned short, 0>(x, wz, bias, slope, wf, biasf, out, V, h, w, s);
  else if (dtype == F16) rc = launch_t<f16_t, 0>(x, wz, bias, slope, wf, biasf, out, V, h, w, s);
  else if (out_f32) rc = launch_t<bx3_t, 1>(x, wz, bias, slope, wf, biasf, out, V, h, w, s);
  else rc = launch_t<bx3_t, 0>(x, wz, bias, slope, wf, biasf, out, V, h, w, s);
  prof_end_launch(s);
  return rc;
}

}
```

Measured before the change: 5810.

## Store f16 feature map with zero border to drop bilinear bounds checks in sweep

When the feature map is stored in f16, it is now laid out with a zero border: one pixel before and two after in each spatial dimension. The plane-sweep conv0 kernel can then gather the four bilinear corners from one offset plus fixed row and column strides, with no per-corner clamping or masking. Weights are packed as f16 pairs and blended with packed FMAs. Every consumer (point gather, fuse points, point MLP, fetch) is updated for the padded pitch, and an extra small kernel zeroes the border after upconv_final, which adds a launch and a little memory.

```diff
diff --git a/include/rgbm.h b/include/rgbm.h
--- a/include/rgbm.h
+++ b/include/rgbm.h
@@ -164,6 +164,9 @@
 int rgbm_conv0_sweep_f16feat(const void* feat_f16_dev, const float* P_views_dev, const float* depths_dev, float* homog_scratch,
                              const float* w_host, const float* bn_scale_host, const float* bn_shift_host, void* out_bf16_dev,
                              int V, int B, int D, int H, int W, void* stream);
+int rgbm_conv0_sweep_f16feat_padded(const void* feat_f16_padded_dev, const float* P_views_dev, const float* depths_dev,
+                                    float* homog_scratch, const float* w_host, const float* bn_scale_host, const float* bn_shift_host,
+                                    void* out_bf16_dev, int V, int B, int D, int H, int W, void* stream);
 int rgbm_adapose_forward_ex(rgbm_adapose_t* h, int B, const float* img1, const float* img2, const int32_t* choose1,
                             const int32_t* choose2, const float* P1, const float* P2, const float* depths, void* workspace,
                             size_t workspace_bytes, const rgbm_adapose_out* out, int stop_after, void* stream);
diff --git a/rgbmanip_amd/_lib.py b/rgbmanip_amd/_lib.py
--- a/rgbmanip_amd/_lib.py
+++ b/rgbmanip_amd/_lib.py
@@ -123,6 +123,7 @@
     "rgbm_conv0_sweep": (_i, [_vp, _vp, _vp, _vp, _vp, _vp, _vp, _vp, _i, _i, _i, _i, _i, _vp]),
     "rgbm_conv0_sweep_dt": (_i, [_i, _vp, _vp, _vp, _vp, _vp, _vp, _vp, _vp, _i, _i, _i, _i, _i, _vp]),
     "rgbm_conv0_sweep_f16feat": (_i, [_vp, _vp, _vp, _vp, _vp, _vp, _vp, _vp, _i, _i, _i, _i, _i, _vp]),
+    "rgbm_conv0_sweep_f16feat_padded": (_i, [_vp, _vp, _vp, _vp, _vp, _vp, _vp, _vp, _i, _i, _i, _i, _i, _vp]),
     "rgbm_prepare_inputs": (_i, [_vp, _vp, _vp, _i, _i, _i, _i, _i, C.c_uint32, _vp, _vp, _vp, _vp, _vp, _vp, _vp, _vp]),
     "rgbm_prepare_inputs_indexed": (_i, [_vp, _vp, _vp, _vp, _i, _i, _i, _i, _i, C.c_uint32, _vp, _vp, _vp, _vp, _vp, _vp, _vp, _vp]),
     "rgbm_prepare_inputs_ex": (_i, [_vp, _vp, _vp, _vp, _i, _i, _i, _i, _i, _i, C.c_uint32, _vp, _vp, _vp, _vp, _vp, _vp, _vp, _vp]),
diff --git a/rgbmanip_amd/csrc/adapose.cpp b/rgbmanip_amd/csrc/adapose.cpp
--- a/rgbmanip_amd/csrc/adapose.cpp
+++ b/rgbmanip_amd/csrc/adapose.cpp
@@ -281,6 +281,8 @@
          tail.ready() && tail.f16_ready();
 }
 
+int AdaPose::feat_pad() const { return feat_f16() ? 1 : 0; }
+
 bool AdaPose::sparse_active() const {
   const bool b16 = dtype_size(dtype) == 2;
   return sparse_dec != 0 && norm_mode == 0 && cost_impl == 3 && (b16 || (dtype == BF16X3 && w11_x3)) && sparse_tail && sweep_w != nullptr &&
@@ -302,7 +304,8 @@
   bf.masks = (unsigned char*)A.alloc((size_t)V * sparse_mask_bytes_per_view(img));
   bf.sweep_list = (int*)A.alloc((size_t)V * ((img + 11) / 12) * ((img + 15) / 16) * 4);
   bf.sweep_count = (int*)A.alloc((size_t)(V + 64) * 4);
-  bf.feat = A.alloc((size_t)V * S * S * 32 * es);
+  const size_t Sp = (size_t)S + 3 * feat_pad();
+  bf.feat = A.alloc((size_t)V * Sp * Sp * 32 * es);
   bf.featf = dtype == BF16X3 ? (float*)A.alloc((size_t)V * S * S * 32 * 4) : nullptr;
   bf.X0 = (float*)A.alloc(VP * 32 * 4);
   bf.X1 = (float*)A.alloc(VP * 64 * 4);
@@ -448,7 +451,7 @@
   }
   fin.out_plain_f32 = feat_f32_only();
   if ((upconv & 4) && tail.ready())
-    return tail.run(bf.u2, fin.out_plain_f32 ? (void*)bf.featf : bf.feat, fin.out_plain_f32 ? 1 : feat_f16() ? 2 : 0, V, 4 * H, 4 * W, s);
+    return tail.run(bf.u2, fin.out_plain_f32 ? (void*)bf.featf : bf.feat, fin.out_plain_f32 ? 1 : feat_f16() ? 2 : 0, V, 4 * H, 4 * W, s, feat_pad());
   if (int rc = launch_resize_bilinear_ac(dtype, bf.u2, bf.ups, V, 4 * H, 4 * W, 64, 8 * H, 8 * W, 64, 0, s)) return rc;
   fin.out_plain_f32 = feat_f32_only();
   if (int rc = up3.run_then_1x1(fin, bf.ups, bf.u3, 64, fin.out_plain_f32 ? (void*)bf.featf : bf.feat, 32, V, 1, 8 * H, 8 * W, fuse_final != 0, nullptr, s)) return rc;
@@ -481,7 +484,7 @@
                     (double)Vc * Do * Ho * Wo * t3d[li].Cout * (res ? 2 : 1)) * (double)dtype_size(dtype);
     if (layer == 10 && cost_impl == 3 && b16 && sweep_w && !(g_debug_flags & 4096)) {
       d.wgt = sweep_w;
-      if (feat_f16()) { d.wgt = sweep_w_f16; d.feat_f16 = 1; }
+      if (feat_f16()) { d.wgt = sweep_w_f16; d.feat_f16 = 1; d.feat_pad = feat_pad(); }
       return launch_conv0_sweep(d, dtype, s);
     }
     if (layer == 10 && cost_impl == 3 && dtype == BF16X3 && sweep_w && !(g_debug_flags & 4096)) {
@@ -616,11 +619,11 @@
   const int Vh = view2_heads ? V : B;
   if (pmlp_table != nullptr && !(g_debug_flags & 2048) && ((long long)Vh * P) % 64 == 0) {
     PointMlpDesc pd{};
-    pd.table = pmlp_table; pd.feat = featg; pd.choose = bf.choose; pd.nocs4 = bf.nocs4; pd.pf = bf.PF96 + 32; pd.ldpf = 96; pd.P = P; pd.HW = S * S;
+    pd.table = pmlp_table; pd.feat = featg; pd.choose = bf.choose; pd.nocs4 = bf.nocs4; pd.pf = bf.PF96 + 32; pd.ldpf = 96; pd.P = P; pd.HW = S * S; pd.W = S; pd.pad = feat_pad();
     pd.N = (long long)Vh * P;
     if (int rc = launch_point_mlp(fdt, pd, s)) return rc;
   } else {
-    if (int rc = launch_gather_points(fdt, featg, bf.choose, bf.X0, Vh, P, S * S, 32, s)) return rc;
+    if (int rc = launch_gather_points(fdt, featg, bf.choose, bf.X0, Vh, P, S * S, 32, s, S, feat_pad())) return rc;
     if (int rc = inst.run(bf.X0, bf.X1, Vh, 1, 1, P, 64, nullptr, 0, nullptr, 0, s)) return rc;
     if (int rc = nh[0].run(bf.X1, bf.H128, Vh, 1, 1, P, 128, nullptr, 0, nullptr, 0, s)) return rc;
     if (int rc = nh[1].run(bf.H128, bf.H64, Vh, 1, 1, P, 64, nullptr, 0, nullptr, 0, s)) return rc;
@@ -632,7 +635,7 @@
   if (int rc = cost_volume(bf, V, B, depths, s)) return rc;
   if (stop_after == 2) return 0;
 
-  if (int rc = launch_fuse_points(fdt, featg, bf.homog, depths, bf.choose, bf.prob, bf.PF96, V, B, P, D, S, S, 96, 0, s, Vh)) return rc;
+  if (int rc = launch_fuse_points(fdt, featg, bf.homog, depths, bf.choose, bf.prob, bf.PF96, V, B, P, D, S, S, 96, 0, s, Vh, feat_pad())) return rc;
   const int pdt = pose_dtype();
   const void* pf_in = bf.PF96;
   if (pdt == F16) {
diff --git a/rgbmanip_amd/csrc/adapose.h b/rgbmanip_amd/csrc/adapose.h
--- a/rgbmanip_amd/csrc/adapose.h
+++ b/rgbmanip_amd/csrc/adapose.h
@@ -104,6 +104,7 @@
   int cost_volume(const Buffers& bf, int V, int B, const float* depths, hipStream_t s) const;
   int chunk_views(int V) const;
   bool feat_f32_only() const;
+  int feat_pad() const;
   bool feat_f16() const;
   bool sparse_active() const;
 };
diff --git a/rgbmanip_amd/csrc/capi.cpp b/rgbmanip_amd/csrc/capi.cpp
--- a/rgbmanip_amd/csrc/capi.cpp
+++ b/rgbmanip_amd/csrc/capi.cpp
@@ -265,6 +265,7 @@
   else if (nm == "u2") { src = bf.u2; cnt = V * (S / 2) * (S / 2) * 64; }
   else if (nm == "u3") { src = bf.u3; cnt = V * S * S * 64; }
   else if (nm == "feat") { src = bf.feat; cnt = V * S * S * 32; if (n.feat_f32_only()) { src = bf.featf; dt = F32; } else if (n.feat_f16()) dt = F16; }
+  else if (nm == "feat_raw") { const size_t Sp = S + 3 * n.feat_pad(); src = bf.feat; cnt = V * Sp * Sp * 32; if (n.feat_f32_only()) { src = bf.featf; cnt = V * S * S * 32; dt = F32; } else if (n.feat_f16()) dt = F16; }
   else if (nm == "vol") { src = bf.vol; cnt = Vc * D * S * S * 32; }
   else if (nm == "c0") { src = bf.c[0]; cnt = Vc * D * S * S * 8; }
   else if (nm == "c2") { src = bf.c[2]; cnt = Vc * (D / 2) * (S / 2) * (S / 2) * 16; }
@@ -284,6 +285,7 @@
                "(the default computes it only inside the chosen pixels' dependency cones)");
   *n_elems = cnt;
   RGBM_REQUIRE(cnt <= capacity, "fetch capacity too small");
+  if (nm == "feat" && n.feat_pad()) return launch_feat_interior_to_f32(src, out_dev, (int)V, (int)S, (int)S, (hipStream_t)stream);
   return launch_to_f32(dt, src, out_dev, (long long)cnt, (hipStream_t)stream);
 }
 
@@ -463,7 +465,7 @@
 
 static int conv0_sweep_entry(int dtype, int feat_f16, const void* feat_dev, const float* P_views_dev, const float* depths_dev,
                              float* homog_scratch, const float* w_host, const float* bn_scale_host, const float* bn_shift_host,
-                             void* out_dev, int V, int B, int D, int H, int W, void* stream) {
+                             void* out_dev, int V, int B, int D, int H, int W, void* stream, int feat_pad = 0) {
   RGBM_REQUIRE(feat_dev && P_views_dev && depths_dev && homog_scratch && w_host && bn_scale_host && bn_shift_host && out_dev,
                "conv0_sweep arguments");
   RGBM_REQUIRE(dtype == BF16 || dtype == F16 || dtype == BF16X3, "conv0_sweep: 16-bit storage types or bf16x3 (fp32 features in, split-pair c0 out)");
@@ -483,6 +485,7 @@
   d.Cout = 8; d.relu = 1; d.prof_variant = -1;
   d.feat = feat_dev; d.homog = homog_scratch; d.depths = depths_dev; d.v0 = 0; d.V = V; d.B = B;
   d.feat_f16 = feat_f16;
+  d.feat_pad = feat_pad;
   int rc = dtype == BF16X3 ? launch_conv0_sweep_x3(d, (hipStream_t)stream) : launch_conv0_sweep(d, dtype, (hipStream_t)stream);
   if (!rc) { hipError_t e = hipStreamSynchronize((hipStream_t)stream); if (e != hipSuccess) { set_error(hipGetErrorString(e)); rc = -2; } }
   (void)hipFree(wdev); (void)hipFree(bdev);
@@ -501,6 +504,13 @@
                                         const float* bn_shift_host, void* out_bf16_dev, int V, int B, int D, int H, int W, void* stream) {
   return conv0_sweep_entry(BF16, 1, feat_f16_dev, P_views_dev, depths_dev, homog_scratch, w_host, bn_scale_host, bn_shift_host, out_bf16_dev,
                            V, B, D, H, W, stream);
+}
+
+extern "C" int rgbm_conv0_sweep_f16feat_padded(const void* feat_f16_padded_dev, const float* P_views_dev, const float* depths_dev,
+                                               float* homog_scratch, const float* w_host, const float* bn_scale_host,
+                                               const float* bn_shift_host, void* out_bf16_dev, int V, int B, int D, int H, int W, void* stream) {
+  return conv0_sweep_entry(BF16, 1, feat_f16_padded_dev, P_views_dev, depths_dev, homog_scratch, w_host, bn_scale_host, bn_shift_host,
+                           out_bf16_dev, V, B, D, H, W, stream, 1);
 }
 
 extern "C" int rgbm_conv0_sweep(const void* feat_dev, const float* P_views_dev, const float* depths_dev, float* homog_scratch,
diff --git a/rgbmanip_amd/csrc/conv0_sweep.hip b/rgbmanip_amd/csrc/conv0_sweep.hip
--- a/rgbmanip_amd/csrc/conv0_sweep.hip
+++ b/rgbmanip_amd/csrc/conv0_sweep.hip
@@ -50,6 +50,7 @@
   const float* depths;
   unsigned short* out;
   int N, D, H, W, v0, V, B, nth, ntw, relu;
+  int pad;
   const int* tile_list; const int* tile_count;
 };
 
@@ -197,10 +198,54 @@
   off[3] = (r1 + (unsigned)xc1) * 64u;
 }
 
-}
-
-template <typename T, typename TO, int BL>
+__device__ __forceinline__ void sw_corner_pad(float rx, float ry, float rz, float t0, float t1, float t2, float depth, float sx, float sy,
+                                              int W, int H, int pitch, bool inb, float (&w)[4], unsigned& off) {
+  const float px = __builtin_fmaf(rx, depth, t0), py = __builtin_fmaf(ry, depth, t1), pz = __builtin_fmaf(rz, depth, t2);
+  const float rinv = __builtin_amdgcn_rcpf(pz);
+  float ix = __builtin_fmaf(px * rinv, sx, -0.5f), iy = __builtin_fmaf(py * rinv, sy, -0.5f);
+  const bool fin = isfinite(ix) && isfinite(iy);
+  ix = __builtin_amdgcn_fmed3f(ix, -1.f, (float)W);
+  iy = __builtin_amdgcn_fmed3f(iy, -1.f, (float)H);
+  const float fx = floorf(ix), fy = floorf(iy);
+  const int x0 = (int)fx, y0 = (int)fy;
+  const float tx = ix - fx, ty = iy - fy;
+  const float ux = 1.f - tx, uy = inb ? 1.f - ty : 0.f, vy = inb ? ty : 0.f;
+  w[0] = ux * uy;
+  w[1] = tx * uy;
+  w[2] = ux * vy;
+  w[3] = tx * vy;
+  if (inb && !fin) w[0] = __builtin_nanf("");
+  off = (unsigned)((y0 + 1) * pitch + x0 + 1) * 64u;
+}
+
+__device__ __forceinline__ void sw_weight_pairs(const float (&w)[4], unsigned (&wp)[2]) {
+  const Sw16<f16_t>::h2 a = {(f16_t)w[0], (f16_t)w[1]}, b = {(f16_t)w[2], (f16_t)w[3]};
+  wp[0] = __builtin_bit_cast(unsigned, a);
+  wp[1] = __builtin_bit_cast(unsigned, b);
+}
+
+__device__ __forceinline__ uint4 sw_blend_pad(const uint4& r, const u32x4& a, const u32x4& b, const u32x4& c, const u32x4& e,
+                                              const unsigned (&w)[2]) {
+  const unsigned rr[4] = {r.x, r.y, r.z, r.w}, aa[4] = {a[0], a[1], a[2], a[3]}, bb[4] = {b[0], b[1], b[2], b[3]};
+  const unsigned cc[4] = {c[0], c[1], c[2], c[3]}, ee[4] = {e[0], e[1], e[2], e[3]};
+  unsigned o[4];
+#pragma unroll
+  for (int q = 0; q < 4; ++q) {
+    unsigned t;
+    asm("v_pk_fma_f16 %0, %1, %2, %3 op_sel_hi:[1,0,1]" : "=v"(t) : "v"(aa[q]), "v"(w[0]), "v"(rr[q]));
+    asm("v_pk_fma_f16 %0, %1, %2, %0 op_sel:[0,1,0] op_sel_hi:[1,1,1]" : "+v"(t) : "v"(bb[q]), "v"(w[0]));
+    asm("v_pk_fma_f16 %0, %1, %2, %0 op_sel_hi:[1,0,1]" : "+v"(t) : "v"(cc[q]), "v"(w[1]));
+    asm("v_pk_fma_f16 %0, %1, %2, %0 op_sel:[0,1,0] op_sel_hi:[1,1,1]" : "+v"(t) : "v"(ee[q]), "v"(w[1]));
+    o[q] = t;
+  }
+  return make_uint4(o[0], o[1], o[2], o[3]);
+}
+
+}
+
+template <typename T, typename TO, int BL, bool PAD = false>
 __global__ __launch_bounds__(SW_THREADS, SW_OCC) void conv0_sweep_kernel(const SweepDesc d) {
+  static_assert(!PAD || (BL == 3 && SW_COOP != 0), "the zero-bordered form is the cooperative packed-f16 one");
   extern __shared__ __attribute__((aligned(16))) unsigned char planes[];
   const int tid = threadIdx.x, lane = tid & 63, wave = tid >> 6;
 
@@ -228,7 +273,9 @@
     const int partner = (vv + d.B) % d.V, bb = vv % d.B;
     const float* __restrict__ hm = d.homog + (long long)vv * 12;
     const float* __restrict__ dep = d.depths + (long long)bb * D;
-    const unsigned char* __restrict__ srcb = reinterpret_cast<const unsigned char*>(d.feat + (long long)partner * H * W * 32);
+    const int Hp = H + (PAD ? 3 : 0), Wp = W + (PAD ? 3 : 0);
+    const unsigned char* __restrict__ srcb = reinterpret_cast<const unsigned char*>(d.feat + (long long)partner * Hp * Wp * 32);
+    const unsigned char* __restrict__ srcb2 = srcb + (long long)Wp * 64;
     uint4 ref[4];
     unsigned dsto[4];
     bool actr[4];
@@ -241,7 +288,7 @@
       dsto[r] = (unsigned)(cv * SW_VS + ck * 16);
       ref[r] = make_uint4(0u, 0u, 0u, 0u);
       if (actr[r] && (unsigned)ggh < (unsigned)H && (unsigned)ggw < (unsigned)W)
-        ref[r] = *reinterpret_cast<const uint4*>(d.feat + (((long long)vv * H + ggh) * W + ggw) * 32 + ck * 8);
+        ref[r] = *reinterpret_cast<const uint4*>(d.feat + (((long long)vv * Hp + ggh + (PAD ? 1 : 0)) * Wp + ggw + (PAD ? 1 : 0)) * 32 + ck * 8);
     }
     float hmv[12];
 #pragma unroll
@@ -253,6 +300,13 @@
     const int dbits = __float_as_int(lane < D ? dep[lane] : 1.f);
     auto corners = [&](int z, unsigned (&off)[4], unsigned (&wp)[4]) {
       float w[4];
+      if constexpr (PAD) {
+        sw_corner_pad(rx, ry, rz, t0, t1, t2, __int_as_float(__builtin_amdgcn_readlane(dbits, z)), sx, sy, W, H, Wp, inb, w, off[0]);
+        unsigned pr[2];
+        sw_weight_pairs(w, pr);
+        wp[0] = pr[0]; wp[1] = pr[1];
+        return;
+      }
       sw_corner_weights(rx, ry, rz, t0, t1, t2, __int_as_float(__builtin_amdgcn_readlane(dbits, z)), sx, sy, W, H, inb, w, off);
 #pragma unroll
       for (int q = 0; q < 4; ++q) {
@@ -268,8 +322,17 @@
     unsigned wco[4][4];
 #define SW_CGATHER(R, Q, OFF) asm volatile("global_load_dwordx4 %0, %1, %2" : "+v"(g[R][Q]) : "v"(OFF), "s"(srcb) : "memory")
 #define SW_CWAIT12(K) asm volatile("s_waitcnt vmcnt(12)" : "+v"(g[K][0]), "+v"(g[K][1]), "+v"(g[K][2]), "+v"(g[K][3]) :: "memory")
+#define SW_CGATHERB(R, Q, OFF, BASE) asm volatile("global_load_dwordx4 %0, %1, %2" : "+v"(g[R][Q]) : "v"(OFF), "s"(BASE) : "memory")
+#define SW_CGATHER64(R, Q, OFF, BASE) asm volatile("global_load_dwordx4 %0, %1, %2 offset:64" : "+v"(g[R][Q]) : "v"(OFF), "s"(BASE) : "memory")
 #define SW_CREQ(R, OFFV, WPV)                                                                                         \
     do {                                                                                                              \
+      if constexpr (PAD) {                                                       \
+        const unsigned o0_ = (unsigned)__builtin_amdgcn_update_dpp(0, (int)(OFFV)[0], (R) * 0x55, 0xf, 0xf, false) | (unsigned)(ck * 16);  \
+        wco[R][0] = (unsigned)__builtin_amdgcn_mov_dpp((int)(WPV)[0], (R) * 0x55, 0xf, 0xf, true);      \
+        wco[R][1] = (unsigned)__builtin_amdgcn_mov_dpp((int)(WPV)[1], (R) * 0x55, 0xf, 0xf, true);                    \
+        SW_CGATHER(R, 0, o0_); SW_CGATHER64(R, 1, o0_, srcb); SW_CGATHERB(R, 2, o0_, srcb2); SW_CGATHER64(R, 3, o0_, srcb2);  \
+        break;                                                                                                        \
+      }                                                                                                               \
       unsigned o_[4];                                                                                                 \
       _Pragma("unroll") for (int q = 0; q < 4; ++q) {                                                                 \
         o_[q] = (unsigned)__builtin_amdgcn_update_dpp(0, (int)(OFFV)[q], (R) * 0x55, 0xf, 0xf, false) | (unsigned)(ck * 16);      \
@@ -304,7 +367,9 @@
       do {                                                                                                            \
         SW_CWAIT12(R);                                                                                                \
         {                                                                                                             \
-          const uint4 o4 = blend4(ref[R], g[R][0], g[R][1], g[R][2], g[R][3], wco[R]);                                \
+          uint4 o4;                                                                                                   \
+          if constexpr (PAD) o4 = sw_blend_pad(ref[R], g[R][0], g[R][1], g[R][2], g[R][3], {wco[R][0], wco[R][1]});   \
+          else o4 = blend4(ref[R], g[R][0], g[R][1], g[R][2], g[R][3], wco[R]);                                       \
           if (actr[R]) *reinterpret_cast<uint4*>(dst + dsto[R]) = o4;                                                 \
         }                                                                                                             \
         SW_CREQ(R, noff, nwp);                                                                                        \
@@ -320,6 +385,8 @@
       asm volatile("" ::: "memory");
     }
 #undef SW_CGATHER
+#undef SW_CGATHERB
+#undef SW_CGATHER64
 #undef SW_CWAIT12
 #undef SW_CREQ
     } else {
@@ -521,12 +588,14 @@
 constexpr int SWP_NSLOT = 4;
 constexpr int SWP_LDS = SWP_NSLOT * SW_SLOT;
 
-template <typename TO, bool MIX>
+template <typename TO, bool MIX, bool PAD>
 __global__ __launch_bounds__(SW_THREADS, 2) void conv0_sweep_persistent_kernel(const SweepDesc d) {
   typedef f16_t T;
+  static_assert(!(PAD && MIX), "the zero-bordered form has the packed blend only");
   extern __shared__ __attribute__((aligned(16))) unsigned char planes[];
   const int tid = threadIdx.x, lane = tid & 63, wave = tid >> 6;
   const int D = d.D, H = d.H, W = d.W;
+  const int Hp = H + (PAD ? 3 : 0), Wp = W + (PAD ? 3 : 0);
   const int nblk = d.tile_list ? d.tile_count[0] : d.N * d.nth * d.ntw;
   const int bq = nblk >> 3, br = nblk & 7, xcd = blockIdx.x & 7;
   const int xbase = xcd < br ? xcd * (bq + 1) : br * (bq + 1) + (xcd - br) * bq, xcnt = bq + (xcd < br);
@@ -554,7 +623,7 @@
       dsto[r] = (unsigned)(cv * SW_VS + ck * 16);
     }
     const float sx = (float)W / (float)(W - 1), sy = (float)H / (float)(H - 1);
-    struct TileP { int inb; float rx, ry, rz, t0, t1, t2; int dbits; const unsigned char* srcb; };
+    struct TileP { int inb; float rx, ry, rz, t0, t1, t2; int dbits; const unsigned char* srcb; const unsigned char* srcb2; };
     struct TileRaw { float hm[12]; int dbits; int gh, gw; const unsigned char* srcb; };
     auto tile_request = [&](int t, TileRaw& R, uint4 (&rf)[4]) {
       const int tw = t % d.ntw; t /= d.ntw;
@@ -566,23 +635,31 @@
       for (int e = 0; e < 12; ++e) R.hm[e] = hm[e];
       R.dbits = __float_as_int(lane < D ? d.depths[(long long)bb * D + lane] : 1.f);
       R.gh = h0 - 1 + hh; R.gw = w0 - 1 + hw;
-      R.srcb = reinterpret_cast<const unsigned char*>(d.feat + (long long)partner * H * W * 32);
+      R.srcb = reinterpret_cast<const unsigned char*>(d.feat + (long long)partner * Hp * Wp * 32);
 #pragma unroll
       for (int r = 0; r < 4; ++r) {
         const int ggh = h0 - 1 + rhh[r], ggw = w0 - 1 + rhw[r];
         rf[r] = make_uint4(0u, 0u, 0u, 0u);
         if (actr[r] && (unsigned)ggh < (unsigned)H && (unsigned)ggw < (unsigned)W)
-          rf[r] = *reinterpret_cast<const uint4*>(d.feat + (((long long)vv * H + ggh) * W + ggw) * 32 + ck * 8);
+          rf[r] = *reinterpret_cast<const uint4*>(d.feat + (((long long)vv * Hp + ggh + (PAD ? 1 : 0)) * Wp + ggw + (PAD ? 1 : 0)) * 32 + ck * 8);
       }
     };
     auto tile_finish = [&](const TileRaw& R, TileP& P) {
       P.inb = act && (unsigned)R.gh < (unsigned)H && (unsigned)R.gw < (unsigned)W;
       sw_ray(R.hm, (float)R.gw, (float)R.gh, P.rx, P.ry, P.rz);
       P.t0 = R.hm[9]; P.t1 = R.hm[10]; P.t2 = R.hm[11];
-      P.dbits = R.dbits; P.srcb = R.srcb;
+      P.dbits = R.dbits; P.srcb = R.srcb; P.srcb2 = R.srcb + (long long)Wp * 64;
     };
     auto corners = [&](int z, const TileP& P, unsigned (&off)[4], unsigned (&wp)[4]) {
       float w[4];
+      if constexpr (PAD) {
+        sw_corner_pad(P.rx, P.ry, P.rz, P.t0, P.t1, P.t2, __int_as_float(__builtin_amdgcn_readlane(P.dbits, z)), sx, sy, W, H, Wp, P.inb != 0, w,
+                      off[0]);
+        unsigned pr[2];
+        sw_weight_pairs(w, pr);
+        wp[0] = pr[0]; wp[1] = pr[1];
+        return;
+      }
       sw_corner_weights(P.rx, P.ry, P.rz, P.t0, P.t1, P.t2, __int_as_float(__builtin_amdgcn_readlane(P.dbits, z)), sx, sy, W, H, P.inb != 0, w, off);
 #pragma unroll
       for (int q = 0; q < 4; ++q) {
@@ -601,8 +678,16 @@
     unsigned wco[4][4];
 #define SWP_GATHER(R, Q, OFF, BASE) asm volatile("global_load_dwordx4 %0, %1, %2" : "+v"(g[R][Q]) : "v"(OFF), "s"(BASE) : "memory")
 #define SWP_WAIT12(K) asm volatile("s_waitcnt vmcnt(12)" : "+v"(g[K][0]), "+v"(g[K][1]), "+v"(g[K][2]), "+v"(g[K][3]) :: "memory")
-#define SWP_REQ(R, OFFV, WPV, BASE)                                                                                   \
+#define SWP_GATHER64(R, Q, OFF, BASE) asm volatile("global_load_dwordx4 %0, %1, %2 offset:64" : "+v"(g[R][Q]) : "v"(OFF), "s"(BASE) : "memory")
+#define SWP_REQ(R, OFFV, WPV, BASE, BASE2)                                                                            \
     do {                                                                                                              \
+      if constexpr (PAD) {                                                                                            \
+        const unsigned o0_ = (unsigned)__builtin_amdgcn_update_dpp(0, (int)(OFFV)[0], (R) * 0x55, 0xf, 0xf, false) | (unsigned)(ck * 16);  \
+        wco[R][0] = (unsigned)__builtin_amdgcn_mov_dpp((int)(WPV)[0], (R) * 0x55, 0xf, 0xf, true);      \
+        wco[R][1] = (unsigned)__builtin_amdgcn_mov_dpp((int)(WPV)[1], (R) * 0x55, 0xf, 0xf, true);                    \
+        SWP_GATHER(R, 0, o0_, BASE); SWP_GATHER64(R, 1, o0_, BASE); SWP_GATHER(R, 2, o0_, BASE2); SWP_GATHER64(R, 3, o0_, BASE2);  \
+        break;                                                                                                        \
+      }                                                                                                               \
       unsigned o_[4];                                                                                                 \
       _Pragma("unroll") for (int q = 0; q < 4; ++q) {                                                                 \
         o_[q] = (unsigned)__builtin_amdgcn_update_dpp(0, (int)(OFFV)[q], (R) * 0x55, 0xf, 0xf, false) | (unsigned)(ck * 16);      \
@@ -647,18 +732,20 @@
     do {                                                                                                              \
       corners((ZREQ), (PREQ), noff, nwp);                                                                             \
       unsigned char* dst = planes + slot * SW_SLOT;                                                                   \
-      SWP_ROUND(0, (PREQ).srcb); SWP_ROUND(1, (PREQ).srcb); SWP_ROUND(2, (PREQ).srcb); SWP_ROUND(3, (PREQ).srcb);     \
+      SWP_ROUND(0, PREQ); SWP_ROUND(1, PREQ); SWP_ROUND(2, PREQ); SWP_ROUND(3, PREQ);                                 \
       slot = (slot + 1) & (SWP_NSLOT - 1);                                                                            \
       asm volatile("s_waitcnt lgkmcnt(0)" ::: "memory");       \
       __builtin_amdgcn_s_barrier();                                                                                   \
       asm volatile("" ::: "memory");                                                                                  \
     } while (0)
-#define SWP_ROUND(R, BASE)                                                                                            \
+#define SWP_ROUND(R, PREQ)                                                                                            \
     do {                                                                                                              \
       SWP_WAIT12(R);                                                                                                  \
-      const uint4 o4 = blend4(ref[R], g[R][0], g[R][1], g[R][2], g[R][3], wco[R]);                                    \
+      uint4 o4;                                                                                                       \
+      if constexpr (PAD) o4 = sw_blend_pad(ref[R], g[R][0], g[R][1], g[R][2], g[R][3], {wco[R][0], wco[R][1]});       \
+      else o4 = blend4(ref[R], g[R][0], g[R][1], g[R][2], g[R][3], wco[R]);                                           \
       if (actr[R]) *reinterpret_cast<uint4*>(dst + dsto[R]) = o4;                                                     \
-      SWP_REQ(R, noff, nwp, BASE);                                                                                    \
+      SWP_REQ(R, noff, nwp, (PREQ).srcb, (PREQ).srcb2);                                                               \
     } while (0)
     TileRaw raw;
     TileP cur, nxt;
@@ -669,7 +756,8 @@
     tile_request(tile_index(0), raw, ref);
     tile_finish(raw, cur);
     corners(0, cur, noff, nwp);
-    SWP_REQ(0, noff, nwp, cur.srcb); SWP_REQ(1, noff, nwp, cur.srcb); SWP_REQ(2, noff, nwp, cur.srcb); SWP_REQ(3, noff, nwp, cur.srcb);
+    SWP_REQ(0, noff, nwp, cur.srcb, cur.srcb2); SWP_REQ(1, noff, nwp, cur.srcb, cur.srcb2); SWP_REQ(2, noff, nwp, cur.srcb, cur.srcb2);
+    SWP_REQ(3, noff, nwp, cur.srcb, cur.srcb2);
     for (int ti = 0; ti < nt; ++ti) {
       const bool has_next = ti + 1 < nt;
       if (has_next) tile_request(t1, raw, nref);
@@ -693,6 +781,7 @@
       asm volatile("" ::: "memory");
     }
 #undef SWP_GATHER
+#undef SWP_GATHER64
 #undef SWP_WAIT12
 #undef SWP_REQ
 #undef SWP_PLANE
@@ -818,6 +907,8 @@
   d.N = t.N; d.D = t.Di; d.H = t.Hi; d.W = t.Wi; d.v0 = t.v0; d.V = t.V; d.B = t.B; d.relu = t.relu;
   d.nth = (d.H + SW_TH - 1) / SW_TH; d.ntw = (d.W + SW_TW - 1) / SW_TW;
   d.tile_list = t.tile_list; d.tile_count = t.tile_count;
+  d.pad = t.feat_pad;
+  RGBM_REQUIRE(d.pad == 0 || (d.pad == 1 && dtype == BF16 && t.feat_f16), "conv0 sweep: the zero-bordered feature map is the f16 map of a bf16 net");
   RGBM_REQUIRE(d.feat && d.wgt && d.bias && d.homog && d.depths && d.out && d.D >= 1 && d.D <= 64 && t.Cout == 8, "conv0 sweep arguments");
   RGBM_REQUIRE(t.relu == 1, "conv0 sweep: the kernel applies conv0's ReLU unconditionally");
   RGBM_REQUIRE((d.tile_list == nullptr) == (d.tile_count == nullptr), "conv0 sweep: tile list and count go together");
@@ -833,8 +924,8 @@
   } while (0)
   const bool f21 = (g_debug_flags & (1 << 21)) != 0, f22 = (g_debug_flags & (1 << 22)) != 0;
   if (((dtype == BF16 && t.feat_f16) || dtype == F16) && !(g_debug_flags & (1 << 28))) {
-    auto kern = dtype == BF16 ? conv0_sweep_persistent_kernel<u16, false> : f21 ? conv0_sweep_persistent_kernel<f16_t, false>
-                                                                                : conv0_sweep_persistent_kernel<f16_t, true>;
+    auto kern = dtype == BF16 ? (d.pad ? conv0_sweep_persistent_kernel<u16, false, true> : conv0_sweep_persistent_kernel<u16, false, false>)
+                              : f21 ? conv0_sweep_persistent_kernel<f16_t, false, false> : conv0_sweep_persistent_kernel<f16_t, true, false>;
     if (int rc = ensure_dynamic_lds(reinterpret_cast<const void*>(kern), SWP_LDS)) return rc;
     int n_cu = 0;
     if (int rc = persistent_grid_cus(&n_cu)) return rc;
@@ -842,6 +933,7 @@
     prof_begin_launch(s, t.prof_variant >= 0 ? 14 : -1, t.algo_flops, t.algo_bytes);
     hipLaunchKernelGGL(kern, dim3((unsigned)grid), dim3(SW_THREADS), SWP_LDS, s, d);
   }
+  else if (dtype == BF16 && t.feat_f16 && d.pad) SW_LAUNCH(f16_t, u16, 3, true);
   else if (dtype == BF16 && t.feat_f16) SW_LAUNCH(f16_t, u16, 3);
   else if (dtype == BF16 && f22) SW_LAUNCH(u16, u16, 2);
   else if (dtype == BF16 && f21) SW_LAUNCH(u16, u16, 1);
diff --git a/rgbmanip_amd/csrc/head_kernels.hip b/rgbmanip_amd/csrc/head_kernels.hip
--- a/rgbmanip_amd/csrc/head_kernels.hip
+++ b/rgbmanip_amd/csrc/head_kernels.hip
@@ -5,7 +5,8 @@
 
 template <typename T>
 __global__ void gather_points_kernel(const T* __restrict__ feat, const int* __restrict__ choose, float* __restrict__ out,
-                                     int V, int P, int HW, int C) {
+                                     int V, int P, int HW, int C, int W, int pad) {
+  const long long vstride = pad ? (long long)(HW / W + 3) * (W + 3) : HW;
   const int q = C / 4;
   const long long total = (long long)V * P * q;
   for (long long i = blockIdx.x * (long long)blockDim.x + threadIdx.x; i < total; i += (long long)gridDim.x * blockDim.x) {
@@ -13,27 +14,29 @@
     const long long vp = i / q;
     const long long v = vp / P;
     const int pix = choose[vp];
+    const int ppix = pad ? pix + (pix / W) * 3 + W + 4 : pix;
     float x[4];
-    load4(feat + (v * HW + pix) * C + c4 * 4, x);
+    load4(feat + (v * vstride + ppix) * C + c4 * 4, x);
     store4(out + vp * C + c4 * 4, x);
   }
 }
 
 int launch_gather_points(int dtype, const void* feat, const int* choose, float* out, int V, int P, int HW, int C,
-                         hipStream_t s) {
+                         hipStream_t s, int W, int pad) {
+  RGBM_REQUIRE(pad == 0 || (pad == 1 && W > 0 && HW % W == 0), "gather_points: the zero-bordered map needs its width");
   const long long total = (long long)V * P * (C / 4);
   const unsigned g = (unsigned)((total + 255) / 256);
   if (dtype == BF16)
     hipLaunchKernelGGL(gather_points_kernel<unsigned short>, dim3(g), dim3(256), 0, s, (const unsigned short*)feat, choose,
-                       out, V, P, HW, C);
+                       out, V, P, HW, C, W, pad);
   else if (dtype == F16)
     hipLaunchKernelGGL(gather_points_kernel<f16_t>, dim3(g), dim3(256), 0, s, (const f16_t*)feat, choose,
-                       out, V, P, HW, C);
+                       out, V, P, HW, C, W, pad);
   else if (dtype == BF16X3)
     hipLaunchKernelGGL(gather_points_kernel<bx3_t>, dim3(g), dim3(256), 0, s, (const bx3_t*)feat, choose,
-                       out, V, P, HW, C);
+                       out, V, P, HW, C, W, pad);
   else
-    hipLaunchKernelGGL(gather_points_kernel<float>, dim3(g), dim3(256), 0, s, (const float*)feat, choose, out, V, P, HW, C);
+    hipLaunchKernelGGL(gather_points_kernel<float>, dim3(g), dim3(256), 0, s, (const float*)feat, choose, out, V, P, HW, C, W, pad);
   RGBM_CHECK_HIP(hipGetLastError());
   return 0;
 }
@@ -111,6 +114,7 @@
   for (int i = tid; i < (W_FLOATS + B_FLOATS) / 4; i += 256) reinterpret_cast<float4*>(wl)[i] = reinterpret_cast<const float4*>(d.table)[i];
   __syncthreads();
   const TF* __restrict__ feat = reinterpret_cast<const TF*>(d.feat);
+  const long long vstride = d.pad ? (long long)(d.HW / d.W + 3) * (d.W + 3) : d.HW;
   const long long ntile = d.N / 64;
   for (long long tile = blockIdx.x; tile < ntile; tile += gridDim.x) {
     const long long p0 = tile * 64 + wave * 16;
@@ -120,8 +124,9 @@
       const long long vp = p0 + pt;
       const long long v = vp / d.P;
       const int pix = d.choose[vp];
+      const int ppix = d.pad ? pix + (pix / d.W) * 3 + d.W + 4 : pix;
       float x[4];
-      load4(feat + (v * d.HW + pix) * 32 + c4 * 4, x);
+      load4(feat + (v * vstride + ppix) * 32 + c4 * 4, x);
 #pragma unroll
       for (int e = 0; e < 4; ++e) xa[(c4 * 4 + e) * 16 + pt] = x[e];
     }
@@ -283,7 +288,7 @@
 template <typename T, bool ROUND_BF16>
 __global__ void fuse_points_kernel(const T* __restrict__ feat, const float* __restrict__ homog, const float* __restrict__ depths,
                                    const int* __restrict__ choose, const float* __restrict__ prob, float* __restrict__ out,
-                                   int V, int B, int P, int D, int H, int W, int ldo, int ch_off, int Vn) {
+                                   int V, int B, int P, int D, int H, int W, int ldo, int ch_off, int Vn, int pad) {
   constexpr int C = 32;
   const long long total = (long long)Vn * P * (C / 4);
   for (long long i = blockIdx.x * (long long)blockDim.x + threadIdx.x; i < total; i += (long long)gridDim.x * blockDim.x) {
@@ -294,9 +299,10 @@
     const int b = v % B;
     const int pix = choose[vp];
     const int y = pix / W, x = pix - y * W;
+    const int Hp = H + 3 * pad, Wp = W + 3 * pad;
     float ref[4];
-    load4(feat + (((long long)v * H + y) * W + x) * C + c4 * 4, ref);
-    const T* src = feat + (long long)partner * H * W * C + c4 * 4;
+    load4(feat + (((long long)v * Hp + y + pad) * Wp + x + pad) * C + c4 * 4, ref);
+    const T* src = feat + ((long long)partner * Hp * Wp + (long long)pad * (Wp + 1)) * C + c4 * 4;
     float acc[4] = {0.f, 0.f, 0.f, 0.f};
     const int lane = threadIdx.x & 63, grp = lane & ~7;
     float cix[3], ciy[3];
@@ -322,10 +328,10 @@
       const int xc0 = min(max(x0, 0), W - 1), xc1 = min(max(x0 + 1, 0), W - 1);
       const int yc0 = min(max(y0, 0), H - 1), yc1 = min(max(y0 + 1, 0), H - 1);
       float s00[4], s01[4], s10[4], s11[4];
-      load4(src + ((long long)yc0 * W + xc0) * C, s00);
-      load4(src + ((long long)yc0 * W + xc1) * C, s01);
-      load4(src + ((long long)yc1 * W + xc0) * C, s10);
-      load4(src + ((long long)yc1 * W + xc1) * C, s11);
+      load4(src + ((long long)yc0 * Wp + xc0) * C, s00);
+      load4(src + ((long long)yc0 * Wp + xc1) * C, s01);
+      load4(src + ((long long)yc1 * Wp + xc0) * C, s10);
+      load4(src + ((long long)yc1 * Wp + xc1) * C, s11);
       const float w00 = (xin0 && yin0) ? (1.f - tx) * (1.f - ty) : 0.f, w01 = (xin1 && yin0) ? tx * (1.f - ty) : 0.f;
       const float w10 = (xin0 && yin1) ? (1.f - tx) * ty : 0.f, w11 = (xin1 && yin1) ? tx * ty : 0.f;
       const float pr = prob[vp * D + dz];
@@ -348,24 +354,25 @@
 
 int launch_fuse_points(int dtype, const void* feat, const float* homog, const float* depths, const int* choose,
                        const float* prob, float* out, int V, int B, int P, int D, int H, int W, int ldo, int ch_off,
-                       hipStream_t s, int Vn) {
+                       hipStream_t s, int Vn, int pad) {
   if (Vn < 0) Vn = V;
+  RGBM_REQUIRE(pad == 0 || pad == 1, "fuse_points: pad is 0 or 1");
   const long long total = (long long)Vn * P * 8;
   RGBM_REQUIRE(D >= 1 && D <= 24 && total > 0 && (total + 255) / 256 < (1ll << 31), "fuse_points supports up to 24 depth planes");
   RGBM_REQUIRE((P & 7) == 0, "fuse_points: the point count must be a multiple of 8 (a wave's 8 points share one view's homography)");
   const unsigned g = (unsigned)((total + 255) / 256);
   if (dtype == BF16)
     hipLaunchKernelGGL((fuse_points_kernel<unsigned short, true>), dim3(g), dim3(256), 0, s, (const unsigned short*)feat,
-                       homog, depths, choose, prob, out, V, B, P, D, H, W, ldo, ch_off, Vn);
+                       homog, depths, choose, prob, out, V, B, P, D, H, W, ldo, ch_off, Vn, pad);
   else if (dtype == F16)
     hipLaunchKernelGGL((fuse_points_kernel<f16_t, true>), dim3(g), dim3(256), 0, s, (const f16_t*)feat,
-                       homog, depths, choose, prob, out, V, B, P, D, H, W, ldo, ch_off, Vn);
+                       homog, depths, choose, prob, out, V, B, P, D, H, W, ldo, ch_off, Vn, pad);
   else if (dtype == BF16X3)
     hipLaunchKernelGGL((fuse_points_kernel<bx3_t, false>), dim3(g), dim3(256), 0, s, (const bx3_t*)feat,
-                       homog, depths, choose, prob, out, V, B, P, D, H, W, ldo, ch_off, Vn);
+                       homog, depths, choose, prob, out, V, B, P, D, H, W, ldo, ch_off, Vn, pad);
   else
     hipLaunchKernelGGL((fuse_points_kernel<float, false>), dim3(g), dim3(256), 0, s, (const float*)feat, homog, depths,
-                       choose, prob, out, V, B, P, D, H, W, ldo, ch_off, Vn);
+                       choose, prob, out, V, B, P, D, H, W, ldo, ch_off, Vn, pad);
   RGBM_CHECK_HIP(hipGetLastError());
   return 0;
 }
diff --git a/rgbmanip_amd/csrc/kernels.h b/rgbmanip_amd/csrc/kernels.h
--- a/rgbmanip_amd/csrc/kernels.h
+++ b/rgbmanip_amd/csrc/kernels.h
@@ -23,7 +23,10 @@
 int launch_upconv_combine(int dtype, const void* z, const float* bias, void* out, int V, int h, int w, int Co, int ldo, int act,
                           float slope, hipStream_t s, const float* drop = nullptr);
 int launch_upconv_final(int dtype, const void* x, const void* wz, const float* bias, float slope, const void* wf, const float* biasf,
-                        void* out, int out_f32, int V, int h, int w, hipStream_t s, const void* wf_f16 = nullptr);
+                        void* out, int out_f32, int V, int h, int w, hipStream_t s, const void* wf_f16 = nullptr,
+                        int pad = 0);
+
+int launch_feat_interior_to_f32(const void* padded, float* out, int V, int H, int W, hipStream_t s);
 
 constexpr int kDropoutPerView = 256 + 64;
 unsigned dropout_threshold(float p);
@@ -36,13 +39,15 @@
 
 int launch_to_f32(int dtype, const void* in, float* out, long long n, hipStream_t s);
 
-int launch_gather_points(int dtype, const void* feat, const int* choose, float* out, int V, int P, int HW, int C, hipStream_t s);
+int launch_gather_points(int dtype, const void* feat, const int* choose, float* out, int V, int P, int HW, int C, hipStream_t s, int W = 0,
+                         int pad = 0);
 int launch_prob_softmax_depth(int dtype, const void* u11, const float* wprob, const int* choose, const float* depths,
                               float* prob, float* depth_out, int v0, int Vc, int B, int P, int D, int H, int W, int classmajor,
                               hipStream_t s);
 int launch_fuse_points(int dtype, const void* feat, const float* homog, const float* depths, const int* choose,
                        const float* prob, float* out, int V, int B, int P, int D, int H, int W, int ldo, int ch_off,
-                       hipStream_t s, int Vn = -1);
+                       hipStream_t s, int Vn = -1,
+                       int pad = 0);
 int launch_mean_points(int dtype, const void* in, float* out, float* scratch, int V, int P, int C, hipStream_t s);
 int launch_f32_to_f16(const float* in, void* out, long long n, hipStream_t s);
 void stem_pack(const float* w, std::vector<float>& packed);
@@ -58,6 +63,7 @@
   float* pf;
   int ldpf, P, HW;
   long long N;
+  int W, pad;
 };
 int point_mlp_table_floats();
 void point_mlp_pack(const float* const w[6], const float* const b[6], float* table);
@@ -86,6 +92,7 @@
   int prof_variant; double algo_flops, algo_bytes;
   int out_classmajor;
   int feat_f16;
+  int feat_pad;
   const int* tile_list; const int* tile_count;
   int tile_mask_stride;
   const unsigned char* tile_mask;
diff --git a/rgbmanip_amd/csrc/layers.cpp b/rgbmanip_amd/csrc/layers.cpp
--- a/rgbmanip_amd/csrc/layers.cpp
+++ b/rgbmanip_amd/csrc/layers.cpp
@@ -338,8 +338,8 @@
   wz = wf = nullptr; bias = biasf = nullptr;
 }
 
-int UpConvFinal::run(const void* in, void* out, int out_kind, int V, int h, int w, hipStream_t s) const {
-  return launch_upconv_final(dtype, in, wz, bias, slope, wf, biasf, out, out_kind, V, h, w, s, wf_h);
-}
-
-}
+int UpConvFinal::run(const void* in, void* out, int out_kind, int V, int h, int w, hipStream_t s, int pad) const {
+  return launch_upconv_final(dtype, in, wz, bias, slope, wf, biasf, out, out_kind, V, h, w, s, wf_h, pad);
+}
+
+}
diff --git a/rgbmanip_amd/csrc/layers.h b/rgbmanip_amd/csrc/layers.h
--- a/rgbmanip_amd/csrc/layers.h
+++ b/rgbmanip_amd/csrc/layers.h
@@ -78,7 +78,7 @@
   bool f16_ready() const { return wf_h != nullptr; }
   int init(int dtype, const float* w3, const float* b3, float slope, const float* wfin, const float* bfin);
   void destroy();
-  int run(const void* in, void* out, int out_kind, int V, int h, int w, hipStream_t s) const;
+  int run(const void* in, void* out, int out_kind, int V, int h, int w, hipStream_t s, int pad = 0) const;
 };
 
 bool weights_fit_f16(const std::vector<float>& w);
diff --git a/rgbmanip_amd/csrc/upconv_final.hip b/rgbmanip_amd/csrc/upconv_final.hip
--- a/rgbmanip_amd/csrc/upconv_final.hip
+++ b/rgbmanip_amd/csrc/upconv_final.hip
@@ -101,7 +101,7 @@
 __global__ __launch_bounds__(256) __attribute__((amdgpu_waves_per_eu(OUTK == 2 ? UF_HF_WAVES : 2, 8))) void upconv_final_kernel(const T* __restrict__ x, const T* __restrict__ wz,
                                                            const float* __restrict__ bias, float nslope, const T* __restrict__ wf,
                                                            const float* __restrict__ biasf, void* __restrict__ out, int V, int h,
-                                                           int w, float sy, float sx) {
+                                                           int w, float sy, float sx, int pad) {
   constexpr bool X3 = std::is_same<T, bx3_t>::value;
   constexpr bool HF = OUTK == 2;
   constexpr int ZROW = HF ? kZRowH : kZRow;
@@ -335,7 +335,8 @@
 #pragma unroll
     for (int q = 0; q < 4; ++q) {
       const int oy = 16 * ty + 4 * wv + q, ox = 16 * tx + lr;
-      const long long o = (((long long)v * Ho + oy) * Wo + ox) * kC2 + m * 16 + lg * 4;
+      const int pd = OUTK == 2 ? pad : 0;
+      const long long o = (((long long)v * (Ho + 3 * pd) + oy + pd) * (Wo + 3 * pd) + ox + pd) * kC2 + m * 16 + lg * 4;
       float r[4];
 #pragma unroll
       for (int e = 0; e < 4; ++e) r[e] = facc[m][q][e] + bv[e];
@@ -346,9 +347,38 @@
   }
 }
 
+__global__ __launch_bounds__(256) void zero_border_kernel(uint4* __restrict__ out, int V, int H, int W) {
+  const int Wp = W + 3, nb = 3 * Wp + 3 * H;
+  const long long total = (long long)V * nb * 4;
+  for (long long i = blockIdx.x * 256ll + threadIdx.x; i < total; i += (long long)gridDim.x * 256) {
+    const int ck = (int)(i & 3);
+    const long long pix = i >> 2;
+    const int v = (int)(pix / nb), b = (int)(pix - (long long)v * nb);
+    int y, x;
+    if (b < 3 * Wp) { const int r = b / Wp; y = r == 0 ? 0 : H + r; x = b - r * Wp; }
+    else { const int j = b - 3 * Wp, c = j % 3; y = 1 + j / 3; x = c == 0 ? 0 : W + c; }
+    out[(((long long)v * (H + 3) + y) * Wp + x) * 4 + ck] = make_uint4(0u, 0u, 0u, 0u);
+  }
+}
+
+typedef __attribute__((ext_vector_type(2))) _Float16 Sw2;
+__global__ __launch_bounds__(256) void feat_interior_kernel(const uint2* __restrict__ in, float4* __restrict__ out, int V, int H, int W) {
+  const long long total = (long long)V * H * W * 8;
+  for (long long i = blockIdx.x * 256ll + threadIdx.x; i < total; i += (long long)gridDim.x * 256) {
+    const int c = (int)(i & 7);
+    const long long p = i >> 3;
+    const int x = (int)(p % W);
+    const long long vy = p / W;
+    const int y = (int)(vy % H), v = (int)(vy / H);
+    const uint2 u = in[(((long long)v * (H + 3) + y + 1) * (W + 3) + x + 1) * 8 + c];
+    const Sw2 a = __builtin_bit_cast(Sw2, u.x), b = __builtin_bit_cast(Sw2, u.y);
+    out[i] = make_float4((float)a.x, (float)a.y, (float)b.x, (float)b.y);
+  }
+}
+
 template <typename T, int OUTK>
 int launch_t(const void* x, const void* wz, const float* bias, float nslope, const void* wf, const float* biasf, void* out, int V,
-             int h, int w, hipStream_t s) {
+             int h, int w, hipStream_t s, int pad) {
   constexpr int XROW = kC * (int)sizeof(T) + 16;
   constexpr int lds_taps = 16 * kNT * XROW + 16 * kNT * (OUTK == 2 ? kZRowH : kZRow), lds_y = 256 * XROW;
   constexpr int lds = lds_taps > lds_y ? lds_taps : lds_y;
@@ -359,15 +389,29 @@
   const unsigned grid = (unsigned)(((ntile + 7) / 8) * 8);
   const float sy = (float)(h - 1) / (float)(2 * h - 1), sx = (float)(w - 1) / (float)(2 * w - 1);
   hipLaunchKernelGGL(kern, dim3(grid), dim3(256), lds, s, (const T*)x, (const T*)wz, bias, nslope, (const T*)wf, biasf, out, V, h, w,
-                     sy, sx);
+                     sy, sx, pad);
+  RGBM_CHECK_HIP(hipGetLastError());
+  if (pad) {
+    const long long n = (long long)V * (3 * (2 * w + 3) + 3 * 2 * h) * 4;
+    hipLaunchKernelGGL(zero_border_kernel, dim3((unsigned)((n + 255) / 256)), dim3(256), 0, s, (uint4*)out, V, 2 * h, 2 * w);
+    RGBM_CHECK_HIP(hipGetLastError());
+  }
+  return 0;
+}
+
+}
+
+int launch_feat_interior_to_f32(const void* padded, float* out, int V, int H, int W, hipStream_t s) {
+  const long long n = (long long)V * H * W * 8;
+  RGBM_REQUIRE(n > 0 && (n + 255) / 256 < (1ll << 31), "feature map interior: size");
+  hipLaunchKernelGGL(feat_interior_kernel, dim3((unsigned)((n + 255) / 256)), dim3(256), 0, s, (const uint2*)padded, (float4*)out, V, H, W);
   RGBM_CHECK_HIP(hipGetLastError());
   return 0;
 }
 
-}
-
 int launch_upconv_final(int dtype, const void* x, const void* wz, const float* bias, float slope, const void* wf, const float* biasf,
-                        void* out, int out_f32, int V, int h, int w, hipStream_t s, const void* wf_f16) {
+                        void* out, int out_f32, int V, int h, int w, hipStream_t s, const void* wf_f16, int pad) {
+  RGBM_REQUIRE(pad == 0 || (pad == 1 && out_f32 == 2), "upconv + final: only the f16 feature map is zero-bordered");
   RGBM_REQUIRE(dtype == BF16 || dtype == F16 || dtype == BF16X3, "upconv + final: 16-bit or split-pair storage");
   RGBM_REQUIRE(h >= 8 && w >= 8 && h % 8 == 0 && w % 8 == 0, "upconv + final: low-resolution size must be a multiple of 8");
   RGBM_REQUIRE(out_f32 >= 0 && out_f32 <= 2 && (out_f32 != 1 || dtype == BF16X3) && (out_f32 != 2 || dtype == BF16),
@@ -377,11 +421,11 @@
                     (npx / 4.0) * kC * dtype_size(dtype) + npx * kC2 * (out_f32 == 1 ? 4.0 : (double)dtype_size(dtype)));
   int rc;
   RGBM_REQUIRE(out_f32 != 2 || wf_f16 != nullptr, "upconv + final: the f16 tail needs `final`'s weights in f16");
-  if (dtype == BF16 && out_f32 == 2) rc = launch_t<unsigned short, 2>(x, wz, bias, slope, wf_f16, biasf, out, V, h, w, s);
-  else if (dtype == BF16) rc = launch_t<unsigned short, 0>(x, wz, bias, slope, wf, biasf, out, V, h, w, s);
-  else if (dtype == F16) rc = launch_t<f16_t, 0>(x, wz, bias, slope, wf, biasf, out, V, h, w, s);
-  else if (out_f32) rc = launch_t<bx3_t, 1>(x, wz, bias, slope, wf, biasf, out, V, h, w, s);
-  else rc = launch_t<bx3_t, 0>(x, wz, bias, slope, wf, biasf, out, V, h, w, s);
+  if (dtype == BF16 && out_f32 == 2) rc = launch_t<unsigned short, 2>(x, wz, bias, slope, wf_f16, biasf, out, V, h, w, s, pad);
+  else if (dtype == BF16) rc = launch_t<unsigned short, 0>(x, wz, bias, slope, wf, biasf, out, V, h, w, s, 0);
+  else if (dtype == F16) rc = launch_t<f16_t, 0>(x, wz, bias, slope, wf, biasf, out, V, h, w, s, 0);
+  else if (out_f32) rc = launch_t<bx3_t, 1>(x, wz, bias, slope, wf, biasf, out, V, h, w, s, 0);
+  else rc = launch_t<bx3_t, 0>(x, wz, bias, slope, wf, biasf, out, V, h, w, s, 0);
   prof_end_launch(s);
   return rc;
 }
```

Result: no change. 5837 (median of 6 runs) (+0.5%).
